# Michaelszeng/GCS-ADMM

Measured on AMD Instinct MI355X. Metric: admm_iterations_per_sec, higher is better.
Workload: dtype f64; 1 GPU; benchmark4; V=42, E=94, n=2, state_dtype=f64, state_columns=incidence, inner_arithmetic=f64, vertex_program=workgroup, vertex_solves=warm start from the previous iteration's record (csrc/warm_start.h), parallelism=1 GPU

## Files before the change

gcs_admm_amd/abi.py:

```python
from __future__ import annotations

import ctypes as C
import os

import numpy as np

LIB_PATH = os.path.join(os.path.dirname(os.path.abspath(__file__)), "libgcsadmm.so")

F64, F32 = 0, 1
RUNNING, CONVERGED, MAX_IT, DIVERGED = -1, 0, 1, 2
STATUS_NAME = {RUNNING: "running", CONVERGED: "converged", MAX_IT: "max_it", DIVERGED: "diverged"}


class GraphDesc(C.Structure):
    _fields_ = [("n", C.c_int32), ("num_vertices", C.c_int32), ("num_edges", C.c_int32), ("num_incidences", C.c_int32),
                ("inc_ptr", C.c_void_p), ("inc_edge", C.c_void_p), ("inc_out", C.c_void_p),
                ("edge_inc_tail", C.c_void_p), ("edge_inc_head", C.c_void_p),
                ("poly_ptr", C.c_void_p), ("poly_A", C.c_void_p), ("poly_b", C.c_void_p), ("center", C.c_void_p),
                ("src", C.c_int32), ("dst", C.c_int32), ("state_dtype", C.c_int32), ("device", C.c_int32),
                ("inc_counted", C.c_void_p), ("edge_counted", C.c_void_p),
                ("nx_global", C.c_double), ("nmu_global", C.c_double),
                ("vertex_program", C.c_int32), ("wave_slots", C.c_int32), ("wave_align", C.c_int32),
                ("wave_store_dl", C.c_int32), ("wave_generic_rows", C.c_int32), ("edge_major_columns", C.c_int32),
                ("vertex_workspace", C.c_int32)]


class Params(C.Structure):
    _fields_ = [("rho", C.c_double), ("tau_incr", C.c_double), ("tau_decr", C.c_double), ("nu", C.c_double),
                ("it_rho_limit", C.c_int32), ("max_it", C.c_int32), ("eps_abs", C.c_double), ("eps_rel", C.c_double),
                ("eps_edge", C.c_double), ("ipm_tol", C.c_double), ("ipm_max_iter", C.c_int32), ("cold_start", C.c_int32)]


class State(C.Structure):
    _fields_ = [("copy", C.c_void_p), ("mu", C.c_void_p), ("zedge", C.c_void_p),
                ("xv", C.c_void_p), ("zv", C.c_void_p), ("yv", C.c_void_p)]


class HaloDesc(C.Structure):
    _fields_ = [("num_peers", C.c_int32), ("peer_rank", C.c_void_p), ("send_ptr", C.c_void_p), ("send_cols", C.c_void_p),
                ("recv_ptr", C.c_void_p), ("recv_cols", C.c_void_p)]


class ControlBlock(C.Structure):
    _fields_ = [("rho", C.c_double), ("mu_scale", C.c_double), ("sums", C.c_double * 5),
                ("pri", C.c_double), ("dual", C.c_double), ("eps_pri", C.c_double), ("eps_dual", C.c_double),
                ("it", C.c_int32), ("status", C.c_int32), ("inner_failures", C.c_int32), ("inner_iters", C.c_int32)]


_p, _i, _d = C.c_void_p, C.c_int32, C.c_double
_run, _run_timed = [_p, _p, _i, _p, _p], [_p, _p, _i, _p, _p] + [_p] * 4
_csr = [_i, _i, _p, _p, _p]
PROTOTYPES = {
    "gcsadmm_create": ([_p, _p], _i),
    "gcsadmm_destroy": ([_p], None),
    "gcsadmm_last_error": ([_p], C.c_char_p),
    "gcsadmm_reset": ([_p] * 3, _i),
    "gcsadmm_vertex_step": ([_p] * 3, _i),
    "gcsadmm_edge_step": ([_p] * 4, _i),
    "gcsadmm_control": ([_p] * 4, _i),
    "gcsadmm_run": (_run, _i),
    "gcsadmm_read_control": ([_p] * 3, _i),
    "gcsadmm_cost": ([_p, _p, _d, _p, _p], _i),
    "gcsadmm_query": ([_p] * 6, _i),
    "gcsadmm_query_workspace": ([_p] * 4, _i),
    "gcsadmm_unit_iterations": ([_p, _p, _i, _p, _p], _i),
    "gcsadmm_run_timed": (_run_timed, _i),
    "gcsadmm_batch_create": ([_p, _i, _p], _i),
    "gcsadmm_batch_destroy": ([_p], None),
    "gcsadmm_batch_last_error": ([_p], C.c_char_p),
    "gcsadmm_batch_bind": ([_p] * 4, _i),
    "gcsadmm_batch_run": ([_p, _i, _p], _i),
    "gcsadmm_batch_poll": ([_p] * 4, _i),
    "gcsadmm_vertex_prox": ([_p] * 6 + [_d, _i, _p, _p], _i),
    "gcsadmm_comm_unique_id": ([_p], _i),
    "gcsadmm_attach_comm": ([_p, _i, _i, _p, _p], _i),
    "gcsadmm_check_halo": ([_p, _i, _i, _p], _i),
    "gcsadmm_run_partitioned": (_run, _i),
    "gcsadmm_run_partitioned_timed": (_run_timed, _i),
    "gcsadmm_set_overlap": ([_p, _i, _p], _i),
    "gcsadmm_comm_count": ([_p, _p], _i),
    "gcsadmm_halo_pack": ([_p] * 3, _i),
    "gcsadmm_halo_unpack": ([_p] * 3, _i),
    "gcsadmm_halo_exchange": ([_p] * 3, _i),
    "gcsadmm_halo_buffers": ([_p] * 4, _i),
    "gcsadmm_polytope_last_error": ([], C.c_char_p),
    "gcsadmm_polytope_centers": (_csr + [_i, _p, _p, _p], _i),
    "gcsadmm_polytope_bounds": (_csr + [_p, _i, _p, _p, _p], _i),
    "gcsadmm_polytope_overlaps": (_csr + [_p, C.c_long, _p, _p, _d, _i, _p, _p], _i),
    "gcsadmm_scene_create": (_csr + [_i, _p], _i),
    "gcsadmm_scene_destroy": ([_p], None),
    "gcsadmm_scene_centers": ([_p] * 4, _i),
    "gcsadmm_scene_bounds": ([_p] * 4, _i),
    "gcsadmm_scene_set_boxes": ([_p] * 3, _i),
    "gcsadmm_scene_candidate_pairs": ([_p, _d, _p], _i),
    "gcsadmm_scene_overlaps": ([_p, _d, _p, _p], _i),
    "gcsadmm_scene_read_pairs": ([_p] * 5, _i),
    "gcsadmm_scene_restrict_paths": ([_p, _i, _p, _p, _p, _d, _i, _p, _p, _p, _p], _i),
    "gcsadmm_scene_locate_points": ([_p, _i, _p, _d, _d, _p], _i),
    "gcsadmm_scene_read_hits": ([_p] * 4, _i),
}
EXPORTS = list(PROTOTYPES)


class GcsAdmmError(RuntimeError):
    pass


def check(status, message):
    if status:
        raise GcsAdmmError(message())


_libs = {}


def load_library(path: str | None = None) -> C.CDLL:
    path = path or LIB_PATH
    if path not in _libs:
        if not os.path.exists(path):
            raise RuntimeError(f"{path} is missing: run `python -m gcs_admm_amd.build` (hipcc, gfx950). "
                               "There is no CPU fallback.")
        import torch
        lib = C.CDLL(path)
        for name, (argtypes, restype) in PROTOTYPES.items():
            f = getattr(lib, name)
            f.argtypes, f.restype = argtypes, restype
        _libs[path] = lib
    return _libs[path]


def graph_desc(g, *, state_dtype, device, num_incidences=None, inc_counted=None, edge_counted=None, nx_global=0.0,
               nmu_global=0.0, columns="incidence", **knobs):
    if columns not in ("incidence", "edge"):
        raise ValueError("columns must be 'incidence' or 'edge'")
    E = g.num_edges
    NI = int(num_incidences) if num_incidences is not None else int(g.inc_ptr[-1])
    tail, head = g.edge_inc_tail.astype(np.int32), g.edge_inc_head.astype(np.int32)
    col_of = np.arange(NI, dtype=np.int64)
    if columns == "edge":
        if NI != 2 * E:
            raise ValueError("edge-major columns need exactly two columns per edge")
        col_of = np.empty(NI, dtype=np.int64)
        col_of[tail] = np.arange(E); col_of[head] = E + np.arange(E)
        tail, head = np.arange(E, dtype=np.int32), (E + np.arange(E)).astype(np.int32)
        if inc_counted is not None:
            ic = np.empty(NI, dtype=np.uint8)
            ic[col_of] = np.asarray(inc_counted, dtype=np.uint8)
            inc_counted = ic
    arrays = dict(inc_ptr=g.inc_ptr.astype(np.int32), inc_edge=g.inc_edge.astype(np.int32), inc_out=g.inc_out.astype(np.int32),
                  edge_inc_tail=tail, edge_inc_head=head, poly_ptr=g.poly_ptr.astype(np.int32), poly_A=g.poly_A.astype(np.float64),
                  poly_b=g.poly_b.astype(np.float64), center=g.interior.astype(np.float64),
                  inc_counted=None if inc_counted is None else np.asarray(inc_counted, dtype=np.uint8),
                  edge_counted=None if edge_counted is None else np.asarray(edge_counted, dtype=np.uint8))
    arrays = {k: None if a is None else np.ascontiguousarray(a) for k, a in arrays.items()}
    desc = GraphDesc(n=g.n, num_vertices=g.num_vertices, num_edges=E, num_incidences=NI, src=g.src, dst=g.dst,
                     state_dtype=state_dtype, device=device, nx_global=float(nx_global), nmu_global=float(nmu_global),
                     edge_major_columns=int(columns == "edge"), **{k: int(v) for k, v in knobs.items()},
                     **{k: None if a is None else a.ctypes.data for k, a in arrays.items()})
    return desc, list(arrays.values()), col_of
```

gcs_admm_amd/build.py:

```python
from __future__ import annotations

import os
import shutil
import subprocess
import sys

HERE = os.path.dirname(os.path.abspath(__file__))
ROOT = os.path.dirname(HERE)
CSRC = os.path.join(HERE, "csrc")
MAIN = os.path.join(CSRC, "gcsadmm.hip")
WG = os.path.join(CSRC, "vertex_wg.hip")
WGD = os.path.join(CSRC, "vertex_wg_dims.hip")
LP = os.path.join(CSRC, "polytope_lp.hip")
TERM = os.path.join(CSRC, "terminal_region.hip")
T512 = ["-DGCS_WG_THREADS=512", "-Dgcs_wg=gcs_wg_t512", "-DGCS_WG_SYM(name)=name##_t512"]
UNITS = [(MAIN, "gcsadmm.o", []), (WG, "vertex_wg.o", []), (WG, "vertex_wg_t512.o", T512), (WGD, "vertex_wg_dims.o", []), (WGD, "vertex_wg_dims_t512.o", T512),
         (LP, "polytope_lp.o", []), (TERM, "terminal_region.o", [])]
HDR = os.path.join(ROOT, "include", "gcsadmm.h")
_c = lambda *names: [os.path.join(CSRC, f) for f in names]
DEPS = [MAIN, HDR] + _c("vertex_program.h", "vertex_program.inc", "vertex_kernel.h", "special_vertex.h", "vertex_wg_launch.h", "canonical_box.h", "create_plan.h", "batch_plan.h", "warm_start.h", "terminal_launch.h", "step_args.h", "gcs_math.h", "hip_owners.h")
UNIT_DEPS = {LP: [LP, HDR] + _c("polytope_lp_core.h", "box_sweep_core.h", "point_locate_core.h", "path_restrict_core.h", "restrict_plan.h", "hip_owners.h", "step_args.h", "gcs_math.h"),
             WG: [WG, HDR] + _c("vertex_wg.h", "vertex_wg_kernel.h", "vertex_wg_launch.h", "special_vertex.h", "gcs_math.h", "warm_start.h", "step_args.h")}
UNIT_DEPS[WGD] = [WGD] + UNIT_DEPS[WG][1:]
UNIT_DEPS[TERM] = [TERM, HDR] + _c("terminal_region.h", "terminal_launch.h", "gcs_math.h", "warm_start.h", "step_args.h")
OUT = os.path.join(HERE, "libgcsadmm.so")


def hipcc() -> str:
    for c in (os.environ.get("HIPCC"), "/opt/rocm/bin/hipcc", shutil.which("hipcc")):
        if c and os.path.exists(c):
            return c
    raise RuntimeError("hipcc not found")


def build(force: bool = False, verbose: bool = False) -> str:
    if not force and os.path.exists(OUT) and all(os.path.getmtime(OUT) >= os.path.getmtime(d) for d in DEPS + UNIT_DEPS[LP] + UNIT_DEPS[WG] + UNIT_DEPS[WGD] + UNIT_DEPS[TERM]):
        return OUT
    flags = ["-Rpass-analysis=kernel-resource-usage", "--offload-arch=gfx950", "-O3", "-std=c++17", "-fPIC",
             "-I" + os.path.join(ROOT, "include"), "-I" + CSRC]
    objs, procs = [], []
    for src, name, extra in UNITS:
        obj = os.path.join(HERE, name)
        objs.append(obj)
        if force or not os.path.exists(obj) or not os.path.exists(obj + ".resources.txt") or \
                any(os.path.getmtime(obj) < os.path.getmtime(d) for d in UNIT_DEPS.get(src, DEPS)):
            log = open(obj + ".resources.txt", "w")
            procs.append((name, subprocess.Popen([hipcc()] + flags + extra + ["-c", src, "-o", obj], stderr=log), log))
    for name, p, log in procs:
        rc = p.wait()
        log.close()
        text = open(os.path.join(HERE, name) + ".resources.txt").read()
        if verbose or rc != 0:
            sys.stderr.write(text)
        if rc != 0:
            os.remove(os.path.join(HERE, name) + ".resources.txt")
            raise RuntimeError(f"hipcc failed on {name}")
    subprocess.check_call([hipcc(), "--offload-arch=gfx950", "-shared", "-fPIC"] + objs + ["-o", OUT])
    return OUT


def kernel_resources() -> dict:
    import re
    build()
    out = {}
    for _, name, _ in UNITS:
        cur = None
        for line in open(os.path.join(HERE, name) + ".resources.txt"):
            m = re.search(r"Function Name: (\S+)", line)
            if m:
                cur = out.setdefault(m.group(1), {})
                continue
            if cur is None:
                continue
            for key, pat in (("vgprs", r" VGPRs: (\d+)"), ("agprs", r"AGPRs: (\d+)"), ("scratch", r"ScratchSize \[bytes/lane\]: (\d+)"),
                             ("lds", r"LDS Size \[bytes/block\]: (\d+)")):
                m = re.search(pat, line)
                if m:
                    cur[key] = int(m.group(1))
    return out


def build_timing() -> str:
    out = os.path.join(HERE, "libgcsadmm_timing.so")
    flags = ["--offload-arch=gfx950", "-O3", "-std=c++17", "-fPIC", "-I" + os.path.join(ROOT, "include"), "-I" + CSRC]
    build()
    obj = os.path.join(HERE, "vertex_wg_t512_timing.o")
    subprocess.check_call([hipcc()] + flags + T512 + ["-DGCS_WG_TIMING", "-c", WG, "-o", obj])
    tobj = os.path.join(HERE, "terminal_region_timing.o")
    subprocess.check_call([hipcc()] + flags + ["-DGCS_TERM_TIMING", "-c", TERM, "-o", tobj])
    objs = [os.path.join(HERE, n) for n in ("gcsadmm.o", "polytope_lp.o", "vertex_wg.o", "vertex_wg_dims.o", "vertex_wg_dims_t512.o")] + [obj, tobj]
    subprocess.check_call([hipcc(), "--offload-arch=gfx950", "-shared", "-fPIC"] + objs + ["-o", out])
    return out


if __name__ == "__main__":
    if "--timing" in sys.argv:
        print(build_timing())
        sys.exit(0)
    print(build(force="--force" in sys.argv, verbose="--verbose" in sys.argv))
```

gcs_admm_amd/csrc/create_plan.h:

```cpp
#pragma once
#include <algorithm>
#include <cmath>
#include <string>
#include <vector>

#include "canonical_box.h"
#include "gcsadmm.h"
#include "step_args.h"
#include "vertex_program.h"
#include "warm_start.h"

int gcsadmm_wg_lds_bytes(int n, int units, int facets, bool box = false);
int gcsadmm_wg_lds_bytes_t512(int n, int units, int facets, bool box = false);
bool gcsadmm_wg_has_box(int n);
long long gcsadmm_terminal_ws_doubles(int n, int facets, int live_edges);
long long gcsadmm_terminal_record_doubles(int n, int facets, int live_edges);

namespace gcsadmm_k {

constexpr int EDGE_BLOCK = 256;
constexpr int REORDER_MIN_UNITS = 512;
constexpr int LDS_CU_BYTES = 160 * 1024;

inline int edge_unroll_rt(int dtype, int c, int E)
{
    const int u = dtype == GCSADMM_F32 ? (c <= 7 ? 4 : 2) : (c <= 7 ? 2 : 1);
    return (E + EDGE_BLOCK * u - 1) / (EDGE_BLOCK * u) >= 256 ? u : 1;
}

struct CreatePlan {
    std::vector<int> deg_in;
    std::vector<double> bc;
    std::vector<int> special_vtx, special_kind;
    int n_term = 0, term_vtx[2] = {-1, -1}, term_is_src[2] = {0, 0};
    long long term_ws_off[2] = {0, 0}, term_rec_off[2] = {0, 0}, term_ws_doubles = 0, term_rec_doubles = 0;
    int term_threads = 256, term_lds_doubles = 0;
    std::vector<int> wg_vtx;
    int wg_lds_bytes = 0, wg_box = 0, wg_t512 = 0;
    std::vector<int> split_vtx;
    std::vector<long long> split_off;
    long long split_doubles = 0;
    int split_lds_bytes = 0;
    std::vector<int> wave_slot_ptr{0}, wave_vtx;
    int slots_cap = 1, align_rows = 0, store_dl = 0, all_m4 = 0;
    int wave_mm = 1;
    int lds_bytes = 0;
    std::vector<long long> warm_ptr;
    bool wave_reorder = false, wg_reorder = false;
    std::vector<int> prox_vtx;
    int prox_lds_bytes = 0;
    std::vector<char> col_owned;
    std::vector<int> col_vertex;
    double nx = 0, nmu = 0;
    int edge_unroll = 1, edge_blocks = 1;
    int n_waves() const { return (int)wave_slot_ptr.size() - 1; }
};

inline gcsadmm_status check_graph_desc(const gcsadmm_graph_desc *g, std::string &err)
{
    auto fail = [&](gcsadmm_status st, const char *msg) { err = msg; return st; };
    if (!g) return fail(GCSADMM_ERR_BAD_ARG, "null descriptor or output pointer");
    if (g->n < 1 || g->n > 8) return fail(GCSADMM_ERR_UNSUPPORTED, "the vertex kernels are instantiated for n = 1 .. 8");
    if (g->num_vertices < 0 || g->num_edges < 0) return fail(GCSADMM_ERR_BAD_ARG, "negative size");
    if (!g->inc_ptr || !g->poly_ptr || (g->num_edges > 0 && (!g->inc_edge || !g->inc_out || !g->edge_inc_tail || !g->edge_inc_head)) ||
        (g->num_vertices > 0 && (!g->poly_A || !g->poly_b || !g->center)))
        return fail(GCSADMM_ERR_BAD_ARG, "null graph array");
    if (g->state_dtype != GCSADMM_F64 && g->state_dtype != GCSADMM_F32) return fail(GCSADMM_ERR_BAD_ARG, "bad state_dtype");
    const int NIo = g->inc_ptr[g->num_vertices];
    if (g->inc_ptr[0] != 0 || NIo < 0 || g->num_incidences < NIo) return fail(GCSADMM_ERR_BAD_ARG, "inconsistent incidence CSR");
    return GCSADMM_OK;
}

inline gcsadmm_status make_create_plan(const gcsadmm_graph_desc &g, CreatePlan &p, std::string &err)
{
    auto fail = [&](gcsadmm_status st, const char *msg) { err = msg; return st; };
    const int V = g.num_vertices, E = g.num_edges, n = g.n;
    p = CreatePlan();

    std::vector<int> deg(V), fac(V);
    p.deg_in.assign(V, 0);
    int mm_all = 1;
    for (int v = 0; v < V; ++v) {
        const int lo = g.inc_ptr[v], hi = g.inc_ptr[v + 1];
        if (hi < lo) return fail(GCSADMM_ERR_BAD_ARG, "inc_ptr not monotone");
        bool seen_out = false;
        for (int k = lo; k < hi; ++k) {
            if (g.inc_edge[k] < 0 || g.inc_edge[k] >= E) return fail(GCSADMM_ERR_BAD_ARG, "inc_edge out of range");
            if (g.inc_out[k]) seen_out = true;
            else { if (seen_out) return fail(GCSADMM_ERR_BAD_ARG, "incoming incidences must precede outgoing ones"); p.deg_in[v]++; }
        }
        deg[v] = hi - lo;
        fac[v] = g.poly_ptr[v + 1] - g.poly_ptr[v];
        if (fac[v] < n + 1) return fail(GCSADMM_ERR_BAD_ARG, "polytope with fewer than n+1 facets cannot be bounded");
        mm_all = std::max(mm_all, fac[v]);
    }
    for (int e = 0; e < E; ++e)
        if (g.edge_inc_tail[e] < 0 || g.edge_inc_tail[e] >= g.num_incidences || g.edge_inc_head[e] < 0 || g.edge_inc_head[e] >= g.num_incidences)
            return fail(GCSADMM_ERR_BAD_ARG, "edge incidence slot out of range");
    if (g.edge_major_columns != 0 && g.edge_major_columns != 1) return fail(GCSADMM_ERR_BAD_ARG, "edge_major_columns must be 0 or 1");
    if (g.edge_major_columns) {
        if (g.num_incidences != 2 * (int64_t)E) return fail(GCSADMM_ERR_BAD_ARG, "edge-major columns: num_incidences must be 2 num_edges");
        for (int e = 0; e < E; ++e)
            if (g.edge_inc_tail[e] != e || g.edge_inc_head[e] != E + e)
                return fail(GCSADMM_ERR_BAD_ARG, "edge-major columns: edge_inc_tail[e] must be e and edge_inc_head[e] num_edges + e");
    }
    auto poly_A = [&](int v) { return g.poly_A + (size_t)g.poly_ptr[v] * n; };

    const int MT = g.poly_ptr[V];
    p.bc.assign(MT > 0 ? MT : 1, 0.0);
    for (int v = 0; v < V; ++v)
        for (int j = g.poly_ptr[v]; j < g.poly_ptr[v + 1]; ++j) {
            double s = g.poly_b[j];
            for (int k = 0; k < n; ++k) s -= g.poly_A[(size_t)j * n + k] * g.center[(size_t)v * n + k];
            p.bc[j] = s;
            if (v != g.src && v != g.dst && !(s > 0.0)) return fail(GCSADMM_ERR_BAD_ARG, "center is not strictly inside its polytope");
        }

    auto live_edges = [&](int v, bool is_src) { return is_src ? deg[v] - p.deg_in[v] : p.deg_in[v]; };
    for (int term : {g.src, g.dst}) {
        if (term < 0 || term >= V) continue;
        double ext = 0;
        for (int j = g.poly_ptr[term]; j < g.poly_ptr[term + 1]; ++j) {
            double nrm = 0;
            for (int k = 0; k < n; ++k) nrm += g.poly_A[(size_t)j * n + k] * g.poly_A[(size_t)j * n + k];
            ext = std::max(ext, std::fabs(p.bc[j]) / std::sqrt(nrm > 0 ? nrm : 1.0));
        }
        if (ext > 1e-5) {
            if (g.src == g.dst) return fail(GCSADMM_ERR_UNSUPPORTED, "source and target are the same region");
            if (live_edges(term, term == g.src) < 1)
                return fail(GCSADMM_ERR_UNSUPPORTED, "a terminal that is a region needs an edge on its live side (outgoing for the source, incoming for the target)");
            p.term_vtx[p.n_term] = term; p.term_is_src[p.n_term] = term == g.src; ++p.n_term;
        }
    }
    auto is_region_terminal = [&](int v) { return (p.n_term > 0 && v == p.term_vtx[0]) || (p.n_term > 1 && v == p.term_vtx[1]); };
    auto is_special = [&](int v) { return v == g.src || v == g.dst || p.deg_in[v] == 0 || deg[v] - p.deg_in[v] == 0; };
    int n_generic = 0;
    for (int v = 0; v < V; ++v) n_generic += !is_region_terminal(v) && !is_special(v);
    constexpr int WG_AUTO_MAX = 1024;
    if (g.vertex_program < 0 || g.vertex_program > 3) return fail(GCSADMM_ERR_BAD_ARG, "vertex_program must be 0, 1, 2 or 3");
    if (g.vertex_workspace < 0 || g.vertex_workspace > 2) return fail(GCSADMM_ERR_BAD_ARG, "vertex_workspace must be 0, 1 or 2");
    const int ws_mode = g.vertex_workspace;
    const bool prefer_wg = g.vertex_program >= 2 || (g.vertex_program == 0 && n_generic <= WG_AUTO_MAX);
    bool wg_box = g.wave_generic_rows == 0 && gcsadmm_wg_has_box(n);
    bool wave_box = n == 2 && g.wave_generic_rows != 1 && g.wave_generic_rows != 2;
    std::vector<int> wave_cand;
    p.warm_ptr.assign(V + 1, 0);
    for (int v = 0; v < V; ++v) {
        p.warm_ptr[v + 1] = p.warm_ptr[v];
        if (is_region_terminal(v)) continue;
        if (is_special(v)) {
            if (deg[v] > MAX_SPECIAL_DEG) return fail(GCSADMM_ERR_UNSUPPORTED, "terminal vertex degree above 256");
            p.special_vtx.push_back(v);
            p.special_kind.push_back(v == g.src ? 1 : (v == g.dst ? 2 : 0));
            continue;
        }
        p.warm_ptr[v + 1] += gcs_ws::warm_record_doubles(n, fac[v], deg[v]);
        const bool wave_too_small = ws_mode == 1 && n == 2 && (size_t)gcs::lds_doubles(n, fac[v], 1, 0) * 8 > (size_t)LDS_CU_BYTES;
        if (n != 2 || deg[v] + 1 > gcs::WAVE || prefer_wg || wave_too_small) {
            p.wg_vtx.push_back(v);
            if (wg_box && !canonical_box(n, fac[v], poly_A(v))) wg_box = false;
        } else {
            wave_cand.push_back(v);
            p.wave_mm = std::max(p.wave_mm, fac[v]);
            if (wave_box && !canonical_box(2, fac[v], poly_A(v))) wave_box = false;
        }
    }

    const int n_wg = (int)p.wg_vtx.size();
    p.wg_t512 = n_wg > 0 && g.vertex_program != 3 && n_wg + 1 <= 256;
    p.wg_box = n_wg > 0 && wg_box;
    auto wg_bytes = [&](int v) { return p.wg_t512 ? gcsadmm_wg_lds_bytes_t512(n, deg[v] + 1, fac[v], wg_box)
                                                  : gcsadmm_wg_lds_bytes(n, deg[v] + 1, fac[v], wg_box); };
    if (ws_mode > 0) {
        std::vector<int> keep;
        for (int v : p.wg_vtx) (ws_mode == 2 || wg_bytes(v) > LDS_CU_BYTES ? p.split_vtx : keep).push_back(v);
        p.wg_vtx.swap(keep);
    }
    for (int v : p.wg_vtx) p.wg_lds_bytes = std::max(p.wg_lds_bytes, wg_bytes(v));
    if (p.wg_lds_bytes > LDS_CU_BYTES) return fail(GCSADMM_ERR_UNSUPPORTED, "a vertex sub-problem (degree x facets) does not fit the 160 KB of LDS of a CU");
    auto heavier = [&](int a, int b) { return (long)(deg[a] + 1) * fac[a] > (long)(deg[b] + 1) * fac[b]; };
    std::stable_sort(p.wg_vtx.begin(), p.wg_vtx.end(), heavier);
    std::stable_sort(p.split_vtx.begin(), p.split_vtx.end(), heavier);
    for (int v : p.split_vtx) {
        const int lds = gcsadmm_wg_lds_bytes(n, 0, fac[v], wg_box);
        if (lds > LDS_CU_BYTES) return fail(GCSADMM_ERR_UNSUPPORTED, "a vertex's border system and polytope do not fit the 160 KB of LDS of a CU");
        p.split_lds_bytes = std::max(p.split_lds_bytes, lds);
        p.split_off.push_back(p.split_doubles);
        p.split_doubles += ((gcsadmm_wg_lds_bytes(n, deg[v] + 1, fac[v], wg_box) - lds) / 8 + 31) / 32 * 32;
    }

    auto lds_need = [&](int slots, int store_dl) {
        return (size_t)(wave_box ? gcs_box::lds_doubles(n, p.wave_mm, slots, store_dl) : gcs::lds_doubles(n, p.wave_mm, slots, store_dl)) * 8;
    };
    int slots_max = gcs::MAX_SLOTS;
    if (!wave_cand.empty()) {
        while (slots_max > 1 && lds_need(slots_max, 0) > LDS_CU_BYTES) --slots_max;
        if (lds_need(slots_max, 0) > LDS_CU_BYTES) return fail(GCSADMM_ERR_UNSUPPORTED, "facet count too large for LDS");
        if (g.wave_slots > 0) slots_max = std::max(1, std::min(slots_max, (int)g.wave_slots));
        else slots_max = std::min(slots_max, std::max(1, ((int)wave_cand.size() + 1023) / 1024));
    }
    auto pack = [&](int align) {
        p.wave_slot_ptr.assign(1, 0); p.wave_vtx.clear();
        int lanes = 0, slots = 0, slots_used = 0;
        for (int v : wave_cand) {
            int base = gcs::group_base(lanes, deg[v], p.deg_in[v], align);
            if (base < 0 || slots + 1 > slots_max) {
                p.wave_slot_ptr.push_back((int)p.wave_vtx.size());
                slots = 0;
                base = gcs::group_base(0, deg[v], p.deg_in[v], align);
            }
            p.wave_vtx.push_back(v);
            lanes = base + deg[v] + 1; slots += 1;
            slots_used = std::max(slots_used, slots);
        }
        if ((int)p.wave_vtx.size() > p.wave_slot_ptr.back()) p.wave_slot_ptr.push_back((int)p.wave_vtx.size());
        p.slots_cap = std::max(1, slots_used);
    };
    pack(1);
    p.align_rows = g.wave_align == 1 ? 1 : (g.wave_align == 2 ? 0 : (p.n_waves() > 2048 ? 0 : 1));
    if (!p.align_rows) pack(0);
    p.all_m4 = wave_box ? 2 : 0;
    if (p.n_waves() > 0) {
        p.store_dl = g.wave_store_dl == 1 ? 1 : (g.wave_store_dl == 2 ? 0 : (lds_need(p.slots_cap, 1) <= 40 * 1024 ? 1 : 0));
        if (p.store_dl && lds_need(p.slots_cap, 1) > LDS_CU_BYTES) p.store_dl = 0;
        p.lds_bytes = (int)lds_need(p.slots_cap, p.store_dl);
    }

    long long largest = 0;
    int rows = 0;
    for (int i = 0; i < p.n_term; ++i) {
        const int v = p.term_vtx[i], live = live_edges(v, p.term_is_src[i]);
        const long long need = gcsadmm_terminal_ws_doubles(n, fac[v], live);
        p.term_ws_off[i] = p.term_ws_doubles; p.term_ws_doubles += need; largest = std::max(largest, need);
        p.term_rec_off[i] = p.term_rec_doubles; p.term_rec_doubles += gcsadmm_terminal_record_doubles(n, fac[v], live);
        rows = std::max(rows, live * 2 * fac[v]);
    }
    if (p.n_term > 0) {
        p.term_lds_doubles = largest * 8 <= 48 * 1024 ? (int)largest : 0;
        p.term_threads = rows <= 256 ? 64 : 256;
    }

    p.wave_reorder = p.n_waves() >= REORDER_MIN_UNITS;
    p.wg_reorder = n_wg >= REORDER_MIN_UNITS;
    for (int v = 0; v < V; ++v)
        if (v != g.src && v != g.dst) p.prox_vtx.push_back(v);
    p.prox_lds_bytes = gcsadmm_wg_lds_bytes(n, 1, mm_all);

    const size_t ncol = (size_t)std::max<int64_t>(g.num_incidences, 1);
    p.col_owned.assign(ncol, 0);
    p.col_vertex.assign(ncol, -1);
    for (int v = 0; v < V; ++v)
        for (int k = g.inc_ptr[v]; k < g.inc_ptr[v + 1]; ++k) {
            const int col = state_column(g.edge_major_columns, E, 0, k, g.inc_edge[k], g.inc_out[k]);
            p.col_owned[col] = 1; p.col_vertex[col] = v;
        }
    p.nx = g.nx_global > 0 ? g.nx_global : (4.0 * n + 1) * (V + 2.0 * E);
    p.nmu = g.nmu_global > 0 ? g.nmu_global : (4.0 * n + 2) * E;
    p.edge_unroll = edge_unroll_rt(g.state_dtype, 2 * n + 1, E);
    const int tile = EDGE_BLOCK * p.edge_unroll;
    p.edge_blocks = std::max(1, std::min((E + tile - 1) / tile, 2048));
    return GCSADMM_OK;
}

}
```

gcs_admm_amd/csrc/gcsadmm.hip:

```cpp
#include <hip/hip_runtime.h>
#include <dlfcn.h>
#include <rccl/rccl.h>

#include <algorithm>
#include <cmath>
#include <cstdio>
#include <cstring>
#include <memory>
#include <new>
#include <string>
#include <type_traits>
#include <vector>

#include "gcsadmm.h"
#include "hip_owners.h"
#include "terminal_launch.h"
#ifdef GCS_PHASE_TIMING
__device__ unsigned long long g_sub_cycles[16];
__device__ __forceinline__ void gcs_stamp(int k)
{
    static __shared__ unsigned long long last;
    __builtin_amdgcn_sched_barrier(0);
    if (threadIdx.x == 0) {
        const unsigned long long t = __builtin_amdgcn_s_memtime();
        if (k > 0) atomicAdd(&g_sub_cycles[k], t - last);
        last = t;
    }
    __builtin_amdgcn_sched_barrier(0);
}
#define GCS_STAMP(k) gcs_stamp(k)
#endif
#include "vertex_kernel.h"
#include "vertex_wg_launch.h"
#include "warm_start.h"
#include "canonical_box.h"
#include "create_plan.h"
#include "batch_plan.h"

namespace {

using namespace gcs;
using namespace gcsadmm_k;

template <class T> struct EdgeArgs {
    int E, NI, c;
    const int *edge_inc_tail, *edge_inc_head;
    const uint8_t *inc_counted, *edge_counted;
    const T *copy;
    T *zedge, *mu;
    double *partials;
};

__device__ __forceinline__ double wave_sum(double v)
{
#pragma unroll
    for (int off = 32; off > 0; off >>= 1) v += __shfl_down(v, off, 64);
    return v;
}

__device__ __forceinline__ double scaled_plus(double scale, double x, double r)
{
#pragma clang fp contract(off)
    return scale * x + r;
}

struct ControlParams {
    double tau_incr, tau_decr, nu, eps_abs, eps_rel, nx, nmu;
    int it_rho_limit, max_it;
};

__device__ void control_body(gcsadmm_control_block *cb, const double *sums, const ControlParams &p, int *counters, double *trace,
                             bool global_fails = false)
{
    if (cb->status != GCSADMM_RUNNING) return;
    double s[5];
    for (int k = 0; k < 5; ++k) { s[k] = sums[k]; cb->sums[k] = s[k]; }
    const int it = cb->it;
    double rho = cb->rho;
    const int fails = global_fails ? (int)(sums[5] + 0.5) : counters[0], iters = counters[1];
    counters[0] = 0; counters[1] = 0;
    cb->inner_failures = fails; cb->inner_iters = iters;
    const double tot = s[0] + s[1] + s[2] + s[3] + s[4];
    if (!(fabs(tot) <= 1.7976931348623157e308)) {
        cb->status = GCSADMM_DIVERGED;
        return;
    }
    const double pri = sqrt(s[0]), dual = rho * sqrt(2.0 * s[1]);
    double mu_scale = 1.0;
    if (pri >= p.nu * dual && it < p.it_rho_limit) { rho *= p.tau_incr; mu_scale = 1.0 / p.tau_incr; }
    else if (dual >= p.nu * pri && it < p.it_rho_limit) { rho *= 1.0 / p.tau_decr; mu_scale = p.tau_incr; }
    const double eps_pri = sqrt(p.nx) * p.eps_abs + p.eps_rel * fmax(sqrt(s[2]), sqrt(2.0 * s[3]));
    const double eps_dual = sqrt(p.nmu) * p.eps_abs + p.eps_rel * mu_scale * sqrt(s[4]);
    cb->rho = rho; cb->mu_scale = mu_scale;
    cb->pri = pri; cb->dual = dual; cb->eps_pri = eps_pri; cb->eps_dual = eps_dual;
    if (trace) {
        double *tr = trace + (size_t)(it - 1) * 6;
        tr[0] = rho; tr[1] = pri; tr[2] = dual; tr[3] = eps_pri; tr[4] = eps_dual; tr[5] = (double)fails;
    }
    if (pri < eps_pri && dual < eps_dual) { cb->status = GCSADMM_CONVERGED; return; }
    cb->it = it + 1;
    if (it + 1 > p.max_it) cb->status = GCSADMM_MAX_IT;
}

__global__ void control_kernel(gcsadmm_control_block *cb, const double *sums, ControlParams p, int *counters, double *trace, bool global_fails)
{
    if (threadIdx.x != 0 || blockIdx.x != 0) return;
    control_body(cb, sums, p, counters, trace, global_fails);
}

template <class T, int C> __host__ __device__ constexpr int edge_unroll() { return sizeof(T) == 4 ? (C <= 7 ? 4 : 2) : (C <= 7 ? 2 : 1); }

template <class T, int MODE, int C, int U>
__device__ __forceinline__ void edge_body(const EdgeArgs<T> &a, gcsadmm_control_block *cb, double *sums, const ControlParams &cp, int *counters,
                                          double *trace, unsigned *ticket, const unsigned bx, const unsigned nblocks, double (*red)[5], int *is_last)
{
    if (cb->status != GCSADMM_RUNNING) return;
    const double mu_scale = cb->mu_scale;
    double s[5] = {0, 0, 0, 0, 0};
    for (int base = bx * (U * EDGE_BLOCK); base < a.E; base += nblocks * (U * EDGE_BLOCK)) {
        int it[U], ih[U];
        T cu_[U][C], cw_[U][C], zo_[U][C], mu_[U][C], mw_[U][C];
#pragma unroll
        for (int q = 0; q < U; ++q) {
            const int e = base + q * EDGE_BLOCK + (int)threadIdx.x, ee = e < a.E ? e : a.E - 1;
            it[q] = a.edge_inc_tail ? a.edge_inc_tail[ee] : ee; ih[q] = a.edge_inc_head ? a.edge_inc_head[ee] : a.E + ee;
#pragma unroll
            for (int w = 0; w < C; ++w) {
                cu_[q][w] = a.copy[(size_t)w * a.NI + it[q]]; cw_[q][w] = a.copy[(size_t)w * a.NI + ih[q]];
                zo_[q][w] = a.zedge[(size_t)w * a.E + ee];
                mu_[q][w] = a.mu[(size_t)w * a.NI + it[q]]; mw_[q][w] = a.mu[(size_t)w * a.NI + ih[q]];
            }
        }
#pragma unroll
        for (int q = 0; q < U; ++q) {
            const int e = base + q * EDGE_BLOCK + (int)threadIdx.x;
            if (e >= a.E) break;
            const double we = a.edge_counted ? (double)a.edge_counted[e] : 1.0;
            const double wt = a.inc_counted ? (double)a.inc_counted[it[q]] : 1.0;
            const double wh = a.inc_counted ? (double)a.inc_counted[ih[q]] : 1.0;
#pragma unroll
            for (int w = 0; w < C; ++w) {
                const double cu = (double)cu_[q][w], cw = (double)cw_[q][w], zo = (double)zo_[q][w];
                const T zn_t = (T)(0.5 * (cu + cw));
                const double zn = (double)zn_t;
                const double ru = cu - zn, rw = cw - zn;
                const T mu_u_t = (T)scaled_plus(mu_scale, (double)mu_[q][w], ru);
                const T mu_w_t = (T)scaled_plus(mu_scale, (double)mw_[q][w], rw);
                a.mu[(size_t)w * a.NI + it[q]] = mu_u_t;
                a.mu[(size_t)w * a.NI + ih[q]] = mu_w_t;
                a.zedge[(size_t)w * a.E + e] = zn_t;
                const double mu_u = (double)mu_u_t, mu_w = (double)mu_w_t;
                s[0] += wt * ru * ru + wh * rw * rw;
                s[1] += we * (zn - zo) * (zn - zo);
                s[2] += wt * cu * cu + wh * cw * cw;
                s[3] += we * zn * zn;
                s[4] += wt * mu_u * mu_u + wh * mu_w * mu_w;
            }
        }
    }
    const int lane = threadIdx.x & 63, wv = threadIdx.x >> 6;
#pragma unroll
    for (int k = 0; k < 5; ++k) {
        const double t = wave_sum(s[k]);
        if (lane == 0) red[wv][k] = t;
    }
    __syncthreads();
    if (threadIdx.x < 5) {
        double t = 0;
        for (int q = 0; q < EDGE_BLOCK / WAVE; ++q) t += red[q][threadIdx.x];
        if (MODE >= 2) __hip_atomic_store(&a.partials[(size_t)bx * 5 + threadIdx.x], t, __ATOMIC_RELAXED, __HIP_MEMORY_SCOPE_AGENT);
        else a.partials[(size_t)bx * 5 + threadIdx.x] = t;
        if (MODE == 1) sums[threadIdx.x] = t;
    }
    if (MODE == 1) {
        __syncthreads();
        if (threadIdx.x == 0) control_body(cb, sums, cp, counters, trace);
    }
    if (MODE >= 2) {
        if (threadIdx.x < WAVE) asm volatile("s_waitcnt vmcnt(0)" ::: "memory");
        if (threadIdx.x == 0) {
            const unsigned t = __hip_atomic_fetch_add(ticket, 1u, __ATOMIC_RELAXED, __HIP_MEMORY_SCOPE_AGENT);
            *is_last = (t == nblocks - 1);
        }
        __syncthreads();
        if (!*is_last) return;
        double acc[5] = {0, 0, 0, 0, 0};
        for (int b = threadIdx.x; b < (int)nblocks; b += EDGE_BLOCK)
            for (int k = 0; k < 5; ++k) acc[k] += __hip_atomic_load(&a.partials[(size_t)b * 5 + k], __ATOMIC_RELAXED, __HIP_MEMORY_SCOPE_AGENT);
        __syncthreads();
        for (int k = 0; k < 5; ++k) red[threadIdx.x][k] = acc[k];
        __syncthreads();
        for (int off = EDGE_BLOCK / 2; off > 0; off >>= 1) {
            if ((int)threadIdx.x < off)
                for (int k = 0; k < 5; ++k) red[threadIdx.x][k] += red[threadIdx.x + off][k];
            __syncthreads();
        }
        if (threadIdx.x < 5) sums[threadIdx.x] = red[0][threadIdx.x];
        __syncthreads();
        if (threadIdx.x == 0) {
            if (MODE == 2) control_body(cb, sums, cp, counters, trace);
            else sums[5] = (double)counters[0];
            __hip_atomic_store(ticket, 0u, __ATOMIC_RELAXED, __HIP_MEMORY_SCOPE_AGENT);
        }
    }
}

template <class T, int MODE, int C, int U>
__global__ __launch_bounds__(EDGE_BLOCK) void edge_kernel(EdgeArgs<T> a, gcsadmm_control_block *cb, double *sums, ControlParams cp,
                                                          int *counters, double *trace, unsigned *ticket)
{
    __shared__ double red[EDGE_BLOCK][5];
    __shared__ int is_last;
    edge_body<T, MODE, C, U>(a, cb, sums, cp, counters, trace, ticket, blockIdx.x, gridDim.x, red, &is_last);
}

template <class T> struct EdgeBatchEntry {
    EdgeArgs<T> a;
    gcsadmm_control_block *cb;
    double *sums;
    ControlParams cp;
    int *counters;
    double *trace;
    unsigned *ticket;
    int nblocks;
};
template <class T, int C>
__global__ __launch_bounds__(EDGE_BLOCK) void edge_batch_kernel(const EdgeBatchEntry<T> *__restrict__ table)
{
    __shared__ double red[EDGE_BLOCK][5];
    __shared__ int is_last;
    __builtin_assume_dereferenceable(table + blockIdx.y, sizeof(EdgeBatchEntry<T>));
    const EdgeBatchEntry<T> e = *(const EdgeBatchEntry<T> *)((const __attribute__((address_space(4))) EdgeBatchEntry<T> *)table + blockIdx.y);
    if ((int)blockIdx.x >= e.nblocks) return;
    if (e.nblocks == 1) edge_body<T, 1, C, 1>(e.a, e.cb, e.sums, e.cp, e.counters, e.trace, e.ticket, 0, 1, red, &is_last);
    else edge_body<T, 2, C, 1>(e.a, e.cb, e.sums, e.cp, e.counters, e.trace, e.ticket, blockIdx.x, (unsigned)e.nblocks, red, &is_last);
}

__global__ __launch_bounds__(256) void batch_poll_kernel(const gcsadmm_control_block *const *cbs, int count, int *out)
{
    const int i = blockIdx.x * blockDim.x + threadIdx.x;
    if (i >= count) return;
    out[i] = cbs[i]->status;
    out[count + i] = cbs[i]->it;
}

constexpr int REORDER_BINS = 64, REORDER_THREADS = 1024, REORDER_EVERY = 8;
__global__ __launch_bounds__(REORDER_THREADS) void reorder_kernel(int n, const int *iters, int *order, const gcsadmm_control_block *cb, const int *ids = nullptr)
{
    if (cb->status != GCSADMM_RUNNING) return;
    __shared__ int cnt[REORDER_BINS], off[REORDER_BINS];
    if (threadIdx.x < REORDER_BINS) cnt[threadIdx.x] = 0;
    __syncthreads();
    auto unit = [&](int i) { return ids ? ids[i] : i; };
    auto key = [&](int i) { const int k = iters[unit(i)]; return k < 0 ? 0 : (k >= REORDER_BINS ? REORDER_BINS - 1 : k); };
    for (int i = threadIdx.x; i < n; i += REORDER_THREADS) atomicAdd(&cnt[key(i)], 1);
    __syncthreads();
    if (threadIdx.x == 0) {
        int run = 0;
        for (int b = REORDER_BINS - 1; b >= 0; --b) { off[b] = run; run += cnt[b]; }
    }
    __syncthreads();
    for (int i = threadIdx.x; i < n; i += REORDER_THREADS) order[atomicAdd(&off[key(i)], 1)] = unit(i);
}

__global__ __launch_bounds__(256) void finalize_kernel(const double *partials, int nblocks, double *sums,
                                                      const gcsadmm_control_block *cb)
{
    if (cb->status != GCSADMM_RUNNING) return;
    __shared__ double red[256][5];
    double s[5] = {0, 0, 0, 0, 0};
    for (int b = threadIdx.x; b < nblocks; b += 256)
        for (int k = 0; k < 5; ++k) s[k] += partials[(size_t)b * 5 + k];
    for (int k = 0; k < 5; ++k) red[threadIdx.x][k] = s[k];
    __syncthreads();
    for (int off = 128; off > 0; off >>= 1) {
        if ((int)threadIdx.x < off)
            for (int k = 0; k < 5; ++k) red[threadIdx.x][k] += red[threadIdx.x + off][k];
        __syncthreads();
    }
    if (threadIdx.x < 5) sums[threadIdx.x] = red[0][threadIdx.x];
}

template <class T>
__global__ __launch_bounds__(256) void halo_pack_kernel(int c, int ncols, int NI, const int *cols, const int *base, const int *stride,
                                                        const T *copy, T *buf, const gcsadmm_control_block *cb)
{
    if (cb->status != GCSADMM_RUNNING) return;
    const int t = blockIdx.x * blockDim.x + threadIdx.x;
    if (t >= c * ncols) return;
    const int w = t / ncols, j = t - w * ncols;
    buf[base[j] + w * stride[j]] = copy[(size_t)w * NI + cols[j]];
}
template <class T>
__global__ __launch_bounds__(256) void halo_unpack_kernel(int c, int ncols, int NI, const int *cols, const int *base, const int *stride,
                                                          const T *buf, T *copy, const gcsadmm_control_block *cb)
{
    if (cb->status != GCSADMM_RUNNING) return;
    const int t = blockIdx.x * blockDim.x + threadIdx.x;
    if (t >= c * ncols) return;
    const int w = t / ncols, j = t - w * ncols;
    copy[(size_t)w * NI + cols[j]] = buf[base[j] + w * stride[j]];
}
template <class T>
__global__ __launch_bounds__(256) void cost_kernel(int V, int E, int n, const double *zv, const T *zedge,
                                                   const uint8_t *edge_counted, double eps_edge, double *cost)
{
    __shared__ double red[256];
    double s = 0;
    for (int v = threadIdx.x; v < V; v += 256) {
        double q = 0;
        for (int k = 0; k < n; ++k) { const double dlt = zv[(size_t)v * 2 * n + k] - zv[(size_t)v * 2 * n + n + k]; q += dlt * dlt; }
        s += sqrt(q);
    }
    for (int e = threadIdx.x; e < E; e += 256)
        s += eps_edge * (edge_counted ? (double)edge_counted[e] : 1.0) * (double)zedge[(size_t)(2 * n) * E + e];
    red[threadIdx.x] = s;
    __syncthreads();
    for (int off = 128; off > 0; off >>= 1) {
        if ((int)threadIdx.x < off) red[threadIdx.x] += red[threadIdx.x + off];
        __syncthreads();
    }
    if (threadIdx.x == 0) cost[0] = red[0];
}


}

struct Halo {
    std::vector<int> peers, peer_cnt, peer_off;
    std::vector<int> send_cols;
    int n_send = 0, n_recv = 0;
    DevBuf<int> d_send_cols, d_send_base, d_send_stride, d_recv_cols, d_recv_base, d_recv_stride;
    DevBuf<char> d_sendbuf, d_recvbuf;
    DevBuf<double> d_sums6;
    bool attached() const { return (bool)d_sums6; }
};
struct Overlap {
    int n_wave_b = 0;
    DevBuf<int> d_split_ids, d_split_order;
    Stream comm_stream;
    Event ev_boundary, ev_halo;
};
struct Terminals {
    DevBuf<double> d_term_ws, d_term_rec;
    Stream term_stream;
    Event ev_term_fork, ev_term_join;
};

struct gcsadmm_handle_s {
    int n = 0, V = 0, E = 0, NI = 0, c = 0, dtype = 0, device = 0, src = -1, dst = -1;
    int edge_major = 0;
    CreatePlan plan;
    gcsadmm_params params{};
    bool params_set = false;
    int vertex_steps = 0;
    unsigned resets = 0;
    gcsadmm_batch_s *batch = nullptr;
    std::vector<gcsadmm_batch_s *> batches;
    int overlap_mode = 0;
    std::string err;
    void *comm = nullptr;
    int rank = 0, world = 1;
    std::vector<int> iota;
    struct Graph {
        DevBuf<int> d_inc_ptr, d_deg_in, d_inc_edge, d_poly_ptr, d_edge_inc_tail, d_edge_inc_head;
        DevBuf<int> d_wave_slot_ptr, d_wave_vtx, d_special_vtx, d_special_kind, d_wg_vtx;
        DevBuf<double> d_poly_A, d_poly_bc, d_center;
        DevBuf<uint8_t> d_inc_counted, d_edge_counted;
        DevBuf<int> d_split_vtx;
        DevBuf<long long> d_split_off;
        DevBuf<double> d_split_ws;
        DevBuf<double> d_warm;
        DevBuf<long long> d_warm_ptr;
        DevBuf<int> d_wave_iters, d_wave_order, d_wg_iters, d_wg_order;
    } g;
    struct Loop {
        DevBuf<gcsadmm_control_block> d_cb;
        DevBuf<int> d_counters;
        DevBuf<double> d_partials, d_sums;
        DevBuf<unsigned> d_ticket;
    } loop;
    struct Prox { DevBuf<int> d_prox_vtx, d_prox_counters; } prox;
    Halo halo;
    Overlap overlap;
    Terminals term;
    std::vector<Event> events;

    int n_special() const { return (int)g.d_special_vtx.size(); }
    int n_wg() const { return (int)g.d_wg_vtx.size(); }
    int n_split() const { return (int)g.d_split_vtx.size(); }
};

struct gcsadmm_batch_s {
    int device = 0;
    std::string err;
    std::vector<gcsadmm_handle> members;
    std::vector<unsigned> resets;
    BatchPlan plan;
    bool bound = false;
    DevBuf<char> d_vertex_table, d_edge_table;
    DevBuf<const gcsadmm_control_block *> d_cbs;
    DevBuf<int> d_poll;
    std::vector<int> poll_host;
};

namespace {
struct RcclApi {
    void *lib = nullptr;
    decltype(&ncclGetUniqueId) GetUniqueId = nullptr;
    decltype(&ncclCommInitRank) CommInitRank = nullptr;
    decltype(&ncclCommDestroy) CommDestroy = nullptr;
    decltype(&ncclGroupStart) GroupStart = nullptr;
    decltype(&ncclGroupEnd) GroupEnd = nullptr;
    decltype(&ncclSend) Send = nullptr;
    decltype(&ncclRecv) Recv = nullptr;
    decltype(&ncclAllReduce) AllReduce = nullptr;
    decltype(&ncclGetErrorString) GetErrorString = nullptr;
    decltype(&ncclCommCount) CommCount = nullptr;
    std::string err;
    bool ok() const { return lib && GetUniqueId && CommInitRank && CommDestroy && GroupStart && GroupEnd && Send && Recv && AllReduce; }
};
RcclApi &rccl()
{
    static RcclApi api = [] {
        RcclApi a;
        for (const char *name : {"librccl.so.1", "librccl.so"}) {
            a.lib = dlopen(name, RTLD_NOW | RTLD_GLOBAL);
            if (a.lib) break;
        }
        if (!a.lib) {
            const char *why = dlerror();
            a.err = std::string("dlopen(librccl): ") + (why ? why : "not found");
            return a;
        }
#define RCCL_SYM(f) a.f = (decltype(a.f))dlsym(a.lib, "nccl" #f)
        RCCL_SYM(GetUniqueId); RCCL_SYM(CommInitRank); RCCL_SYM(CommDestroy); RCCL_SYM(GroupStart); RCCL_SYM(GroupEnd);
        RCCL_SYM(Send); RCCL_SYM(Recv); RCCL_SYM(AllReduce); RCCL_SYM(GetErrorString); RCCL_SYM(CommCount);
#undef RCCL_SYM
        if (!a.ok()) a.err = "librccl lacks an expected symbol";
        return a;
    }();
    return api;
}
}
#define NCCLCHK(h, call)                                                                             \
    do {                                                                                             \
        ncclResult_t r_ = (call);                                                                    \
        if (r_ != ncclSuccess) {                                                                     \
            (h)->err = std::string(#call) + ": " + (rccl().GetErrorString ? rccl().GetErrorString(r_) : "RCCL error"); \
            return GCSADMM_ERR_HIP;                                                                  \
        }                                                                                            \
    } while (0)


static thread_local std::string g_create_error;

#define USE_DEVICE(h)                                                                               \
    DeviceGuard device_guard_((h)->device);                                                          \
    do {                                                                                             \
        if (device_guard_.err != hipSuccess) {                                                       \
            (h)->err = std::string("hipSetDevice: ") + hipGetErrorString(device_guard_.err);        \
            return GCSADMM_ERR_HIP;                                                                  \
        }                                                                                            \
    } while (0)

#define HIPCHK(h, call)                                                                              \
    do {                                                                                             \
        hipError_t e_ = (call);                                                                      \
        if (e_ != hipSuccess) {                                                                      \
            (h)->err = std::string(#call) + ": " + hipGetErrorString(e_);                            \
            return GCSADMM_ERR_HIP;                                                                  \
        }                                                                                            \
    } while (0)

template <class F> static auto with_state(const gcsadmm_handle_s *h, F &&f) { return with_state_type(h->dtype == GCSADMM_F64, f); }
static size_t state_bytes(const gcsadmm_handle_s *h) { return h->dtype == GCSADMM_F64 ? 8 : 4; }

static ControlParams control_params(const gcsadmm_handle_s *h)
{
    const gcsadmm_params &p = h->params;
    return ControlParams{p.tau_incr, p.tau_decr, p.nu, p.eps_abs, p.eps_rel, h->plan.nx, h->plan.nmu, p.it_rho_limit, p.max_it};
}

static StepDesc make_step(gcsadmm_handle h, const gcsadmm_state *st)
{
    StepDesc a;
    a.inc_ptr = h->g.d_inc_ptr.get(); a.deg_in = h->g.d_deg_in.get(); a.inc_edge = h->g.d_inc_edge.get(); a.poly_ptr = h->g.d_poly_ptr.get();
    a.poly_A = h->g.d_poly_A.get(); a.poly_bc = h->g.d_poly_bc.get(); a.center = h->g.d_center.get();
    a.E = h->E; a.NI = h->NI; a.edge_major = h->edge_major;
    a.zedge = st->zedge; a.mu = st->mu; a.copy = st->copy; a.xv = st->xv; a.zv = st->zv; a.yv = st->yv;
    a.counters = h->loop.d_counters.get(); a.cb = h->loop.d_cb.get();
    a.eps_edge = h->params.eps_edge; a.ipm_tol = h->params.ipm_tol; a.ipm_max_iter = h->params.ipm_max_iter;
    a.warm = h->params.cold_start ? nullptr : h->g.d_warm.get(); a.warm_ptr = h->g.d_warm_ptr.get();
    return a;
}

static WgLaunchDesc make_wg_desc(gcsadmm_handle h, const gcsadmm_state *st, bool with_special)
{
    WgLaunchDesc d;
    d.step = make_step(h, st);
    d.n = h->n; d.dtype = h->dtype; d.n_vtx = h->n_wg(); d.n_special = with_special ? h->n_special() : 0; d.lds_bytes = h->plan.wg_lds_bytes;
    d.vtx = h->g.d_wg_vtx.get(); d.special_vtx = h->g.d_special_vtx.get(); d.special_kind = h->g.d_special_kind.get(); d.box = h->plan.wg_box;
    d.order = h->g.d_wg_order.get(); d.unit_iters = h->g.d_wg_iters.get();
    return d;
}

static gcsadmm_k::TermLaunchDesc make_term_desc(gcsadmm_handle h, const gcsadmm_state *st)
{
    gcsadmm_k::TermLaunchDesc d;
    const CreatePlan &p = h->plan;
    d.step = make_step(h, st);
    d.n = h->n; d.dtype = h->dtype; d.count = p.n_term; d.threads = p.term_threads; d.lds_doubles = p.term_lds_doubles;
    for (int i = 0; i < 2; ++i) {
        d.t.vtx[i] = p.term_vtx[i]; d.t.is_src[i] = p.term_is_src[i]; d.t.ws_off[i] = p.term_ws_off[i]; d.t.rec_off[i] = p.term_rec_off[i];
    }
    d.t.ws = h->term.d_term_ws.get();
    d.t.rec = h->params.cold_start ? nullptr : h->term.d_term_rec.get();
    return d;
}

static VertexLaunchDesc make_launch_desc(gcsadmm_handle h, const gcsadmm_state *st)
{
    VertexLaunchDesc d;
    const CreatePlan &p = h->plan;
    d.step = make_step(h, st);
    d.n_waves = p.n_waves(); d.n_special = h->n_special(); d.all_m4 = p.all_m4; d.lds_bytes = p.lds_bytes; d.align_rows = p.align_rows;
    d.store_dl = p.store_dl; d.MM = p.wave_mm;
    d.wave_slot_ptr = h->g.d_wave_slot_ptr.get(); d.wave_vtx = h->g.d_wave_vtx.get(); d.special_vtx = h->g.d_special_vtx.get(); d.special_kind = h->g.d_special_kind.get();
    d.wave_order = h->g.d_wave_order.get(); d.wave_iters = h->g.d_wave_iters.get();
    return d;
}

static gcsadmm_status launch_vertex(gcsadmm_handle h, const gcsadmm_state *st, hipStream_t s, int part = -1, bool reorder = false)
{
    const auto &g = h->g;
    const int n_waves = h->plan.n_waves();
    const gcsadmm_control_block *cb = h->loop.d_cb.get();
    auto launch_waves = [&](const VertexLaunchDesc &d) { with_state(h, [&](auto t) { launch_vertex_dim<2, decltype(t)>(d, s); }); };
    const bool with_term = h->plan.n_term > 0 && part <= 0;
    if (with_term) {
        HIPCHK(h, hipEventRecord(h->term.ev_term_fork.get(), s));
        HIPCHK(h, hipStreamWaitEvent(h->term.term_stream.get(), h->term.ev_term_fork.get(), 0));
        gcsadmm_terminal_launch(make_term_desc(h, st), h->term.term_stream.get());
        HIPCHK(h, hipEventRecord(h->term.ev_term_join.get(), h->term.term_stream.get()));
    }
    struct Join {
        gcsadmm_handle h; hipStream_t s; bool on;
        ~Join() { if (on) (void)hipStreamWaitEvent(s, h->term.ev_term_join.get(), 0); }
    } join_{h, s, with_term};
    if (part >= 0) {
        const Overlap &o = h->overlap;
        VertexLaunchDesc d = make_launch_desc(h, st);
        const int off = part ? o.n_wave_b : 0, cnt = part ? n_waves - o.n_wave_b : o.n_wave_b;
        d.wave_order = o.d_split_order.get() + off;
        d.n_waves = cnt;
        if (part) d.n_special = 0;
        launch_waves(d);
        if (reorder && g.d_wave_iters)
            hipLaunchKernelGGL(reorder_kernel, dim3(1), dim3(REORDER_THREADS), 0, s, cnt, g.d_wave_iters.get(), o.d_split_order.get() + off, cb, o.d_split_ids.get() + off);
        HIPCHK(h, hipGetLastError());
        return GCSADMM_OK;
    }
    const bool special_on_wave = n_waves > 0;
    if (n_waves > 0) launch_waves(make_launch_desc(h, st));
    if (h->n_wg() > 0 || (!special_on_wave && h->n_special() > 0)) {
        if (h->plan.wg_t512) gcsadmm_wg_launch_t512(make_wg_desc(h, st, !special_on_wave), s);
        else gcsadmm_wg_launch(make_wg_desc(h, st, !special_on_wave), s);
    }
    if (h->n_split() > 0) {
        WgLaunchDesc d = make_wg_desc(h, st, false);
        d.n_vtx = h->n_split(); d.vtx = g.d_split_vtx.get(); d.lds_bytes = h->plan.split_lds_bytes; d.order = nullptr; d.unit_iters = nullptr;
        gcsadmm_wg_launch_split(d, WgSplitArgs{g.d_split_ws.get(), g.d_split_off.get()}, s);
    }
    if (++h->vertex_steps % REORDER_EVERY == 0) {
        if (g.d_wave_order) hipLaunchKernelGGL(reorder_kernel, dim3(1), dim3(REORDER_THREADS), 0, s, n_waves, g.d_wave_iters.get(), g.d_wave_order.get(), cb);
        if (g.d_wg_order) hipLaunchKernelGGL(reorder_kernel, dim3(1), dim3(REORDER_THREADS), 0, s, h->n_wg(), g.d_wg_iters.get(), g.d_wg_order.get(), cb);
    }
    HIPCHK(h, hipGetLastError());
    return GCSADMM_OK;
}

template <class T> static EdgeArgs<T> make_edge_args(gcsadmm_handle h, const gcsadmm_state *st)
{
    EdgeArgs<T> a;
    a.E = h->E; a.NI = h->NI; a.c = h->c;
    a.edge_inc_tail = h->edge_major ? nullptr : h->g.d_edge_inc_tail.get(); a.edge_inc_head = h->edge_major ? nullptr : h->g.d_edge_inc_head.get();
    a.inc_counted = h->g.d_inc_counted.get(); a.edge_counted = h->g.d_edge_counted.get();
    a.copy = (const T *)st->copy; a.zedge = (T *)st->zedge; a.mu = (T *)st->mu; a.partials = h->loop.d_partials.get();
    return a;
}

static gcsadmm_status launch_edge(gcsadmm_handle h, const gcsadmm_state *st, double *sums, hipStream_t s, bool with_control = false,
                                  double *trace = nullptr, bool sums6 = false)
{
    const ControlParams cp = control_params(h);
    const int edge_blocks = h->plan.edge_blocks;
    with_state(h, [&](auto t) {
        using T = decltype(t);
        const EdgeArgs<T> a = make_edge_args<T>(h, st);
        auto go = [&](auto mode, int blocks) {
            constexpr int M = decltype(mode)::value;
#define GCS_EDGE_U(CC, UU) hipLaunchKernelGGL((edge_kernel<T, M, CC, UU>), dim3(blocks), dim3(EDGE_BLOCK), 0, s, a, h->loop.d_cb.get(), sums, cp, h->loop.d_counters.get(), trace, h->loop.d_ticket.get())
#define GCS_EDGE(CC) do { if (h->plan.edge_unroll > 1) GCS_EDGE_U(CC, (edge_unroll<T, CC>())); else GCS_EDGE_U(CC, 1); } while (0)
            switch (h->c) {
            case 3: GCS_EDGE(3); break;
            case 5: GCS_EDGE(5); break;
            case 7: GCS_EDGE(7); break;
            case 9: GCS_EDGE(9); break;
            case 11: GCS_EDGE(11); break;
            case 13: GCS_EDGE(13); break;
            case 15: GCS_EDGE(15); break;
            default: GCS_EDGE(17);
            }
#undef GCS_EDGE_U
#undef GCS_EDGE
        };
        if (sums6) go(std::integral_constant<int, 3>(), edge_blocks);
        else if (with_control && edge_blocks == 1) go(std::integral_constant<int, 1>(), 1);
        else if (with_control) go(std::integral_constant<int, 2>(), edge_blocks);
        else {
            go(std::integral_constant<int, 0>(), edge_blocks);
            hipLaunchKernelGGL(finalize_kernel, dim3(1), dim3(256), 0, s, a.partials, edge_blocks, sums, h->loop.d_cb.get());
        }
    });
    HIPCHK(h, hipGetLastError());
    return GCSADMM_OK;
}

static bool state_ok(gcsadmm_handle h, const gcsadmm_state *st)
{
    if (!h || !st || !st->copy || !st->mu || !st->zedge || !st->xv || !st->zv || !st->yv) { if (h) h->err = "null state pointer"; return false; }
    if (!h->params_set) { h->err = "gcsadmm_reset has not been called"; return false; }
    return true;
}

static gcsadmm_status halo_validate(gcsadmm_handle h, int rank, int world, const gcsadmm_halo_desc *hd)
{
    if (!hd || world < 1 || rank < 0 || rank >= world) { h->err = "bad communicator arguments"; return GCSADMM_ERR_BAD_ARG; }
    const int P = hd->num_peers;
    if (P < 0 || (P > 0 && (!hd->peer_rank || !hd->send_ptr || !hd->recv_ptr || !hd->send_cols || !hd->recv_cols))) { h->err = "null halo array"; return GCSADMM_ERR_BAD_ARG; }
    const int n_send = P ? hd->send_ptr[P] : 0, n_recv = P ? hd->recv_ptr[P] : 0;
    if (n_send != n_recv) { h->err = "halo lists: a partition sends and receives one column per cut edge and neighbour"; return GCSADMM_ERR_BAD_ARG; }
    for (int p = 0; p < P; ++p) {
        const int lo = hd->send_ptr[p], cnt = hd->send_ptr[p + 1] - lo;
        if (cnt < 0 || hd->recv_ptr[p + 1] - hd->recv_ptr[p] != cnt || hd->recv_ptr[p] != lo) { h->err = "halo lists: send and receive counts per peer must agree"; return GCSADMM_ERR_BAD_ARG; }
        if (hd->peer_rank[p] < 0 || hd->peer_rank[p] >= world || hd->peer_rank[p] == rank) { h->err = "halo lists: bad peer rank"; return GCSADMM_ERR_BAD_ARG; }
    }
    const std::vector<char> &col_owned = h->plan.col_owned;
    for (int j = 0; j < n_send; ++j) {
        if (hd->send_cols[j] < 0 || hd->send_cols[j] >= h->NI || hd->recv_cols[j] < 0 || hd->recv_cols[j] >= h->NI) { h->err = "halo lists: column out of range"; return GCSADMM_ERR_BAD_ARG; }
        if (!col_owned[hd->send_cols[j]]) { h->err = "halo lists: send column is not an owned incidence"; return GCSADMM_ERR_BAD_ARG; }
        if (col_owned[hd->recv_cols[j]]) { h->err = "halo lists: receive column is not a ghost column"; return GCSADMM_ERR_BAD_ARG; }
    }
    return GCSADMM_OK;
}

static gcsadmm_status overlap_setup(gcsadmm_handle h, const std::vector<int> &send_cols)
{
    const CreatePlan &p = h->plan;
    const int n_waves = p.n_waves(), n_send = (int)send_cols.size();
    Overlap &o = h->overlap;
    o = {};
    if (h->overlap_mode == 2 || n_waves < 2 || h->n_wg() > 0 || h->n_split() > 0) return GCSADMM_OK;
    if (n_send == 0 && h->overlap_mode != 1) return GCSADMM_OK;
    std::vector<char> vb((size_t)std::max(h->V, 1), 0);
    for (int j = 0; j < n_send; ++j) {
        const int v = p.col_vertex[send_cols[j]];
        if (v >= 0) vb[v] = 1;
    }
    std::vector<int> ids_b, ids_i;
    for (int w = 0; w < n_waves; ++w) {
        bool b = (n_send == 0) && w < std::max(1, n_waves / 4);
        for (int q = p.wave_slot_ptr[w]; q < p.wave_slot_ptr[w + 1] && !b; ++q) b = vb[p.wave_vtx[q]] != 0;
        (b ? ids_b : ids_i).push_back(w);
    }
    if (ids_b.empty() || ids_i.empty()) return GCSADMM_OK;
    o.n_wave_b = (int)ids_b.size();
    ids_b.insert(ids_b.end(), ids_i.begin(), ids_i.end());
    HIPCHK(h, o.d_split_ids.upload(ids_b.data(), ids_b.size()));
    HIPCHK(h, o.d_split_order.upload(ids_b.data(), ids_b.size()));
    if (!h->g.d_wave_iters) HIPCHK(h, h->g.d_wave_iters.upload(nullptr, (size_t)n_waves));
    HIPCHK(h, create_owned(o.comm_stream, hipStreamCreateWithFlags, hipStreamNonBlocking));
    HIPCHK(h, create_owned(o.ev_boundary, hipEventCreateWithFlags, hipEventDisableTiming));
    HIPCHK(h, create_owned(o.ev_halo, hipEventCreateWithFlags, hipEventDisableTiming));
    return GCSADMM_OK;
}

static gcsadmm_status halo_upload(gcsadmm_handle h, const gcsadmm_halo_desc *hd)
{
    const int P = hd->num_peers, c = h->c;
    Halo &H = h->halo;
    H.peers.assign(hd->peer_rank, hd->peer_rank + P);
    H.peer_cnt.resize(P); H.peer_off.resize(P);
    H.n_send = P ? hd->send_ptr[P] : 0; H.n_recv = P ? hd->recv_ptr[P] : 0;
    H.send_cols.assign(hd->send_cols, hd->send_cols + H.n_send);
    std::vector<int> sbase(std::max(H.n_send, 1)), sstride(std::max(H.n_send, 1));
    for (int p = 0; p < P; ++p) {
        const int lo = hd->send_ptr[p], cnt = hd->send_ptr[p + 1] - lo;
        H.peer_cnt[p] = cnt; H.peer_off[p] = lo;
        for (int j = 0; j < cnt; ++j) { sbase[lo + j] = lo * c + j; sstride[lo + j] = cnt; }
    }
    const size_t esz = state_bytes(h);
    HIPCHK(h, H.d_send_cols.upload(hd->send_cols, (size_t)H.n_send));
    HIPCHK(h, H.d_recv_cols.upload(hd->recv_cols, (size_t)H.n_recv));
    HIPCHK(h, H.d_send_base.upload(sbase.data(), (size_t)H.n_send));
    HIPCHK(h, H.d_send_stride.upload(sstride.data(), (size_t)H.n_send));
    HIPCHK(h, H.d_recv_base.upload(sbase.data(), (size_t)H.n_recv));
    HIPCHK(h, H.d_recv_stride.upload(sstride.data(), (size_t)H.n_recv));
    HIPCHK(h, H.d_sendbuf.alloc(std::max<size_t>((size_t)H.n_send * c * esz, 16)));
    HIPCHK(h, H.d_recvbuf.alloc(std::max<size_t>((size_t)H.n_recv * c * esz, 16)));
    HIPCHK(h, H.d_sums6.upload(nullptr, 12));
    return GCSADMM_OK;
}

template <class T> static gcsadmm_status halo_pack(gcsadmm_handle h, const gcsadmm_state *st, hipStream_t s)
{
    const Halo &H = h->halo;
    if (H.n_send == 0) return GCSADMM_OK;
    const int tot = h->c * H.n_send;
    hipLaunchKernelGGL((halo_pack_kernel<T>), dim3((tot + 255) / 256), dim3(256), 0, s, h->c, H.n_send, h->NI, H.d_send_cols.get(),
                       H.d_send_base.get(), H.d_send_stride.get(), (const T *)st->copy, (T *)H.d_sendbuf.get(), h->loop.d_cb.get());
    HIPCHK(h, hipGetLastError());
    return GCSADMM_OK;
}
template <class T> static gcsadmm_status halo_unpack(gcsadmm_handle h, const gcsadmm_state *st, hipStream_t s)
{
    const Halo &H = h->halo;
    if (H.n_recv == 0) return GCSADMM_OK;
    const int tot = h->c * H.n_recv;
    hipLaunchKernelGGL((halo_unpack_kernel<T>), dim3((tot + 255) / 256), dim3(256), 0, s, h->c, H.n_recv, h->NI, H.d_recv_cols.get(),
                       H.d_recv_base.get(), H.d_recv_stride.get(), (const T *)H.d_recvbuf.get(), (T *)st->copy, h->loop.d_cb.get());
    HIPCHK(h, hipGetLastError());
    return GCSADMM_OK;
}

static gcsadmm_status halo_transfer(gcsadmm_handle h, hipStream_t s)
{
    const Halo &H = h->halo;
    if (H.peers.empty()) return GCSADMM_OK;
    if (!h->comm) { h->err = "halo exchange needs a communicator (gcsadmm_attach_comm with an id)"; return GCSADMM_ERR_BAD_ARG; }
    const ncclDataType_t dt = h->dtype == GCSADMM_F64 ? ncclFloat64 : ncclFloat32;
    const size_t esz = state_bytes(h);
    NCCLCHK(h, rccl().GroupStart());
    for (size_t p = 0; p < H.peers.size(); ++p) {
        const size_t off = (size_t)H.peer_off[p] * h->c * esz, cnt = (size_t)H.peer_cnt[p] * h->c;
        NCCLCHK(h, rccl().Send(H.d_sendbuf.get() + off, cnt, dt, H.peers[p], (ncclComm_t)h->comm, s));
        NCCLCHK(h, rccl().Recv(H.d_recvbuf.get() + off, cnt, dt, H.peers[p], (ncclComm_t)h->comm, s));
    }
    NCCLCHK(h, rccl().GroupEnd());
    return GCSADMM_OK;
}

static gcsadmm_status ensure_events(gcsadmm_handle h, size_t count)
{
    while (h->events.size() < count) {
        Event e;
        HIPCHK(h, create_owned(e, hipEventCreateWithFlags, hipEventDefault));
        h->events.push_back(std::move(e));
    }
    return GCSADMM_OK;
}

static gcsadmm_status batch_plan_of(const std::vector<gcsadmm_handle> &members, BatchPlan &bp, std::string &err)
{
    std::vector<BatchMember> m;
    for (gcsadmm_handle h : members)
        m.push_back(h ? BatchMember{h, &h->plan, h->n, h->dtype, h->device, h->n_wg(), h->n_special(), h->n_split(), h->halo.attached() || h->comm != nullptr}
                      : BatchMember{});
    return make_batch_plan(m.data(), (int)m.size(), bp, err);
}

static void batch_unbind(gcsadmm_batch_s *b)
{
    for (gcsadmm_handle h : b->members)
        if (h && h->batch == b) h->batch = nullptr;
    b->bound = false;
}

static void batches_forget(gcsadmm_handle h)
{
    for (gcsadmm_batch_s *b : h->batches) {
        batch_unbind(b);
        std::replace(b->members.begin(), b->members.end(), h, (gcsadmm_handle) nullptr);
    }
}

static gcsadmm_status launch_batch_iteration(gcsadmm_batch_s *b, hipStream_t s)
{
    const BatchPlan &bp = b->plan;
    if (bp.vertex_grid_x > 0)
        gcsadmm_wg_launch_batch(WgBatchLaunch{bp.n, bp.dtype, bp.box, b->d_vertex_table.get(), (unsigned)bp.vertex_grid_x, (unsigned)bp.count, bp.vertex_lds_bytes}, s);
    with_state_type(bp.dtype == GCSADMM_F64, [&](auto t) {
        using T = decltype(t);
        const auto *table = (const EdgeBatchEntry<T> *)b->d_edge_table.get();
#define GCS_EDGE_BATCH(CC) hipLaunchKernelGGL((edge_batch_kernel<T, CC>), dim3(bp.edge_grid_x, bp.count), dim3(EDGE_BLOCK), 0, s, table)
        switch (2 * bp.n + 1) {
        case 3: GCS_EDGE_BATCH(3); break;
        case 5: GCS_EDGE_BATCH(5); break;
        case 7: GCS_EDGE_BATCH(7); break;
        case 9: GCS_EDGE_BATCH(9); break;
        case 11: GCS_EDGE_BATCH(11); break;
        case 13: GCS_EDGE_BATCH(13); break;
        case 15: GCS_EDGE_BATCH(15); break;
        default: GCS_EDGE_BATCH(17);
        }
#undef GCS_EDGE_BATCH
    });
    HIPCHK(b, hipGetLastError());
    return GCSADMM_OK;
}

extern "C" {

const char *gcsadmm_last_error(gcsadmm_handle h) { return h ? h->err.c_str() : g_create_error.c_str(); }

void gcsadmm_destroy(gcsadmm_handle h)
{
    if (!h) return;
    DeviceGuard device_guard_(h->device);
    batches_forget(h);
    if (h->comm && rccl().ok()) (void)rccl().CommDestroy((ncclComm_t)h->comm);
    delete h;
}

gcsadmm_status gcsadmm_create(const gcsadmm_graph_desc *g, gcsadmm_handle *out)
{
    if (out) *out = nullptr;
    auto fail = [&](gcsadmm_status st, const std::string &msg) { g_create_error = msg; return st; };
    std::string msg;
    gcsadmm_status st;
    if (!out) return fail(GCSADMM_ERR_BAD_ARG, "null descriptor or output pointer");
    if ((st = check_graph_desc(g, msg)) != GCSADMM_OK) return fail(st, msg);
    int ndev = 0;
    if (hipGetDeviceCount(&ndev) != hipSuccess || ndev <= 0) return fail(GCSADMM_ERR_NO_DEVICE, "no HIP device");
    if (g->device < 0 || g->device >= ndev) return fail(GCSADMM_ERR_BAD_ARG, "device ordinal out of range");
    CreatePlan plan;
    if ((st = make_create_plan(*g, plan, msg)) != GCSADMM_OK) return fail(st, msg);

    const int V = g->num_vertices, E = g->num_edges, n = g->n, NIo = g->inc_ptr[V], MT = g->poly_ptr[V];
    auto *h = new (std::nothrow) gcsadmm_handle_s;
    if (!h) return fail(GCSADMM_ERR_HIP, "out of host memory");
    h->n = n; h->V = V; h->E = E; h->NI = g->num_incidences; h->c = 2 * n + 1;
    h->edge_major = g->edge_major_columns; h->src = g->src; h->dst = g->dst;
    h->dtype = g->state_dtype; h->device = g->device;
    h->plan = std::move(plan);
    CreatePlan &p = h->plan;
    DeviceGuard device_guard_(g->device);
    auto bail = [&](hipError_t e, const char *what) {
        g_create_error = std::string(what) + ": " + hipGetErrorString(e);
        delete h;
        return GCSADMM_ERR_HIP;
    };
    hipError_t e;
    if ((e = device_guard_.err) != hipSuccess) return bail(e, "hipSetDevice");
#define UP(group, dst, src, cnt) if ((e = h->group.dst.upload(src, (size_t)(cnt))) != hipSuccess) return bail(e, "upload " #dst)
    UP(g, d_inc_ptr, g->inc_ptr, V + 1);
    UP(g, d_deg_in, p.deg_in.data(), V);
    UP(g, d_inc_edge, g->inc_edge, NIo);
    UP(g, d_poly_ptr, g->poly_ptr, V + 1);
    UP(g, d_edge_inc_tail, g->edge_inc_tail, E);
    UP(g, d_edge_inc_head, g->edge_inc_head, E);
    UP(g, d_wave_slot_ptr, p.wave_slot_ptr.data(), p.wave_slot_ptr.size());
    UP(g, d_wave_vtx, p.wave_vtx.data(), p.wave_vtx.size());
    UP(g, d_special_vtx, p.special_vtx.data(), p.special_vtx.size());
    UP(g, d_special_kind, p.special_kind.data(), p.special_kind.size());
    UP(g, d_wg_vtx, p.wg_vtx.data(), p.wg_vtx.size());
    if (!p.split_vtx.empty()) {
        UP(g, d_split_vtx, p.split_vtx.data(), p.split_vtx.size());
        UP(g, d_split_off, p.split_off.data(), p.split_off.size());
        UP(g, d_split_ws, nullptr, p.split_doubles);
    }
    UP(g, d_poly_A, g->poly_A, (size_t)MT * n);
    UP(g, d_poly_bc, p.bc.data(), MT);
    UP(g, d_center, g->center, (size_t)V * n);
    if (g->inc_counted) UP(g, d_inc_counted, g->inc_counted, g->num_incidences);
    if (g->edge_counted) UP(g, d_edge_counted, g->edge_counted, E);
    UP(loop, d_cb, nullptr, 1);
    UP(loop, d_counters, nullptr, 2);
    UP(loop, d_partials, nullptr, (size_t)p.edge_blocks * 5);
    UP(loop, d_sums, nullptr, 5);
    UP(loop, d_ticket, nullptr, 1);
    if (p.n_term > 0) {
        UP(term, d_term_ws, nullptr, p.term_ws_doubles);
        UP(term, d_term_rec, nullptr, p.term_rec_doubles);
        if ((e = create_owned(h->term.term_stream, hipStreamCreateWithFlags, hipStreamNonBlocking)) != hipSuccess) return bail(e, "hipStreamCreate");
        if ((e = create_owned(h->term.ev_term_fork, hipEventCreateWithFlags, hipEventDisableTiming)) != hipSuccess) return bail(e, "hipEventCreate");
        if ((e = create_owned(h->term.ev_term_join, hipEventCreateWithFlags, hipEventDisableTiming)) != hipSuccess) return bail(e, "hipEventCreate");
    }
    UP(g, d_warm_ptr, p.warm_ptr.data(), V + 1);
    UP(g, d_warm, nullptr, p.warm_ptr[V]);
    const int n_waves = p.n_waves(), n_wg = h->n_wg();
    h->iota.resize(std::max(std::max(n_waves, n_wg), 1));
    for (size_t i = 0; i < h->iota.size(); ++i) h->iota[i] = (int)i;
    if (p.wave_reorder) { UP(g, d_wave_iters, nullptr, n_waves); UP(g, d_wave_order, h->iota.data(), n_waves); }
    if (p.wg_reorder) { UP(g, d_wg_iters, nullptr, n_wg); UP(g, d_wg_order, h->iota.data(), n_wg); }
    UP(prox, d_prox_vtx, p.prox_vtx.data(), p.prox_vtx.size());
    UP(prox, d_prox_counters, nullptr, 2);
#undef UP
    auto release = [](auto &v) { v.clear(); v.shrink_to_fit(); };
    release(p.bc); release(p.deg_in); release(p.warm_ptr); release(p.prox_vtx); release(p.special_vtx); release(p.special_kind);
    release(p.wg_vtx); release(p.split_vtx); release(p.split_off);
    if (p.lds_bytes > 48 * 1024) {
        e = with_state(h, [&](auto t) { return set_lds_attr<2, decltype(t)>(p.all_m4, p.lds_bytes); });
        if (e != hipSuccess) return bail(e, "hipFuncSetAttribute(MaxDynamicSharedMemorySize)");
    }
    if (p.wg_lds_bytes > 48 * 1024 && (e = p.wg_t512 ? gcsadmm_wg_set_lds_t512(h->n, h->dtype, p.wg_lds_bytes)
                                                      : gcsadmm_wg_set_lds(h->n, h->dtype, p.wg_lds_bytes)) != hipSuccess)
        return bail(e, "hipFuncSetAttribute(MaxDynamicSharedMemorySize, workgroup program)");
    if (p.split_lds_bytes > 48 * 1024 && (e = gcsadmm_wg_set_split_lds(h->n, h->dtype, p.split_lds_bytes)) != hipSuccess)
        return bail(e, "hipFuncSetAttribute(MaxDynamicSharedMemorySize, split workgroup program)");
    *out = h;
    return GCSADMM_OK;
}

gcsadmm_status gcsadmm_reset(gcsadmm_handle h, const gcsadmm_params *p, void *stream)
{
    if (!h || !p) return GCSADMM_ERR_BAD_ARG;
    if (!(p->rho > 0) || p->max_it < 1 || !(p->ipm_tol > 0) || p->ipm_max_iter < 1) { h->err = "bad parameter"; return GCSADMM_ERR_BAD_ARG; }
    h->params = *p; h->params_set = true; ++h->resets;
    gcsadmm_control_block cb{};
    cb.rho = p->rho; cb.mu_scale = 1.0; cb.it = 1; cb.status = GCSADMM_RUNNING;
    USE_DEVICE(h);
    hipStream_t s = (hipStream_t)stream;
    HIPCHK(h, hipMemcpyAsync(h->loop.d_cb.get(), &cb, sizeof(cb), hipMemcpyHostToDevice, s));
    HIPCHK(h, h->loop.d_counters.zero(s));
    HIPCHK(h, h->g.d_warm.zero(s));
    HIPCHK(h, h->term.d_term_rec.zero(s));
    h->vertex_steps = 0;
    const Overlap &o = h->overlap;
    if (o.d_split_order) HIPCHK(h, hipMemcpyAsync(o.d_split_order.get(), o.d_split_ids.get(), sizeof(int) * o.d_split_order.size(), hipMemcpyDeviceToDevice, s));
    for (const DevBuf<int> *order : {&h->g.d_wave_order, &h->g.d_wg_order})
        if (*order) HIPCHK(h, hipMemcpyAsync(order->get(), h->iota.data(), sizeof(int) * order->size(), hipMemcpyHostToDevice, s));
    HIPCHK(h, hipStreamSynchronize(s));
    return GCSADMM_OK;
}

gcsadmm_status gcsadmm_vertex_step(gcsadmm_handle h, const gcsadmm_state *st, void *stream)
{
    if (!state_ok(h, st)) return GCSADMM_ERR_BAD_ARG;
    USE_DEVICE(h);
    return launch_vertex(h, st, (hipStream_t)stream);
}

gcsadmm_status gcsadmm_edge_step(gcsadmm_handle h, const gcsadmm_state *st, double *sums_dev, void *stream)
{
    if (!state_ok(h, st) || !sums_dev) return GCSADMM_ERR_BAD_ARG;
    USE_DEVICE(h);
    return launch_edge(h, st, sums_dev, (hipStream_t)stream);
}

gcsadmm_status gcsadmm_control(gcsadmm_handle h, const double *sums_dev, double *trace_dev, void *stream)
{
    if (!h || !sums_dev || !h->params_set) return GCSADMM_ERR_BAD_ARG;
    USE_DEVICE(h);
    hipLaunchKernelGGL(control_kernel, dim3(1), dim3(1), 0, (hipStream_t)stream, h->loop.d_cb.get(), sums_dev, control_params(h), h->loop.d_counters.get(), trace_dev, false);
    HIPCHK(h, hipGetLastError());
    return GCSADMM_OK;
}

gcsadmm_status gcsadmm_run(gcsadmm_handle h, const gcsadmm_state *st, int32_t k, double *trace_dev, void *stream)
{
    if (!state_ok(h, st) || k < 0) return GCSADMM_ERR_BAD_ARG;
    USE_DEVICE(h);
    for (int i = 0; i < k; ++i) {
        gcsadmm_status s;
        if ((s = gcsadmm_vertex_step(h, st, stream)) != GCSADMM_OK) return s;
        if ((s = launch_edge(h, st, h->loop.d_sums.get(), (hipStream_t)stream, true, trace_dev)) != GCSADMM_OK) return s;
    }
    return GCSADMM_OK;
}

gcsadmm_status gcsadmm_comm_unique_id(void *id128)
{
    if (!id128) return GCSADMM_ERR_BAD_ARG;
    if (!rccl().ok()) { g_create_error = rccl().err; return GCSADMM_ERR_HIP; }
    static_assert(sizeof(ncclUniqueId) == 128, "ncclUniqueId is 128 bytes");
    ncclUniqueId id;
    if (rccl().GetUniqueId(&id) != ncclSuccess) { g_create_error = "ncclGetUniqueId failed"; return GCSADMM_ERR_HIP; }
    std::memcpy(id128, &id, sizeof(id));
    return GCSADMM_OK;
}

gcsadmm_status gcsadmm_check_halo(gcsadmm_handle h, int32_t rank, int32_t world, const gcsadmm_halo_desc *halo)
{
    if (!h) return GCSADMM_ERR_BAD_ARG;
    if (h->halo.attached()) { h->err = "a communicator is already attached"; return GCSADMM_ERR_BAD_ARG; }
    return halo_validate(h, rank, world, halo);
}

gcsadmm_status gcsadmm_attach_comm(gcsadmm_handle h, int32_t rank, int32_t world, const void *id128, const gcsadmm_halo_desc *halo)
{
    gcsadmm_status st = gcsadmm_check_halo(h, rank, world, halo);
    if (st != GCSADMM_OK) return st;
    if (id128 && !rccl().ok()) { h->err = rccl().err; return GCSADMM_ERR_HIP; }
    USE_DEVICE(h);
    h->rank = rank; h->world = world;
    if ((st = halo_upload(h, halo)) != GCSADMM_OK) { h->halo = {}; return st; }
    if (id128) {
        ncclUniqueId id;
        std::memcpy(&id, id128, sizeof(id));
        ncclComm_t comm = nullptr;
        const ncclResult_t r = rccl().CommInitRank(&comm, world, id, rank);
        if (r != ncclSuccess) {
            h->err = std::string("ncclCommInitRank: ") + (rccl().GetErrorString ? rccl().GetErrorString(r) : "RCCL error");
            h->halo = {};
            return GCSADMM_ERR_HIP;
        }
        h->comm = comm;
    }
    return overlap_setup(h, h->halo.send_cols);
}

gcsadmm_status gcsadmm_halo_pack(gcsadmm_handle h, const gcsadmm_state *st, void *stream)
{
    if (!state_ok(h, st) || !h->halo.attached()) { if (h) h->err = "no halo attached"; return GCSADMM_ERR_BAD_ARG; }
    USE_DEVICE(h);
    return with_state(h, [&](auto t) { return halo_pack<decltype(t)>(h, st, (hipStream_t)stream); });
}
gcsadmm_status gcsadmm_halo_unpack(gcsadmm_handle h, const gcsadmm_state *st, void *stream)
{
    if (!state_ok(h, st) || !h->halo.attached()) { if (h) h->err = "no halo attached"; return GCSADMM_ERR_BAD_ARG; }
    USE_DEVICE(h);
    return with_state(h, [&](auto t) { return halo_unpack<decltype(t)>(h, st, (hipStream_t)stream); });
}
gcsadmm_status gcsadmm_halo_buffers(gcsadmm_handle h, void **send_buf, void **recv_buf, int64_t *num_elements)
{
    if (!h || !h->halo.attached()) { if (h) h->err = "no halo attached"; return GCSADMM_ERR_BAD_ARG; }
    if (send_buf) *send_buf = h->halo.d_sendbuf.get();
    if (recv_buf) *recv_buf = h->halo.d_recvbuf.get();
    if (num_elements) *num_elements = (int64_t)h->c * h->halo.n_send;
    return GCSADMM_OK;
}

gcsadmm_status gcsadmm_halo_exchange(gcsadmm_handle h, const gcsadmm_state *st, void *stream)
{
    if (!state_ok(h, st) || !h->halo.attached()) { if (h) h->err = "no halo attached"; return GCSADMM_ERR_BAD_ARG; }
    USE_DEVICE(h);
    hipStream_t s = (hipStream_t)stream;
    return with_state(h, [&](auto t) {
        using T = decltype(t);
        gcsadmm_status r;
        if ((r = halo_pack<T>(h, st, s)) != GCSADMM_OK) return r;
        if ((r = halo_transfer(h, s)) != GCSADMM_OK) return r;
        return halo_unpack<T>(h, st, s);
    });
}

static gcsadmm_status partitioned_tail(gcsadmm_handle h, const gcsadmm_state *st, double *trace_dev, hipStream_t s, const Event *ev)
{
    double *sums6 = h->halo.d_sums6.get();
    gcsadmm_status r = launch_edge(h, st, sums6, s, false, nullptr, true);
    if (r != GCSADMM_OK) return r;
    if (ev) HIPCHK(h, hipEventRecord(ev[0].get(), s));
    const double *reduced = sums6;
    if (h->comm) {
        NCCLCHK(h, rccl().AllReduce(sums6, sums6 + 6, 6, ncclFloat64, ncclSum, (ncclComm_t)h->comm, s));
        reduced = sums6 + 6;
    }
    if (ev) HIPCHK(h, hipEventRecord(ev[1].get(), s));
    hipLaunchKernelGGL(control_kernel, dim3(1), dim3(1), 0, s, h->loop.d_cb.get(), reduced, control_params(h), h->loop.d_counters.get(), trace_dev, true);
    HIPCHK(h, hipGetLastError());
    if (ev) HIPCHK(h, hipEventRecord(ev[2].get(), s));
    return GCSADMM_OK;
}

static gcsadmm_status run_partitioned_loop(gcsadmm_handle h, const gcsadmm_state *st, int k, double *trace_dev, hipStream_t s, const Event *ev)
{
    if (!h->comm && h->world > 1) { h->err = "gcsadmm_run_partitioned needs a communicator (gcsadmm_attach_comm with an id)"; return GCSADMM_ERR_BAD_ARG; }
    gcsadmm_status r;
    const Overlap &o = h->overlap;
    if (!ev && o.n_wave_b > 0 && h->overlap_mode != 2) {
        hipStream_t sc = o.comm_stream.get();
        for (int i = 0; i < k; ++i) {
            const bool reorder = ++h->vertex_steps % REORDER_EVERY == 0;
            HIPCHK(h, hipEventRecord(o.ev_boundary.get(), s));
            HIPCHK(h, hipStreamWaitEvent(sc, o.ev_boundary.get(), 0));
            if ((r = launch_vertex(h, st, sc, 0, reorder)) != GCSADMM_OK) return r;
            if ((r = gcsadmm_halo_exchange(h, st, (void *)sc)) != GCSADMM_OK) return r;
            HIPCHK(h, hipEventRecord(o.ev_halo.get(), sc));
            if ((r = launch_vertex(h, st, s, 1, reorder)) != GCSADMM_OK) return r;
            HIPCHK(h, hipStreamWaitEvent(s, o.ev_halo.get(), 0));
            if ((r = partitioned_tail(h, st, trace_dev, s, nullptr)) != GCSADMM_OK) return r;
        }
        HIPCHK(h, hipEventRecord(o.ev_halo.get(), sc));
        HIPCHK(h, hipStreamWaitEvent(s, o.ev_halo.get(), 0));
        return GCSADMM_OK;
    }
    for (int i = 0; i < k; ++i) {
        if (ev) HIPCHK(h, hipEventRecord(ev[6 * i + 0].get(), s));
        if ((r = gcsadmm_vertex_step(h, st, (void *)s)) != GCSADMM_OK) return r;
        if (ev) HIPCHK(h, hipEventRecord(ev[6 * i + 1].get(), s));
        if ((r = gcsadmm_halo_exchange(h, st, (void *)s)) != GCSADMM_OK) return r;
        if (ev) HIPCHK(h, hipEventRecord(ev[6 * i + 2].get(), s));
        if ((r = partitioned_tail(h, st, trace_dev, s, ev ? ev + 6 * i + 3 : nullptr)) != GCSADMM_OK) return r;
    }
    return GCSADMM_OK;
}

gcsadmm_status gcsadmm_run_partitioned(gcsadmm_handle h, const gcsadmm_state *st, int32_t k, double *trace_dev, void *stream)
{
    if (!state_ok(h, st) || k < 0) return GCSADMM_ERR_BAD_ARG;
    if (!h->halo.attached()) { h->err = "gcsadmm_attach_comm has not been called"; return GCSADMM_ERR_BAD_ARG; }
    USE_DEVICE(h);
    return run_partitioned_loop(h, st, k, trace_dev, (hipStream_t)stream, nullptr);
}

gcsadmm_status gcsadmm_run_partitioned_timed(gcsadmm_handle h, const gcsadmm_state *st, int32_t k, double *trace_dev, void *stream,
                                             float *vertex_ms, float *halo_ms, float *edge_ms, float *reduce_ms)
{
    if (!state_ok(h, st) || k < 0 || !vertex_ms || !halo_ms || !edge_ms || !reduce_ms) return GCSADMM_ERR_BAD_ARG;
    if (!h->halo.attached()) { h->err = "gcsadmm_attach_comm has not been called"; return GCSADMM_ERR_BAD_ARG; }
    USE_DEVICE(h);
    hipStream_t s = (hipStream_t)stream;
    gcsadmm_status r = ensure_events(h, (size_t)6 * k);
    if (r != GCSADMM_OK) return r;
    const std::vector<Event> &ev = h->events;
    if ((r = run_partitioned_loop(h, st, k, trace_dev, s, ev.data())) != GCSADMM_OK) return r;
    HIPCHK(h, hipStreamSynchronize(s));
    double acc[4] = {0, 0, 0, 0};
    for (int i = 0; i < k; ++i) {
        float t = 0;
        HIPCHK(h, hipEventElapsedTime(&t, ev[6 * i + 0].get(), ev[6 * i + 1].get())); acc[0] += t;
        HIPCHK(h, hipEventElapsedTime(&t, ev[6 * i + 1].get(), ev[6 * i + 2].get())); acc[1] += t;
        HIPCHK(h, hipEventElapsedTime(&t, ev[6 * i + 2].get(), ev[6 * i + 3].get())); acc[2] += t;
        HIPCHK(h, hipEventElapsedTime(&t, ev[6 * i + 3].get(), ev[6 * i + 5].get())); acc[3] += t;
    }
    *vertex_ms = (float)acc[0]; *halo_ms = (float)acc[1]; *edge_ms = (float)acc[2]; *reduce_ms = (float)acc[3];
    return GCSADMM_OK;
}

gcsadmm_status gcsadmm_set_overlap(gcsadmm_handle h, int32_t mode, int32_t *boundary_units)
{
    if (!h || mode < 0 || mode > 2) return GCSADMM_ERR_BAD_ARG;
    if (boundary_units) *boundary_units = 0;
    if (!h->halo.attached()) { h->err = "gcsadmm_attach_comm has not been called"; return GCSADMM_ERR_BAD_ARG; }
    USE_DEVICE(h);
    h->overlap_mode = mode;
    const gcsadmm_status r = overlap_setup(h, h->halo.send_cols);
    if (boundary_units) *boundary_units = h->overlap.n_wave_b;
    return r;
}

gcsadmm_status gcsadmm_comm_count(gcsadmm_handle h, int32_t *count)
{
    if (!h || !count) return GCSADMM_ERR_BAD_ARG;
    *count = 0;
    if (!h->comm) return GCSADMM_OK;
    if (!rccl().CommCount) { h->err = "librccl lacks ncclCommCount"; return GCSADMM_ERR_HIP; }
    USE_DEVICE(h);
    int n = 0;
    NCCLCHK(h, rccl().CommCount((ncclComm_t)h->comm, &n));
    *count = n;
    return GCSADMM_OK;
}

gcsadmm_status gcsadmm_vertex_prox(gcsadmm_handle h, const double *q_dev, const double *c_dev, double *xv_dev, double *zv_dev,
                                   double *yv_dev, double ipm_tol, int32_t ipm_max_iter, int32_t *failures_host, void *stream)
{
    if (!h || !q_dev || !c_dev || !xv_dev || !zv_dev || !yv_dev || !(ipm_tol > 0) || ipm_max_iter < 1) { if (h) h->err = "bad prox argument"; return GCSADMM_ERR_BAD_ARG; }
    if (h->plan.prox_lds_bytes > 160 * 1024) { h->err = "facet count too large for LDS"; return GCSADMM_ERR_UNSUPPORTED; }
    if (h->plan.n_term > 0) { h->err = "the prox kernel (v1 x-update) takes its terminals as points; this graph has a terminal that is a region"; return GCSADMM_ERR_UNSUPPORTED; }
    USE_DEVICE(h);
    hipStream_t s = (hipStream_t)stream;
    const auto &g = h->g;
    HIPCHK(h, h->prox.d_prox_counters.zero(s));
    WgLaunchDesc d{};
    d.n = h->n; d.dtype = GCSADMM_F64; d.n_vtx = (int)h->prox.d_prox_vtx.size(); d.lds_bytes = h->plan.prox_lds_bytes; d.vtx = h->prox.d_prox_vtx.get();
    StepDesc &p = d.step;
    p.inc_ptr = g.d_inc_ptr.get(); p.deg_in = g.d_deg_in.get(); p.inc_edge = g.d_inc_edge.get(); p.poly_ptr = g.d_poly_ptr.get();
    p.poly_A = g.d_poly_A.get(); p.poly_bc = g.d_poly_bc.get(); p.center = g.d_center.get();
    p.xv = xv_dev; p.zv = zv_dev; p.yv = yv_dev; p.counters = h->prox.d_prox_counters.get(); p.ipm_tol = ipm_tol; p.ipm_max_iter = ipm_max_iter;
    gcsadmm_wg_launch_prox(d, q_dev, c_dev, h->src, h->dst, s);
    HIPCHK(h, hipGetLastError());
    if (failures_host) {
        int cnt[2] = {0, 0};
        HIPCHK(h, hipMemcpyAsync(cnt, h->prox.d_prox_counters.get(), sizeof(cnt), hipMemcpyDeviceToHost, s));
        HIPCHK(h, hipStreamSynchronize(s));
        *failures_host = cnt[0];
    }
    return GCSADMM_OK;
}

gcsadmm_status gcsadmm_run_timed(gcsadmm_handle h, const gcsadmm_state *st, int32_t k, double *trace_dev, void *stream,
                                 float *vertex_ms, int32_t *vertex_launches, float *edge_ms, int32_t *edge_launches)
{
    if (!state_ok(h, st) || k < 0 || !vertex_ms || !edge_ms || !vertex_launches || !edge_launches) return GCSADMM_ERR_BAD_ARG;
    USE_DEVICE(h);
    hipStream_t s = (hipStream_t)stream;
    gcsadmm_status r = ensure_events(h, (size_t)4 * k);
    if (r != GCSADMM_OK) return r;
    const std::vector<Event> &ev = h->events;
    for (int i = 0; i < k; ++i) {
        HIPCHK(h, hipEventRecord(ev[4 * i + 0].get(), s));
        if ((r = gcsadmm_vertex_step(h, st, stream)) != GCSADMM_OK) return r;
        HIPCHK(h, hipEventRecord(ev[4 * i + 1].get(), s));
        HIPCHK(h, hipEventRecord(ev[4 * i + 2].get(), s));
        if ((r = launch_edge(h, st, h->loop.d_sums.get(), s, true, trace_dev)) != GCSADMM_OK) return r;
        HIPCHK(h, hipEventRecord(ev[4 * i + 3].get(), s));
    }
    HIPCHK(h, hipStreamSynchronize(s));
    double vm = 0, em = 0;
    for (int i = 0; i < k; ++i) {
        float t = 0;
        HIPCHK(h, hipEventElapsedTime(&t, ev[4 * i + 0].get(), ev[4 * i + 1].get())); vm += t;
        HIPCHK(h, hipEventElapsedTime(&t, ev[4 * i + 2].get(), ev[4 * i + 3].get())); em += t;
    }
    *vertex_ms = (float)vm; *edge_ms = (float)em; *vertex_launches = k; *edge_launches = k;
    return GCSADMM_OK;
}

gcsadmm_status gcsadmm_read_control(gcsadmm_handle h, gcsadmm_control_block *out, void *stream)
{
    if (!h || !out) return GCSADMM_ERR_BAD_ARG;
    USE_DEVICE(h);
    HIPCHK(h, hipMemcpyAsync(out, h->loop.d_cb.get(), sizeof(*out), hipMemcpyDeviceToHost, (hipStream_t)stream));
    HIPCHK(h, hipStreamSynchronize((hipStream_t)stream));
    return GCSADMM_OK;
}

gcsadmm_status gcsadmm_cost(gcsadmm_handle h, const gcsadmm_state *st, double eps_edge, double *cost_dev, void *stream)
{
    if (!h || !st || !st->zv || !st->zedge || !cost_dev) return GCSADMM_ERR_BAD_ARG;
    USE_DEVICE(h);
    with_state(h, [&](auto t) {
        using T = decltype(t);
        hipLaunchKernelGGL((cost_kernel<T>), dim3(1), dim3(256), 0, (hipStream_t)stream, h->V, h->E, h->n, st->zv,
                           (const T *)st->zedge, h->g.d_edge_counted.get(), eps_edge, cost_dev);
    });
    HIPCHK(h, hipGetLastError());
    return GCSADMM_OK;
}

#ifdef GCS_PHASE_TIMING
int gcsadmm_debug_sub_cycles(unsigned long long *out16)
{
    return (int)hipMemcpyFromSymbol(out16, HIP_SYMBOL(g_sub_cycles), 16 * sizeof(unsigned long long));
}

int gcsadmm_debug_phase_cycles(unsigned long long *out64)
{
    return (int)hipMemcpyFromSymbol(out64, HIP_SYMBOL(g_phase_cycles), 64 * sizeof(unsigned long long));
}
#endif

gcsadmm_status gcsadmm_query(gcsadmm_handle h, int32_t *num_waves, int32_t *lds_bytes, int32_t *num_special,
                             int32_t *num_workgroup_vertices, int32_t *workgroup_lds_bytes)
{
    if (!h) return GCSADMM_ERR_BAD_ARG;
    if (num_waves) *num_waves = h->plan.n_waves();
    if (lds_bytes) *lds_bytes = h->plan.lds_bytes;
    if (num_special) *num_special = h->n_special();
    if (num_workgroup_vertices) *num_workgroup_vertices = h->n_wg();
    if (workgroup_lds_bytes) *workgroup_lds_bytes = h->plan.wg_lds_bytes;
    return GCSADMM_OK;
}

gcsadmm_status gcsadmm_query_workspace(gcsadmm_handle h, int32_t *num_split_vertices, int32_t *split_lds_bytes, int64_t *workspace_bytes)
{
    if (!h) return GCSADMM_ERR_BAD_ARG;
    if (num_split_vertices) *num_split_vertices = h->n_split();
    if (split_lds_bytes) *split_lds_bytes = h->plan.split_lds_bytes;
    if (workspace_bytes) *workspace_bytes = (int64_t)((size_t)h->plan.split_doubles * sizeof(double));
    return GCSADMM_OK;
}

gcsadmm_status gcsadmm_unit_iterations(gcsadmm_handle h, int32_t *out, int32_t capacity, int32_t *count, void *stream)
{
    if (!h || !count) return GCSADMM_ERR_BAD_ARG;
    USE_DEVICE(h);
    const auto &g = h->g;
    const int *src = g.d_wave_iters ? g.d_wave_iters.get() : g.d_wg_iters.get();
    const int n = g.d_wave_iters ? h->plan.n_waves() : (g.d_wg_iters ? h->n_wg() : 0);
    *count = n;
    if (n == 0 || !out) return GCSADMM_OK;
    HIPCHK(h, hipStreamSynchronize((hipStream_t)stream));
    HIPCHK(h, hipMemcpy(out, src, sizeof(int) * (size_t)(n < capacity ? n : capacity), hipMemcpyDeviceToHost));
    return GCSADMM_OK;
}

const char *gcsadmm_batch_last_error(struct gcsadmm_batch_s *b) { return b ? b->err.c_str() : g_create_error.c_str(); }

void gcsadmm_batch_destroy(struct gcsadmm_batch_s *b)
{
    if (!b) return;
    DeviceGuard device_guard_(b->device);
    batch_unbind(b);
    for (gcsadmm_handle h : b->members)
        if (h) h->batches.erase(std::remove(h->batches.begin(), h->batches.end(), b), h->batches.end());
    delete b;
}

gcsadmm_status gcsadmm_batch_create(const gcsadmm_handle *members, int32_t count, struct gcsadmm_batch_s **out)
{
    if (out) *out = nullptr;
    auto fail = [&](gcsadmm_status st, const std::string &msg) { g_create_error = msg; return st; };
    if (!out) return fail(GCSADMM_ERR_BAD_ARG, "null output pointer");
    if (!members || count < 1) return fail(GCSADMM_ERR_BAD_ARG, "a batch needs at least one member");
    auto b = std::unique_ptr<gcsadmm_batch_s>(new (std::nothrow) gcsadmm_batch_s);
    if (!b) return fail(GCSADMM_ERR_HIP, "out of host memory");
    b->members.assign(members, members + count);
    std::string msg;
    const gcsadmm_status st = batch_plan_of(b->members, b->plan, msg);
    if (st != GCSADMM_OK) return fail(st, msg);
    b->device = b->plan.device;
    DeviceGuard device_guard_(b->device);
    hipError_t e = device_guard_.err;
    if (e == hipSuccess) e = b->d_vertex_table.alloc(gcsadmm_wg_batch_entry_bytes(b->plan.dtype) * (size_t)count);
    if (e == hipSuccess) e = b->d_edge_table.alloc((b->plan.dtype == GCSADMM_F64 ? sizeof(EdgeBatchEntry<double>) : sizeof(EdgeBatchEntry<float>)) * (size_t)count);
    if (e == hipSuccess) e = b->d_cbs.alloc((size_t)count);
    if (e == hipSuccess) e = b->d_poll.upload(nullptr, 2 * (size_t)count);
    if (e == hipSuccess && b->plan.vertex_lds_bytes > 48 * 1024) e = gcsadmm_wg_set_batch_lds(b->plan.n, b->plan.dtype, b->plan.vertex_lds_bytes);
    if (e != hipSuccess) return fail(GCSADMM_ERR_HIP, std::string("gcsadmm_batch_create: ") + hipGetErrorString(e));
    b->poll_host.resize(2 * (size_t)count);
    for (gcsadmm_handle h : b->members) h->batches.push_back(b.get());
    *out = b.release();
    return GCSADMM_OK;
}

gcsadmm_status gcsadmm_batch_bind(struct gcsadmm_batch_s *b, const gcsadmm_state *states, double *const *traces_dev, void *stream)
{
    if (!b) return GCSADMM_ERR_BAD_ARG;
    if (!states) { b->err = "null state array"; return GCSADMM_ERR_BAD_ARG; }
    const int count = (int)b->members.size();
    BatchPlan bp;
    gcsadmm_status st = batch_plan_of(b->members, bp, b->err);
    if (st != GCSADMM_OK) return st;
    for (int i = 0; i < count; ++i) {
        gcsadmm_handle h = b->members[i];
        const std::string who = "member " + std::to_string(i) + ": ";
        if (!state_ok(h, &states[i])) { b->err = who + h->err; return GCSADMM_ERR_BAD_ARG; }
        if (h->batch && h->batch != b) { b->err = who + "the handle is bound to another batch (destroy that batch, or bind it to other states, first)"; return GCSADMM_ERR_BAD_ARG; }
    }
    DeviceGuard device_guard_(b->device);
    HIPCHK(b, device_guard_.err);
    hipStream_t s = (hipStream_t)stream;
    HIPCHK(b, hipStreamSynchronize(s));
    batch_unbind(b);
    b->plan = bp;
    const size_t vbytes = gcsadmm_wg_batch_entry_bytes(bp.dtype);
    std::vector<char> vtab(vbytes * (size_t)count);
    std::vector<const gcsadmm_control_block *> cbs((size_t)count);
    b->resets.assign((size_t)count, 0u);
    for (int i = 0; i < count; ++i) {
        gcsadmm_handle h = b->members[i];
        gcsadmm_wg_batch_fill(make_wg_desc(h, &states[i], true), vtab.data() + vbytes * (size_t)i);
        cbs[i] = h->loop.d_cb.get();
        b->resets[i] = h->resets;
    }
    HIPCHK(b, hipMemcpy(b->d_vertex_table.get(), vtab.data(), vtab.size(), hipMemcpyHostToDevice));
    HIPCHK(b, hipMemcpy(b->d_cbs.get(), cbs.data(), sizeof(cbs[0]) * cbs.size(), hipMemcpyHostToDevice));
    const gcsadmm_status est = with_state_type(bp.dtype == GCSADMM_F64, [&](auto t) -> gcsadmm_status {
        using T = decltype(t);
        std::vector<EdgeBatchEntry<T>> etab((size_t)count);
        for (int i = 0; i < count; ++i) {
            gcsadmm_handle h = b->members[i];
            etab[i] = EdgeBatchEntry<T>{make_edge_args<T>(h, &states[i]), h->loop.d_cb.get(), h->loop.d_sums.get(), control_params(h), h->loop.d_counters.get(),
                                        traces_dev ? traces_dev[i] : nullptr, h->loop.d_ticket.get(), h->plan.edge_blocks};
        }
        HIPCHK(b, hipMemcpy(b->d_edge_table.get(), etab.data(), sizeof(etab[0]) * etab.size(), hipMemcpyHostToDevice));
        return GCSADMM_OK;
    });
    if (est != GCSADMM_OK) return est;
    for (gcsadmm_handle h : b->members) h->batch = b;
    b->bound = true;
    return GCSADMM_OK;
}

gcsadmm_status gcsadmm_batch_run(struct gcsadmm_batch_s *b, int32_t k, void *stream)
{
    if (!b || k < 0) return GCSADMM_ERR_BAD_ARG;
    if (!b->bound) { b->err = "gcsadmm_batch_bind has not been called"; return GCSADMM_ERR_BAD_ARG; }
    for (size_t i = 0; i < b->members.size(); ++i)
        if (b->members[i]->resets != b->resets[i]) {
            b->err = "member " + std::to_string(i) + ": gcsadmm_reset was called after gcsadmm_batch_bind (bind again: the tables hold the parameters)";
            return GCSADMM_ERR_BAD_ARG;
        }
    DeviceGuard device_guard_(b->device);
    HIPCHK(b, device_guard_.err);
    for (int i = 0; i < k; ++i) {
        const gcsadmm_status st = launch_batch_iteration(b, (hipStream_t)stream);
        if (st != GCSADMM_OK) return st;
    }
    return GCSADMM_OK;
}

gcsadmm_status gcsadmm_batch_poll(struct gcsadmm_batch_s *b, int32_t *status, int32_t *it, void *stream)
{
    if (!b) return GCSADMM_ERR_BAD_ARG;
    if (!b->bound) { b->err = "gcsadmm_batch_bind has not been called"; return GCSADMM_ERR_BAD_ARG; }
    DeviceGuard device_guard_(b->device);
    HIPCHK(b, device_guard_.err);
    hipStream_t s = (hipStream_t)stream;
    const int count = (int)b->members.size();
    hipLaunchKernelGGL(batch_poll_kernel, dim3((count + 255) / 256), dim3(256), 0, s, b->d_cbs.get(), count, b->d_poll.get());
    HIPCHK(b, hipGetLastError());
    HIPCHK(b, hipMemcpyAsync(b->poll_host.data(), b->d_poll.get(), sizeof(int) * 2 * (size_t)count, hipMemcpyDeviceToHost, s));
    HIPCHK(b, hipStreamSynchronize(s));
    for (int i = 0; i < count; ++i) {
        if (status) status[i] = b->poll_host[i];
        if (it) it[i] = b->poll_host[count + i];
    }
    return GCSADMM_OK;
}

}
```

gcs_admm_amd/csrc/step_args.h:

```cpp
#pragma once
#include <type_traits>

#include "gcs_math.h"

struct gcsadmm_control_block;

namespace gcsadmm_k {

constexpr int MAX_SPECIAL_DEG = 256;

struct StepArgsBase {
    const int *inc_ptr;
    const int *deg_in;
    const int *inc_edge;
    const int *poly_ptr;
    const double *poly_A;
    const double *poly_bc;
    const double *center;
    int E, NI;
    int edge_major = 0;
    double *xv, *zv, *yv;
    int *counters;
    double eps_edge, ipm_tol;
    int ipm_max_iter;
    double *warm = nullptr;
    const long long *warm_ptr = nullptr;
};

template <class T> struct StepArgs : StepArgsBase {
    const T *zedge, *mu;
    T *copy;
};

struct StepDesc : StepArgsBase {
    const void *zedge, *mu;
    void *copy;
    const gcsadmm_control_block *cb;
    template <class T> StepArgs<T> typed() const
    {
        StepArgs<T> a;
        static_cast<StepArgsBase &>(a) = *this;
        a.zedge = (const T *)zedge; a.mu = (const T *)mu; a.copy = (T *)copy;
        return a;
    }
};

GCS_HD int state_column(int edge_major, int E, int lo, int k, int edge, bool out) { return edge_major ? edge + (out ? 0 : E) : lo + k; }
template <class A> GCS_HD int state_column(const A &a, int lo, int k, int edge, bool out) { return state_column(a.edge_major, a.E, lo, k, edge, out); }
template <class A> GCS_HD int state_column(const A &a, int lo, int k, const int *edges, bool out)
{
    return state_column(a.edge_major, a.E, lo, k, a.edge_major ? edges[k] : 0, out);
}

template <class A> GCS_HD double consensus_target(const A &a, int w, int edge, int col, double mu_scale)
{
    return (double)a.zedge[(size_t)w * a.E + edge] - mu_scale * (double)a.mu[(size_t)w * a.NI + col];
}

template <int... Ns, class F> bool dispatch_dim(int n, F &&f)
{
    return ((n == Ns ? (f(std::integral_constant<int, Ns>()), true) : false) || ...);
}

template <class F> auto with_state_type(bool f64, F &&f) { return f64 ? f(double()) : f(float()); }

}
```

gcs_admm_amd/csrc/vertex_wg.h:

```cpp
#pragma once
#include <type_traits>

#include "gcs_math.h"
#include "step_args.h"
#include "warm_start.h"

#if defined(__HIP_DEVICE_COMPILE__)
#define WG_DEVICE 1
#else
#define WG_DEVICE 0
#endif

namespace gcs_wg {

using gcs_math::REG_DELTA;
using gcs_math::rcp;
using gcs_math::rcp1;
using gcs_math::rsqrt_nr;
using gcs_math::sqrt_nr;

#ifndef GCS_WG_THREADS
#define GCS_WG_THREADS 256
#endif
constexpr int WG_THREADS = GCS_WG_THREADS;
// ... 1154 lines not shown
            double acc2 = 0;
            if constexpr (BOX) {
                if (c == r) {
#pragma unroll 4
                    for (int u = 0; u <= d; ++u) acc2 += UN(u)[W::XD + r];
                }
            } else {
#pragma unroll 4
                for (int u = 0; u <= d; ++u) acc2 += UN(u)[W::X + r * NX + c];
            }
            sm[W::XS + tt] = acc2;
        }
        WG_FOR_AT(tt, 2 * NW, plq.at(2 * NW)) {
            const int s = tt / NW, k = tt - s * NW;
            double acc2 = UN(0)[W::P + k];
#pragma unroll 4
            for (int u = side_lo(s); u <= side_hi(s); ++u) acc2 -= UN(u)[W::P + k];
            sm[W::RP + tt] = acc2;
        }
        if (!first_warm) bg_tasks(plq);
        WG_ARRIVE(6);
        WG_SYNC();
        WG_STAMP(6);
        Place ply;
        if (sides) {
            WG_FIRST_WAVES(sd, 2) wave_ldl<NW>(sm + W::BS + sd * NW * NW, sm + W::PIVS + sd * NW);
            WG_ARRIVE(7);
            WG_SYNC();
            WG_STAMP(7);
            WG_FOR(t, 2 * NW) {
                const int s = t / NW, c = t - s * NW;
                ldl_inverse_col<NW, (!BOX && NW > 9)>(sm + W::BS + s * NW * NW, sm + W::PIVS + s * NW, c, sm + W::BSI + s * NW * NW, NW);
            }
            WG_SYNC();
            WG_FOR_AT(t, 2 * NW * NX, ply.at(2 * NW * NX)) {
                const int s = t / (NW * NX), ic = t - s * NW * NX, i = ic / NX, c = ic - i * NX;
                const double *Bsi = sm + W::BSI + s * NW * NW, *BXs = sm + W::BXS + s * NW * NX;
                double acc2 = 0;
#pragma unroll
                for (int k = 0; k < NW; ++k) acc2 += Bsi[i * NW + k] * BXs[k * NX + c];
                sm[W::BS + s * NW * NW + ic] = acc2;
            }
        } else {
            WG_FOR(t, 2 * NW * NW) { sm[W::BSI + t] = 0.0; sm[W::BS + t] = 0.0; }
            WG_SYNC();
        }
        if (!first_warm) v_tasks(ply);
        WG_ARRIVE(9);
        WG_SYNC();
        WG_STAMP(9);
        {
            const double *YS0 = sm + W::BS, *YS1 = sm + W::BS + NW * NW, *u0 = UN(0);
            auto x0 = [&](int i, int c) {
                if constexpr (BOX) return i == c ? u0[W::XD + c] : (i == 2 * N ? u0[W::XY + c] : 0.0);
                else return u0[W::X + i * NX + c];
            };
            auto k0 = [&](int hi, int lo) {
                if constexpr (BOX) return hi == lo ? (hi < 2 * N ? u0[W::KD + hi] : u0[W::KYY]) : (hi == 2 * N ? u0[W::KY + lo] : 0.0);
                else return u0[W::K + hi * NW + lo];
            };
            auto zx = [&](int i, int c) { return x0(i, c) + YS0[i * NX + c] + YS1[i * NX + c]; };
            auto zz = [&](int i, int k) {
                const int hi = i > k ? i : k, lo = i > k ? k : i;
                return k0(hi, lo) + sm[W::BSI + hi * NW + lo] + sm[W::BSI + NW * NW + hi * NW + lo];
            };
            Place plm;
            WG_FOR_AT(t, NX * (NX + 1) / 2, plm.at(NX * (NX + 1) / 2)) {
                int r, c;
                tri_decode(t, r, c);
                double val = (r == c ? REG_DELTA + (prox ? sm[W::PQ + r] : 0.0) : 0.0) - sm[W::XBX + r * NX + c] - sm[W::XBX + NX * NX + r * NX + c];
                if (r / N == c / N) val -= sm[W::XS + r * N + (c - (c / N) * N)];
#pragma unroll
                for (int k = 0; k < NW; ++k)
                    val += sm[W::BXS + k * NX + r] * YS0[k * NX + c] + sm[W::BXS + NW * NX + k * NX + r] * YS1[k * NX + c];
                sm[W::M + r * NB1 + c] = val;
            }
            WG_FOR_AT(t, NW * NX, plm.at(NW * NX)) {
                const int i = t / NX, c = t - i * NX;
                double val = zx(i, c);
                if (i >= N && i < 2 * N) val += zx(i - N, c);
                sm[W::M + (NX + i) * NB1 + c] = val;
            }
            WG_FOR_AT(t, NW * (NW + 1) / 2, plm.at(NW * (NW + 1) / 2)) {
                int i, k;
                tri_decode(t, i, k);
                const bool rz2 = i >= N && i < 2 * N, cz2 = k >= N && k < 2 * N;
                double val = zz(i, k);
                if (cz2) val += zz(i, k - N);
                if (rz2) val += zz(i - N, k);
                if (rz2 && cz2) val += zz(i - N, k - N);
                if (i < N && k < N) val += SOC[SO::SU + i * N + k];
                sm[W::M + (NX + i) * NB1 + NX + k] = val;
            }
            if (!first_warm) rhs_tasks(plm, false);
        }
        WG_ARRIVE(10);
        WG_SYNC();
        WG_STAMP(10);
        WG_WAVE0() wave_ldl<NB1>(sm + W::M, sm + W::PIVM);
        WG_ARRIVE(11);
        WG_SYNC();
        WG_STAMP(11);
        WG_STAMP(12);
        double rmax = 0.0, c1 = 0.0, c2 = 0.0, amax_cone = 1e300;
        double sigmu;
        if (first_warm) {
            Place plb;
            WG_ROWS_BEGIN(plb)
                un[oR1 + ro] = 0.0;
                un[oR2 + ro] = rcp1(s);
            WG_ROWS_END()
            WG_FOR_AT(u, U, plb.at(U)) { double *un = UN(u); un[W::KB] = 0.0; un[W::KB + 1] = 0.0; }
            sigmu = mu_ref;
            WG_ARRIVE(14);
            WG_SYNC();
            WG_STAMP(14);
        } else {
        solve_tail(SC_DTA, false);
        WG_STAMP(13);
        Place plb;
        WG_ROWS_BEGIN_DS(plb)
            const double l = un[oLAM + ro], is = rcp1(s);
            const double q = ds * is, dl = -l - l * q;
            rmax = fmax(rmax, fmax(-q, 1.0 + q));
            c1 += s * dl + l * ds; c2 += ds * dl;
            un[oR1 + ro] = ds * dl;
            un[oR2 + ro] = is;
        WG_ROWS_END()
        WG_FOR_AT(u, U, plb.at(U)) {
            double *un = UN(u);
            const double yy = un[W::P + 2 * N], dy = un[W::DW + 2 * N];
            const double s5 = yy, s6 = 1.0 - yy, l5 = un[W::LB], l6 = un[W::LB + 1];
            const double q5 = dy * rcp1(s5), q6 = -dy * rcp1(s6);
            const double dl5 = -l5 - l5 * q5, dl6 = -l6 - l6 * q6;
            rmax = fmax(rmax, fmax(fmax(-q5, 1.0 + q5), fmax(-q6, 1.0 + q6)));
            c1 += s5 * dl5 + l5 * dy + s6 * dl6 - l6 * dy; c2 += dy * dl5 - dy * dl6;
            un[W::KB] = dy * dl5; un[W::KB + 1] = -dy * dl6;
        }
        WG_CONE() { amax_cone = fmin(SC[SC_AMAXC], SC[SC_AMAXC2]); c1 += SC[SC_C1C]; c2 += SC[SC_C2C]; }
        WG_ARRIVE(14);
        const Red3 rb = wg_reduce<WG_VM>(Red3{fmin(rmax > 0.0 ? rcp1(rmax) : 1e300, amax_cone), c1, c2}, sm + W::RED, red_phase);
        WG_STAMP(14);
        {
            const double al = fmin(1.0, rb.mn);
            const double mu_aff = (gap + al * rb.s1 + al * al * rb.s2) * inv_deg;
            sigmu = wg_uniform(gcs_math::centring(mu_aff * rcp(mu)) * mu);
        }
        }
        WG_CONE() {
            double wb[Q], a1[Q], a2[Q], pr[Q], qv[Q], xs[Q], lt[Q], ss[Q];
            const double eta = SC[SC_ETA];
#pragma unroll
            for (int k = 0; k < Q; ++k) { wb[k] = SOC[SO::WB + k]; xs[k] = SOC[SO::DSSA + k]; lt[k] = SOC[SO::LT + k]; ss[k] = SOC[SO::SS + k]; }
            soc_apply_Wi<Q>(wb, eta, xs, a1);
#pragma unroll
            for (int k = 0; k < Q; ++k) xs[k] = SOC[SO::DLSA + k];
            soc_apply_W<Q>(wb, eta, xs, a2);
            double dsum = 0;
#pragma unroll
            for (int k = 0; k < Q; ++k) dsum += a1[k] * a2[k];
            pr[0] = dsum;
#pragma unroll
            for (int k = 1; k < Q; ++k) pr[k] = a1[0] * a2[k] + a2[0] * a1[k];
            const double det = gcs_math::soc_det<Q>(lt);
            double ld1 = 0;
#pragma unroll
            for (int k = 1; k < Q; ++k) ld1 += lt[k] * pr[k];
            qv[0] = (lt[0] * pr[0] - ld1) * rcp(det);
            const double ilt0 = rcp(lt[0]);
#pragma unroll
            for (int k = 1; k < Q; ++k) qv[k] = (pr[k] - qv[0] * lt[k]) * ilt0;
            const double smd = sigmu * rcp(gcs_math::soc_det<Q>(ss));
            soc_apply_Wi<Q>(wb, eta, qv, a1);
#pragma unroll
            for (int i = 0; i < Q; ++i) SOC[SO::KS + i] = smd * (i == 0 ? ss[0] : -ss[i]) - (first_warm ? 0.0 : a1[i]);
            SC[SC_GT] = 1.0 - SOC[SO::KS];
        }
        Place plg;
        WG_FOR_AT(t, U * 2 * N, plg.at(U * 2 * N)) {
            const int u = t / (2 * N), q = t - u * (2 * N), i = q / N, k = q - i * N;
            double *un = UN(u);
            const double *ea = un + oR1, *eb = ea + m2, *ia = un + oR2, *ib = ia + m2;
            double su = 0, sx = 0;
            if constexpr (BOX) {
                const int jp = i * m + k, jn = jp + N;
                const double kbp = (sigmu - eb[jp]) * ib[jp], kbn = (sigmu - eb[jn]) * ib[jn];
                su = ((sigmu - ea[jp]) * ia[jp] - kbp) - ((sigmu - ea[jn]) * ia[jn] - kbn);
                sx = kbp - kbn;
            } else {
#pragma unroll 4
                for (int j = 0; j < m; ++j) {
                    const double kb = (sigmu - eb[i * m + j]) * ib[i * m + j], aj = A[j * N + k];
                    su += aj * ((sigmu - ea[i * m + j]) * ia[i * m + j] - kb);
                    sx += aj * kb;
                }
            }
            un[W::GU + q] = su;
            un[W::GX + q] = sx;
        }
        WG_FOR_AT(u, U, plg.at(U)) {
            double *un = UN(u);
            const double *ea = un + oR1, *eb = ea + m2, *ia = un + oR2, *ib = ia + m2;
            double s = 0;
#pragma unroll 4
            for (int j = 0; j < m2; ++j) s += BC[j >= m ? j - m : j] * ((sigmu - eb[j]) * ib[j] - (sigmu - ea[j]) * ia[j]);
            const double yy = un[W::P + 2 * N];
            un[W::GU + 2 * N] = s - (sigmu - un[W::KB]) * rcp1(yy) + (sigmu - un[W::KB + 1]) * rcp1(1.0 - yy);
        }
        WG_ARRIVE(16);
        WG_SYNC();
        WG_STAMP(16);
        solve_head(true);
        solve_tail(SC_DT, true);
        WG_STAMP(18);
        rmax = 0.0;
        Place pld;
        WG_ROWS_BEGIN_DS(pld)
            const double l = un[oLAM + ro];
            const double ip = rcp1(s * l), is = l * ip, il = s * ip;
            const double dl = (sigmu - un[oR1 + ro]) * un[oR2 + ro] - l - (l * is) * ds;
            un[oR2 + ro] = dl;
            rmax = fmax(rmax, fmax(-ds * is, -dl * il));
        WG_ROWS_END()
        WG_FOR_AT(u, U, pld.at(U)) {
            double *un = UN(u);
            const double yy = un[W::P + 2 * N], dy = un[W::DW + 2 * N];
            const double s5 = yy, s6 = 1.0 - yy, l5 = un[W::LB], l6 = un[W::LB + 1];
            const double i5 = rcp1(s5), i6 = rcp1(s6);
            const double dl5 = (sigmu - un[W::KB]) * i5 - l5 - l5 * i5 * dy, dl6 = (sigmu - un[W::KB + 1]) * i6 - l6 + l6 * i6 * dy;
            un[W::DLB] = dl5; un[W::DLB + 1] = dl6;
            rmax = fmax(rmax, fmax(fmax(-dy * i5, -dl5 * rcp1(l5)), fmax(dy * i6, -dl6 * rcp1(l6))));
        }
        amax_cone = 1e300;
        WG_CONE() amax_cone = fmin(SC[SC_AMAXC], SC[SC_AMAXC2]);
        WG_ARRIVE(19);
        const Red3 rd = wg_reduce<WG_VM>(Red3{fmin(rmax > 0.0 ? rcp1(rmax) : 1e300, amax_cone), 0.0, 0.0}, sm + W::RED, red_phase);
        WG_STAMP(19);
        WG_CONE() {
            double al = gcs_math::step_length(rd.mn);
            for (int tries = 0; tries < 40; ++tries) {
                double s2[Q], l2[Q];
#pragma unroll
                for (int k = 0; k < Q; ++k) { s2[k] = SOC[SO::SS + k] + al * SOC[SO::DSS + k]; l2[k] = SOC[SO::LS + k] + al * SOC[SO::DLS + k]; }
                if (gcs_math::soc_interior<Q>(s2) && gcs_math::soc_interior<Q>(l2)) break;
                al *= 0.7;
            }
            SC[SC_ALPHA] = al;
        }
        WG_ARRIVE(20);
        WG_SYNC();
        WG_STAMP(20);
        const double alpha = wg_uniform(SC[SC_ALPHA]);
        stalled = gcs_math::step_stalled(alpha);
        Place plu;
        WG_ROWS_BEGIN(plu)
            (void)s;
            un[oLAM + ro] += alpha * un[oR2 + ro];
        WG_ROWS_END()
        WG_FOR_AT(t, U * NW, plu.at(U * NW)) {
            const int u = t / NW, k = t - u * NW;
            double *un = UN(u);
            un[W::P + k] += alpha * un[W::DW + k];
        }
        WG_FOR_AT(t, 2 * U, plu.at(2 * U)) {
            double *un = UN(t >> 1);
            un[W::LB + (t & 1)] += alpha * un[W::DLB + (t & 1)];
        }
        WG_FOR_AT(t, NX + 2 * NW, plu.at(NX + 2 * NW)) {
            if (t < NX) sm[W::XV + t] += alpha * sm[W::DX + t];
            else sm[W::NU + (t - NX)] += alpha * sm[W::DNU + (t - NX)];
        }
        WG_CONE() {
            SC[SC_T] += alpha * SC[SC_DT];
            for (int k = 0; k < Q; ++k) SOC[SO::LS + k] += alpha * SOC[SO::DLS + k];
        }
        WG_ARRIVE(21);
        WG_SYNC();
        WG_STAMP(21);
    }
#undef WG_FAIL_OR_RESTART
    it_total += it;
    if (wrec != nullptr) {
        WG_ONE() {
            if (status != 0) wrec[0] = 0.0;
            else gcs_ws::ws_learn(wrec, use_warm, ws_started_warm && !use_warm, ws_dT, it);
        }
    }
    status_out = status;
    iters_out = it_total;
    WG_STAMP(22);
    WG_SYNC();
    if (status != 0) return;
    Place plo;
    WG_FOR_AT(t, d * NW, plo.at(d * NW)) {
        const int e = t / NW, w = t - e * NW;
        const bool out = e >= d_in;
        const int inc = gcsadmm_k::state_column(a, lo, e, a.inc_edge + lo, out);
        const double *un = UN(e + 1), *p = un + W::P;
        const double yy = p[2 * N];
        double val;
        if (w == 2 * N) val = yy;
        else if (w < N) val = out ? p[w] + yy * CEN[w] : un[W::TF + w];
        else val = out ? p[w] + yy * CEN[w - N] : p[w - N] + yy * CEN[w - N];
        a.copy[(size_t)w * a.NI + inc] = (T)val;
    }
    WG_FOR_AT(k, NX, plo.at(NX)) {
        const int c = k < N ? k : k - N;
        const double *u0 = UN(0);
        a.xv[(size_t)v * NX + k] = sm[W::XV + k] + CEN[c];
        a.zv[(size_t)v * NX + k] = u0[W::P + k] + u0[W::P + 2 * N] * CEN[c];
    }
    WG_ONE() a.yv[v] = UN(0)[W::P + 2 * N];
}

}
```

gcs_admm_amd/csrc/vertex_wg_kernel.h:

```cpp
#pragma once
#include <hip/hip_runtime.h>

#include <algorithm>

#include "special_vertex.h"
#include "vertex_wg.h"
#include "vertex_wg_launch.h"

namespace {

using namespace gcsadmm_k;
using gcs_wg::WG_THREADS;

#ifdef GCS_WG_TIMING
#define GCS_WG_MIN_BLOCKS 1
#else
#define GCS_WG_MIN_BLOCKS (gcs_wg::WG_THREADS <= 256 ? 2 : 1)
#endif
#if defined(GCS_WG_TIMING) && !defined(GCS_WG_BLOCKTIME)
#define GCS_WG_BLOCKTIME 1
#endif
#ifdef GCS_WG_BLOCKTIME
__device__ unsigned long long g_wg_block_ticks[64], g_wg_block_iters[64];
#endif
template <int N, bool BOX> constexpr int wg_min_blocks() { return GCS_WG_MIN_BLOCKS == 1 ? 1 : (N <= 3 ? 4 : 2); }
template <int N, class T, bool BOX>
__device__ __forceinline__ void vertex_wg_body(const gcs_wg::WgArgs<T> &a, const SpecialArgs &sp, double rho, double mu_scale, int bx, double *smem)
{
    if (bx >= a.n_vtx) {
        const int i = (bx - a.n_vtx) * WG_THREADS + (int)threadIdx.x;
        if (i < sp.count) {
            double *vals = smem + (sp.kind[i] == 2 ? 2 * MAX_SPECIAL_DEG : 0);
            special_body<N, T>(a, sp, i, rho, mu_scale, vals, vals + MAX_SPECIAL_DEG);
        }
        return;
    }
    int status = 0, iters = 0;
#ifdef GCS_WG_BLOCKTIME
    const unsigned long long t_begin = __builtin_amdgcn_s_memtime();
#endif
    const int slot = a.order ? a.order[bx] : bx;
    gcs_wg::wg_solve_vertex<N, T, BOX>(a, a.vtx[slot], rho, mu_scale, smem, status, iters);
    if (threadIdx.x == 0) {
        if (status != 0) atomicAdd(&a.counters[0], 1);
        atomicAdd(&a.counters[1], iters);
        if (a.unit_iters) a.unit_iters[slot] = iters;
#ifdef GCS_WG_BLOCKTIME
        if (bx < 64) {
            g_wg_block_ticks[bx] += __builtin_amdgcn_s_memtime() - t_begin;
            g_wg_block_iters[bx] += (unsigned long long)iters;
        }
#endif
    }
}

template <int N, class T, bool BOX>
__global__ __launch_bounds__(WG_THREADS, (wg_min_blocks<N, BOX>())) void vertex_wg_kernel(gcs_wg::WgArgs<T> a, SpecialArgs sp, const gcsadmm_control_block *cb)
{
    extern __shared__ __attribute__((aligned(16))) double smem[];
    if (cb->status != GCSADMM_RUNNING) return;
    vertex_wg_body<N, T, BOX>(a, sp, cb->rho, cb->mu_scale, (int)blockIdx.x, smem);
}

#if GCS_WG_THREADS == 256
template <class T> struct WgBatchEntry {
    gcs_wg::WgArgs<T> a;
    SpecialArgs sp;
    const gcsadmm_control_block *cb;
    int grid_x;
};
template <int N, class T, bool BOX>
__global__ __launch_bounds__(WG_THREADS, (wg_min_blocks<N, BOX>())) void vertex_wg_batch_kernel(const WgBatchEntry<T> *__restrict__ table)
{
    extern __shared__ __attribute__((aligned(16))) double smem[];
    __builtin_assume_dereferenceable(table + blockIdx.y, sizeof(WgBatchEntry<T>));
    const WgBatchEntry<T> e = *(const WgBatchEntry<T> *)((const __attribute__((address_space(4))) WgBatchEntry<T> *)table + blockIdx.y);
    if ((int)blockIdx.x >= e.grid_x || e.cb->status != GCSADMM_RUNNING) return;
    vertex_wg_body<N, T, BOX>(e.a, e.sp, e.cb->rho, e.cb->mu_scale, (int)blockIdx.x, smem);
}
#endif

template <int N, bool BOX> constexpr int wg_split_min_blocks() { return N >= 7 ? 1 : wg_min_blocks<N, BOX>(); }
template <int N, class T, bool BOX>
__global__ __launch_bounds__(WG_THREADS, (wg_split_min_blocks<N, BOX>())) void vertex_wg_split_kernel(gcs_wg::WgArgs<T> a, WgSplitArgs w,
                                                                                              const gcsadmm_control_block *cb)
{
    extern __shared__ __attribute__((aligned(16))) double smem[];
    if (cb->status != GCSADMM_RUNNING) return;
    int status = 0, iters = 0;
    gcs_wg::wg_solve_vertex<N, T, BOX, true>(a, a.vtx[blockIdx.x], cb->rho, cb->mu_scale, smem, status, iters, w.units + w.unit_off[blockIdx.x]);
    if (threadIdx.x == 0) {
        if (status != 0) atomicAdd(&a.counters[0], 1);
        atomicAdd(&a.counters[1], iters);
    }
}

struct InLdsKernels { template <int N, class T, bool BOX> static constexpr auto kernel() { return vertex_wg_kernel<N, T, BOX>; } };
struct SplitKernels { template <int N, class T, bool BOX> static constexpr auto kernel() { return vertex_wg_split_kernel<N, T, BOX>; } };
#if GCS_WG_THREADS == 256
struct BatchKernels { template <int N, class T, bool BOX> static constexpr auto kernel() { return vertex_wg_batch_kernel<N, T, BOX>; } };
#endif
template <int N> constexpr bool WG_HAS_BOX = N == 3 || N == 6;
template <class F> auto with_state(int dtype, F &&f) { return with_state_type(dtype == GCSADMM_F64, f); }

template <class K, int N, class T, class X>
void launch_kernels(const WgLaunchDesc &d, const gcs_wg::WgArgs<T> &a, unsigned grid, int lds, const X &extra, hipStream_t s)
{
    if constexpr (WG_HAS_BOX<N>) {
        if (d.box) { hipLaunchKernelGGL((K::template kernel<N, T, true>()), dim3(grid), dim3(WG_THREADS), lds, s, a, extra, d.step.cb); return; }
    }
    hipLaunchKernelGGL((K::template kernel<N, T, false>()), dim3(grid), dim3(WG_THREADS), lds, s, a, extra, d.step.cb);
}

template <class K, int N> hipError_t set_lds(int dtype, int lds_bytes)
{
    return with_state(dtype, [&](auto t) {
        using T = decltype(t);
        hipError_t e = hipFuncSetAttribute((const void *)K::template kernel<N, T, false>(), hipFuncAttributeMaxDynamicSharedMemorySize, lds_bytes);
        if constexpr (WG_HAS_BOX<N>)
            if (e == hipSuccess) e = hipFuncSetAttribute((const void *)K::template kernel<N, T, true>(), hipFuncAttributeMaxDynamicSharedMemorySize, lds_bytes);
        return e;
    });
}

template <class T> gcs_wg::WgArgs<T> in_lds_args(const WgLaunchDesc &d)
{
    gcs_wg::WgArgs<T> a;
    static_cast<StepArgs<T> &>(a) = d.step.typed<T>();
    a.n_vtx = d.n_vtx; a.vtx = d.vtx; a.order = d.order; a.unit_iters = d.unit_iters;
    return a;
}

template <int N> void launch(const WgLaunchDesc &d, hipStream_t s)
{
    with_state(d.dtype, [&](auto t) {
        using T = decltype(t);
        const gcs_wg::WgArgs<T> a = in_lds_args<T>(d);
        const SpecialArgs sp{d.n_special, d.special_vtx, d.special_kind};
        const unsigned grid = (unsigned)(d.n_vtx + (d.n_special + WG_THREADS - 1) / WG_THREADS);
        if (grid == 0) return;
        const int lds = std::max(d.lds_bytes, (int)(4 * MAX_SPECIAL_DEG * sizeof(double)));
        launch_kernels<InLdsKernels, N, T>(d, a, grid, lds, sp, s);
    });
}

#if GCS_WG_THREADS == 256
template <int N> void launch_batch(const WgBatchLaunch &b, hipStream_t s)
{
    with_state(b.dtype, [&](auto t) {
        using T = decltype(t);
        const auto *table = (const WgBatchEntry<T> *)b.table;
        if constexpr (WG_HAS_BOX<N>) {
            if (b.box) { hipLaunchKernelGGL((vertex_wg_batch_kernel<N, T, true>), dim3(b.grid_x, b.count), dim3(WG_THREADS), b.lds_bytes, s, table); return; }
        }
        hipLaunchKernelGGL((vertex_wg_batch_kernel<N, T, false>), dim3(b.grid_x, b.count), dim3(WG_THREADS), b.lds_bytes, s, table);
    });
}
#endif

template <int N> void launch_split(const WgLaunchDesc &d, const WgSplitArgs &w, hipStream_t s)
{
    if (d.n_vtx <= 0) return;
    with_state(d.dtype, [&](auto t) {
        using T = decltype(t);
        gcs_wg::WgArgs<T> a;
        static_cast<StepArgs<T> &>(a) = d.step.typed<T>();
        a.n_vtx = d.n_vtx; a.vtx = d.vtx;
        launch_kernels<SplitKernels, N, T>(d, a, (unsigned)d.n_vtx, d.lds_bytes, w, s);
    });
}

template <int N>
__global__ __launch_bounds__(WG_THREADS, 2) void vertex_prox_kernel(gcs_wg::WgArgs<double> a, int src, int dst)
{
    extern __shared__ __attribute__((aligned(16))) double smem[];
    constexpr int NX = 2 * N, NU = 4 * N + 1;
    if ((int)blockIdx.x >= a.n_vtx) {
        const int t = (int)threadIdx.x;
        const int v = t == 0 ? src : (t == 1 ? dst : -1);
        if (v < 0) return;
        const double *q = a.prox_q + (size_t)v * NU, *c = a.prox_c + (size_t)v * NU;
        double num = q[2 * NX] * c[2 * NX], den = q[2 * NX];
        for (int k = 0; k < NX; ++k) {
            const double pt = a.center[(size_t)v * N + (k < N ? k : k - N)];
            num += q[NX + k] * pt * c[NX + k];
            den += q[NX + k] * pt * pt;
        }
        double y = den > 0.0 ? num / den : 0.5;
        y = y < 0.0 ? 0.0 : (y > 1.0 ? 1.0 : y);
        for (int k = 0; k < NX; ++k) {
            const double pt = a.center[(size_t)v * N + (k < N ? k : k - N)];
            a.xv[(size_t)v * NX + k] = pt;
            a.zv[(size_t)v * NX + k] = y * pt;
        }
        a.yv[v] = y;
        return;
    }
    int status = 0, iters = 0;
    gcs_wg::wg_solve_vertex<N, double>(a, a.vtx[blockIdx.x], 1.0, 1.0, smem, status, iters);
    if (threadIdx.x == 0 && a.counters) {
        if (status != 0) atomicAdd(&a.counters[0], 1);
        atomicAdd(&a.counters[1], iters);
    }
}

template <int N> void launch_prox(const WgLaunchDesc &d, const double *q, const double *c, int src, int dst, hipStream_t s)
{
    gcs_wg::WgArgs<double> a{};
    static_cast<StepArgs<double> &>(a) = d.step.typed<double>();
    a.n_vtx = d.n_vtx; a.vtx = d.vtx; a.prox_q = q; a.prox_c = c;
    if (d.lds_bytes > 48 * 1024)
        (void)hipFuncSetAttribute((const void *)vertex_prox_kernel<N>, hipFuncAttributeMaxDynamicSharedMemorySize, d.lds_bytes);
    hipLaunchKernelGGL((vertex_prox_kernel<N>), dim3(d.n_vtx + 1), dim3(WG_THREADS), d.lds_bytes, s, a, src, dst);
}

}
```

gcs_admm_amd/csrc/vertex_wg_launch.h:

```cpp
#pragma once
#include <hip/hip_runtime.h>

#include "gcsadmm.h"
#include "step_args.h"

namespace gcsadmm_k {

struct WgLaunchDesc {
    StepDesc step;
    int n, dtype;
    int n_vtx, n_special, lds_bytes;
    const int *vtx;
    const int *special_vtx, *special_kind;
    int box;
    const int *order;
    int *unit_iters;
};

struct WgSplitArgs {
    double *units;
    const long long *unit_off;
};

struct WgBatchLaunch {
    int n, dtype, box;
    const void *table;
    unsigned grid_x, count;
    int lds_bytes;
};

}

hipError_t gcsadmm_wg_set_lds(int n, int dtype, int lds_bytes);
void gcsadmm_wg_launch(const gcsadmm_k::WgLaunchDesc &d, hipStream_t s);

hipError_t gcsadmm_wg_set_lds_t512(int n, int dtype, int lds_bytes);
void gcsadmm_wg_launch_t512(const gcsadmm_k::WgLaunchDesc &d, hipStream_t s);

hipError_t gcsadmm_wg_set_split_lds(int n, int dtype, int lds_bytes);
void gcsadmm_wg_launch_split(const gcsadmm_k::WgLaunchDesc &d, const gcsadmm_k::WgSplitArgs &w, hipStream_t s);

size_t gcsadmm_wg_batch_entry_bytes(int dtype);
int gcsadmm_wg_batch_fill(const gcsadmm_k::WgLaunchDesc &d, void *entry_host);
hipError_t gcsadmm_wg_set_batch_lds(int n, int dtype, int lds_bytes);
void gcsadmm_wg_launch_batch(const gcsadmm_k::WgBatchLaunch &b, hipStream_t s);

void gcsadmm_wg_launch_prox(const gcsadmm_k::WgLaunchDesc &d, const double *q, const double *c, int src, int dst, hipStream_t s);
```

gcs_admm_amd/solver.py:

```python
from __future__ import annotations

import contextlib
import ctypes as C
import time
from typing import Optional

import numpy as np

from . import abi
from .abi import (CONVERGED, DIVERGED, EXPORTS, F32, F64, LIB_PATH, MAX_IT, RUNNING, STATUS_NAME,
                  ControlBlock, GcsAdmmError, GraphDesc, HaloDesc, Params, State)
from .graph import GcsGraph


def load_library() -> C.CDLL:
    return abi.load_library(LIB_PATH)


def halo_arrays(send_idx, recv_idx):
    peers = sorted(send_idx)
    if sorted(recv_idx) != peers:
        raise ValueError("a partition sends to and receives from the same neighbours")
    cnt = [len(send_idx[r]) for r in peers]
    if cnt != [len(recv_idx[r]) for r in peers]:
        raise ValueError("send and receive lists of a neighbour must be equally long")
    ptr = np.zeros(len(peers) + 1, np.int32); ptr[1:] = np.cumsum(cnt)
    cat = lambda d: (np.concatenate([np.asarray(d[r], np.int32) for r in peers]) if peers else np.zeros(0, np.int32))
    return np.asarray(peers, np.int32), ptr, np.ascontiguousarray(cat(send_idx)), np.ascontiguousarray(cat(recv_idx))


class DeviceSolver:

    def __init__(self, graph: GcsGraph, state_dtype: str = "f64", device: Optional[int] = None,
                 num_incidences: Optional[int] = None, inc_counted=None, edge_counted=None,
                 nx_global: float = 0.0, nmu_global: float = 0.0, program: str = "auto", wave_slots: int = 0,
                 wave_align: int = 0, wave_store_dl: int = 0, wave_generic_rows: int = 0, columns: str = "incidence",
                 vertex_workspace: int = 0):
        import torch
        if not torch.cuda.is_available():
            raise RuntimeError("no HIP device visible: the ADMM loop only runs on the GPU (no CPU fallback)")
        self.torch = torch
        self.lib = load_library()
        self.g = g = graph
        self.device_index = torch.cuda.current_device() if device is None else int(device)
        self.device = torch.device("cuda", self.device_index)
        self.dtype_code = {"f64": F64, "f32": F32}[state_dtype]
        self.tdtype = torch.float64 if state_dtype == "f64" else torch.float32
        desc, self._keep, self.col_of = abi.graph_desc(
            g, state_dtype=self.dtype_code, device=self.device_index, num_incidences=num_incidences, inc_counted=inc_counted,
            edge_counted=edge_counted, nx_global=nx_global, nmu_global=nmu_global, columns=columns,
            vertex_program={"auto": 0, "wavefront": 1, "workgroup": 2, "workgroup256": 3}[program], wave_slots=wave_slots,
            wave_align=wave_align, wave_store_dl=wave_store_dl, wave_generic_rows=wave_generic_rows, vertex_workspace=vertex_workspace)
        self.NI, self.edge_major = desc.num_incidences, columns == "edge"
        h = C.c_void_p()
        self._call("gcsadmm_create", C.byref(desc), C.byref(h), handle=False, select=False)
        self.h = h
        c, E, V, n = g.c, g.num_edges, g.num_vertices, g.n
        z = lambda *s, dt=self.tdtype: torch.zeros(*s, dtype=dt, device=self.device)
        self.copy, self.mu, self.zedge = z(c, max(self.NI, 1)), z(c, max(self.NI, 1)), z(c, max(E, 1))
        self.xv, self.zv, self.yv = z(V, 2 * n, dt=torch.float64), z(V, 2 * n, dt=torch.float64), z(V, dt=torch.float64)
        self.sums = z(5, dt=torch.float64)
        self._cost = z(1, dt=torch.float64)
        self.state = State(self.copy.data_ptr(), self.mu.data_ptr(), self.zedge.data_ptr(),
                           self.xv.data_ptr(), self.zv.data_ptr(), self.yv.data_ptr())
        self.params = None
        self.trace = None

    def _call(self, name, *args, handle=True, select=True):
        h = self.h if handle else None
        with self.torch.cuda.device(self.device) if select else contextlib.nullcontext():
            st = getattr(self.lib, name)(*((h,) if handle else ()), *args)
        abi.check(st, lambda: f"{name} failed ({st}): {self.lib.gcsadmm_last_error(h).decode()}")

    def _stream(self):
        return self.torch.cuda.current_stream(self.device).cuda_stream

    def close(self):
        if getattr(self, "h", None):
            self._call("gcsadmm_destroy", select=False)
            self.h = None

    def __del__(self):
        try:
            self.close()
        except Exception:
            pass

    def reset(self, rho=1.0, tau_incr=2.0, tau_decr=2.0, nu=10.0, it_rho_limit=100, max_it=1000, eps_abs=1e-4,
              eps_rel=1e-3, eps_edge=1e-4, ipm_tol=None, ipm_max_iter=60, zero_state=True, cold_start=False):
        if ipm_tol is None:
            from . import IPM_TOL as ipm_tol
        self.params = Params(rho, tau_incr, tau_decr, nu, it_rho_limit, max_it, eps_abs, eps_rel, eps_edge,
                             ipm_tol, ipm_max_iter, 1 if cold_start else 0)
        if zero_state:
            for t in (self.copy, self.mu, self.zedge, self.xv, self.zv, self.yv):
                t.zero_()
        self.trace = self.torch.zeros(max_it, 6, dtype=self.torch.float64, device=self.device)
        self._call("gcsadmm_reset", C.byref(self.params), self._stream())

    def vertex_step(self):
        self._call("gcsadmm_vertex_step", C.byref(self.state), self._stream())

    def edge_step(self):
        self._call("gcsadmm_edge_step", C.byref(self.state), self.sums.data_ptr(), self._stream())
        return self.sums

    def control(self, sums=None):
        s = self.sums if sums is None else sums
        self._call("gcsadmm_control", s.data_ptr(), self.trace.data_ptr(), self._stream())

    def enqueue(self, k: int):
        self._call("gcsadmm_run", C.byref(self.state), int(k), self.trace.data_ptr(), self._stream())

    def enqueue_timed(self, k: int):
        vm, em = C.c_float(0), C.c_float(0)
        vl, el = C.c_int32(0), C.c_int32(0)
        self._call("gcsadmm_run_timed", C.byref(self.state), int(k), self.trace.data_ptr(), self._stream(),
                   C.byref(vm), C.byref(vl), C.byref(em), C.byref(el))
        return dict(vertex_ms=vm.value, vertex_launches=vl.value, edge_ms=em.value, edge_launches=el.value)

    def vertex_prox(self, q, c, ipm_tol: float = 1e-10, ipm_max_iter: int = 60):
        torch = self.torch
        V, n = self.g.num_vertices, self.g.n
        qd = torch.as_tensor(np.ascontiguousarray(q, dtype=np.float64), device=self.device)
        cd = torch.as_tensor(np.ascontiguousarray(c, dtype=np.float64), device=self.device)
        assert qd.shape == (V, 4 * n + 1) and cd.shape == qd.shape
        xv = torch.zeros(V, 2 * n, dtype=torch.float64, device=self.device); zv = torch.zeros_like(xv)
        yv = torch.zeros(V, dtype=torch.float64, device=self.device)
        fails = C.c_int32(0)
        self._call("gcsadmm_vertex_prox", qd.data_ptr(), cd.data_ptr(), xv.data_ptr(), zv.data_ptr(), yv.data_ptr(),
                   float(ipm_tol), int(ipm_max_iter), C.byref(fails), self._stream(), select=False)
        return xv, zv, yv, fails.value

    def unique_id(self) -> bytes:
        buf = (C.c_ubyte * 128)()
        self._call("gcsadmm_comm_unique_id", buf, handle=False, select=False)
        return bytes(buf)

    def _halo_desc(self, send_idx, recv_idx):
        peers, ptr, sc, rc = halo_arrays(send_idx, recv_idx)
        if self.edge_major:
            sc = np.ascontiguousarray(self.col_of[sc].astype(np.int32)); rc = np.ascontiguousarray(self.col_of[rc].astype(np.int32))
        self._halo_keep = (peers, ptr, sc, rc)
        return HaloDesc(len(peers), peers.ctypes.data, ptr.ctypes.data, sc.ctypes.data, ptr.ctypes.data, rc.ctypes.data)

    def check_halo(self, rank: int, world: int, send_idx, recv_idx):
        self._call("gcsadmm_check_halo", int(rank), int(world), C.byref(self._halo_desc(send_idx, recv_idx)), select=False)

    def attach_comm(self, rank: int, world: int, unique_id, send_idx, recv_idx):
        idb = (C.c_ubyte * 128).from_buffer_copy(unique_id) if unique_id is not None else None
        self._call("gcsadmm_attach_comm", int(rank), int(world), idb, C.byref(self._halo_desc(send_idx, recv_idx)))
        self.has_comm = unique_id is not None

    def enqueue_partitioned(self, k: int):
        self._call("gcsadmm_run_partitioned", C.byref(self.state), int(k), self.trace.data_ptr(), self._stream())

    def enqueue_partitioned_timed(self, k: int):
        v, hl, e, r = (C.c_float(0) for _ in range(4))
        self._call("gcsadmm_run_partitioned_timed", C.byref(self.state), int(k), self.trace.data_ptr(), self._stream(),
                   C.byref(v), C.byref(hl), C.byref(e), C.byref(r))
        return dict(vertex_ms=v.value, halo_ms=hl.value, edge_ms=e.value, reduce_ms=r.value)

    def set_overlap(self, mode: int = 0) -> int:
        n = C.c_int32(0)
        self._call("gcsadmm_set_overlap", int(mode), C.byref(n))
        return n.value

    def comm_count(self) -> int:
        n = C.c_int32(0)
        self._call("gcsadmm_comm_count", C.byref(n), select=False)
        return n.value

    def halo_pack(self):
        self._call("gcsadmm_halo_pack", C.byref(self.state), self._stream(), select=False)

    def halo_unpack(self):
        self._call("gcsadmm_halo_unpack", C.byref(self.state), self._stream(), select=False)

    def halo_exchange(self):
        self._call("gcsadmm_halo_exchange", C.byref(self.state), self._stream(), select=False)

    def halo_buffers(self):
        a, b, n = C.c_void_p(), C.c_void_p(), C.c_int64(0)
        self._call("gcsadmm_halo_buffers", C.byref(a), C.byref(b), C.byref(n), select=False)
        return a.value, b.value, n.value

    def read_control(self) -> ControlBlock:
        cb = ControlBlock()
        self._call("gcsadmm_read_control", C.byref(cb), self._stream(), select=False)
        return cb

    def query(self):
        a, b, c, d, e = (C.c_int32(0) for _ in range(5))
        self._call("gcsadmm_query", C.byref(a), C.byref(b), C.byref(c), C.byref(d), C.byref(e), select=False)
        return dict(num_waves=a.value, lds_bytes=b.value, num_special=c.value, num_workgroup_vertices=d.value,
                    workgroup_lds_bytes=e.value)

    def query_workspace(self):
        a, b, c = C.c_int32(0), C.c_int32(0), C.c_int64(0)
        self._call("gcsadmm_query_workspace", C.byref(a), C.byref(b), C.byref(c), select=False)
        return dict(num_split_vertices=a.value, split_lds_bytes=b.value, workspace_bytes=c.value)

    def unit_iterations(self):
        n = C.c_int32(0)
        self._call("gcsadmm_unit_iterations", None, 0, C.byref(n), self._stream())
        out = np.zeros(n.value, np.int32)
        if n.value:
            self._call("gcsadmm_unit_iterations", out.ctypes.data, n.value, C.byref(n), self._stream())
        return out

    def cost(self) -> float:
        eps = self.params.eps_edge if self.params is not None else 1e-4
        self._call("gcsadmm_cost", C.byref(self.state), eps, self._cost.data_ptr(), self._stream(), select=False)
        return float(self._cost.item())

    def _loop(self, enqueue, chunk, params, clock=False):
        self.reset(**params)
        max_it, done, dev_ms = self.params.max_it, 0, 0.0
        if clock:
            self.torch.cuda.synchronize(self.device)
        t0 = time.perf_counter()
        while True:
            k = min(chunk, max_it - done)
            if k > 0:
                dev_ms += enqueue(k) or 0.0
                done += k
            cb = self.read_control()
            if cb.status != RUNNING or done >= max_it:
                return cb, time.perf_counter() - t0, dev_ms

    def solve_partitioned(self, chunk: int = 25, **params):
        return self._loop(self.enqueue_partitioned, chunk, params)[0]

    def solve(self, chunk: int = 25, timed: bool = False, **params):
        def enqueue_timed(k):
            tm = self.enqueue_timed(k)
            return tm["vertex_ms"] + tm["edge_ms"]
        cb, wall, dev_ms = self._loop(enqueue_timed if timed else self.enqueue, chunk, params, clock=True)
        return self.record(cb, wall, dev_ms * 1e-3 if timed else None)

    def record(self, cb, wall_time_s, device_time_s=None):
        tr = self.trace[:min(cb.it, self.params.max_it)].cpu().numpy()
        return dict(iterations=int(cb.it), status=STATUS_NAME[cb.status],
                    rho_seq=np.concatenate([[self.params.rho], tr[:, 0]]),
                    pri_res_seq=np.concatenate([[0.0], tr[:, 1]]),
                    dual_res_seq=np.concatenate([[0.0], tr[:, 2]]),
                    eps_pri_seq=tr[:, 3], eps_dual_seq=tr[:, 4],
                    inner_failures=int(tr[:, 5].sum()), cost=self.cost(),
                    wall_time_s=wall_time_s, device_time_s=device_time_s)
```

include/gcsadmm.h:

```cpp
#ifndef GCSADMM_H
#define GCSADMM_H

#include <stdint.h>

#ifdef __cplusplus
extern "C" {
#endif

typedef enum gcsadmm_status {
    GCSADMM_OK = 0,
    GCSADMM_ERR_BAD_ARG = 1,
    GCSADMM_ERR_UNSUPPORTED = 2,
    GCSADMM_ERR_HIP = 3,
    GCSADMM_ERR_NO_DEVICE = 4,
    GCSADMM_ERR_NO_MEMORY = 5
} gcsadmm_status;

enum { GCSADMM_F64 = 0, GCSADMM_F32 = 1 };

enum { GCSADMM_RUNNING = -1, GCSADMM_CONVERGED = 0, GCSADMM_MAX_IT = 1, GCSADMM_DIVERGED = 2 };

typedef struct gcsadmm_graph_desc {
    int32_t n;
    int32_t num_vertices;
    int32_t num_edges;
    int32_t num_incidences;
    const int32_t *inc_ptr;
    const int32_t *inc_edge;
    const int32_t *inc_out;
    const int32_t *edge_inc_tail;
    const int32_t *edge_inc_head;
    const int32_t *poly_ptr;
    const double *poly_A;
    const double *poly_b;
    const double *center;
    int32_t src, dst;
    int32_t state_dtype;
    int32_t device;
    const uint8_t *inc_counted;
    const uint8_t *edge_counted;
    double nx_global, nmu_global;
    int32_t vertex_program;
    int32_t wave_slots;
    int32_t wave_align;
    int32_t wave_store_dl;
    int32_t wave_generic_rows;
    int32_t edge_major_columns;
    int32_t vertex_workspace;
} gcsadmm_graph_desc;

typedef struct gcsadmm_params {
    double rho;
    double tau_incr;
    double tau_decr;
    double nu;
    int32_t it_rho_limit;
    int32_t max_it;
    double eps_abs;
    double eps_rel;
    double eps_edge;
    double ipm_tol;
    int32_t ipm_max_iter;
    int32_t cold_start;
} gcsadmm_params;

typedef struct gcsadmm_state {
    void *copy;
    void *mu;
    void *zedge;
    double *xv;
    double *zv;
    double *yv;
} gcsadmm_state;

typedef struct gcsadmm_control_block {
    double rho;
    double mu_scale;
    double sums[5];
    double pri, dual, eps_pri, eps_dual;
    int32_t it;
    int32_t status;
    int32_t inner_failures;
    int32_t inner_iters;
} gcsadmm_control_block;

typedef struct gcsadmm_handle_s *gcsadmm_handle;

gcsadmm_status gcsadmm_create(const gcsadmm_graph_desc *desc, gcsadmm_handle *out);
void gcsadmm_destroy(gcsadmm_handle h);
const char *gcsadmm_last_error(gcsadmm_handle h);

gcsadmm_status gcsadmm_reset(gcsadmm_handle h, const gcsadmm_params *p, void *stream);

gcsadmm_status gcsadmm_vertex_step(gcsadmm_handle h, const gcsadmm_state *st, void *stream);

gcsadmm_status gcsadmm_edge_step(gcsadmm_handle h, const gcsadmm_state *st, double *sums_dev, void *stream);

gcsadmm_status gcsadmm_control(gcsadmm_handle h, const double *sums_dev, double *trace_dev, void *stream);

gcsadmm_status gcsadmm_run(gcsadmm_handle h, const gcsadmm_state *st, int32_t k, double *trace_dev, void *stream);

gcsadmm_status gcsadmm_read_control(gcsadmm_handle h, gcsadmm_control_block *out, void *stream);

gcsadmm_status gcsadmm_cost(gcsadmm_handle h, const gcsadmm_state *st, double eps_edge, double *cost_dev, void *stream);

gcsadmm_status gcsadmm_query(gcsadmm_handle h, int32_t *num_waves, int32_t *lds_bytes, int32_t *num_special,
                             int32_t *num_workgroup_vertices, int32_t *workgroup_lds_bytes);

gcsadmm_status gcsadmm_query_workspace(gcsadmm_handle h, int32_t *num_split_vertices, int32_t *split_lds_bytes, int64_t *workspace_bytes);

gcsadmm_status gcsadmm_unit_iterations(gcsadmm_handle h, int32_t *out, int32_t capacity, int32_t *count, void *stream);

gcsadmm_status gcsadmm_run_timed(gcsadmm_handle h, const gcsadmm_state *st, int32_t k, double *trace_dev,
                                 void *stream, float *vertex_ms, int32_t *vertex_launches,
                                 float *edge_ms, int32_t *edge_launches);

typedef struct gcsadmm_batch_s gcsadmm_batch_s;

gcsadmm_status gcsadmm_batch_create(const gcsadmm_handle *members, int32_t count, struct gcsadmm_batch_s **out);
void gcsadmm_batch_destroy(struct gcsadmm_batch_s *b);
const char *gcsadmm_batch_last_error(struct gcsadmm_batch_s *b);

gcsadmm_status gcsadmm_batch_bind(struct gcsadmm_batch_s *b, const gcsadmm_state *states, double *const *traces_dev, void *stream);

gcsadmm_status gcsadmm_batch_run(struct gcsadmm_batch_s *b, int32_t k, void *stream);

gcsadmm_status gcsadmm_batch_poll(struct gcsadmm_batch_s *b, int32_t *status, int32_t *it, void *stream);

gcsadmm_status gcsadmm_vertex_prox(gcsadmm_handle h, const double *q_dev, const double *c_dev, double *xv_dev, double *zv_dev,
                                   double *yv_dev, double ipm_tol, int32_t ipm_max_iter, int32_t *failures_host, void *stream);

typedef struct gcsadmm_halo_desc {
    int32_t num_peers;
    const int32_t *peer_rank;
    const int32_t *send_ptr;
    const int32_t *send_cols;
    const int32_t *recv_ptr;
    const int32_t *recv_cols;
} gcsadmm_halo_desc;

gcsadmm_status gcsadmm_comm_unique_id(void *id128);

gcsadmm_status gcsadmm_attach_comm(gcsadmm_handle h, int32_t rank, int32_t world, const void *id128, const gcsadmm_halo_desc *halo);
gcsadmm_status gcsadmm_check_halo(gcsadmm_handle h, int32_t rank, int32_t world, const gcsadmm_halo_desc *halo);

gcsadmm_status gcsadmm_run_partitioned(gcsadmm_handle h, const gcsadmm_state *st, int32_t k, double *trace_dev, void *stream);

gcsadmm_status gcsadmm_run_partitioned_timed(gcsadmm_handle h, const gcsadmm_state *st, int32_t k, double *trace_dev, void *stream,
                                             float *vertex_ms, float *halo_ms, float *edge_ms, float *reduce_ms);

gcsadmm_status gcsadmm_set_overlap(gcsadmm_handle h, int32_t mode, int32_t *boundary_units);

gcsadmm_status gcsadmm_comm_count(gcsadmm_handle h, int32_t *count);

gcsadmm_status gcsadmm_halo_pack(gcsadmm_handle h, const gcsadmm_state *st, void *stream);
gcsadmm_status gcsadmm_halo_unpack(gcsadmm_handle h, const gcsadmm_state *st, void *stream);
gcsadmm_status gcsadmm_halo_exchange(gcsadmm_handle h, const gcsadmm_state *st, void *stream);
gcsadmm_status gcsadmm_halo_buffers(gcsadmm_handle h, void **send_buf, void **recv_buf, int64_t *num_elements);

const char *gcsadmm_polytope_last_error(void);

int gcsadmm_polytope_centers(int n, int num_polytopes, const int *poly_ptr, const double *poly_A, const double *poly_b,
                             int device, double *centers, double *radii, int *status);

int gcsadmm_polytope_bounds(int n, int num_polytopes, const int *poly_ptr, const double *poly_A, const double *poly_b,
                            const double *centers, int device, double *lo, double *hi, int *status);

int gcsadmm_polytope_overlaps(int n, int num_polytopes, const int *poly_ptr, const double *poly_A, const double *poly_b,
                              const double *centers, long num_pairs, const int *pair_a, const int *pair_b, double tol,
                              int device, unsigned char *overlap, int *status);

typedef struct gcsadmm_scene_s *gcsadmm_scene;

int gcsadmm_scene_create(int n, int num_polytopes, const int *poly_ptr, const double *poly_A, const double *poly_b, int device,
                         gcsadmm_scene *out);
void gcsadmm_scene_destroy(gcsadmm_scene s);

int gcsadmm_scene_centers(gcsadmm_scene s, double *centers, double *radii, int *status);

int gcsadmm_scene_bounds(gcsadmm_scene s, double *lo, double *hi, int *status);

int gcsadmm_scene_set_boxes(gcsadmm_scene s, const double *lo, const double *hi);

int gcsadmm_scene_candidate_pairs(gcsadmm_scene s, double pad, int64_t *num_pairs);

int gcsadmm_scene_overlaps(gcsadmm_scene s, double tol, int64_t *num_overlapping, int64_t *num_undecided);

int gcsadmm_scene_read_pairs(gcsadmm_scene s, int *pair_a, int *pair_b, unsigned char *overlap, int *status);

int gcsadmm_scene_restrict_paths(gcsadmm_scene s, int num_paths, const int *path_ptr, const int *path_poly, const double *start, double tol,
                                 int max_iter, double *points, double *cost, int *iterations, int *status);

int gcsadmm_scene_locate_points(gcsadmm_scene s, int num_points, const double *points, double eps, double tol, int64_t *num_hits);

int gcsadmm_scene_read_hits(gcsadmm_scene s, int64_t *hit_ptr, int *hit_region, unsigned char *hit_class);

#ifdef __cplusplus
}
#endif
#endif
```

Before: 9796 iterations/s.

## Fuse single-block edge step and control into the vertex workgroup kernel tail

For small graphs where the edge step fits in one block (E <= EDGE_BLOCK, no waves, no split or terminal vertices, not partitioned), the last vertex workgroup to finish, chosen by an atomic ticket, runs the edge update, the residual reduction and the control logic. This removes the separate edge and control kernel launches each iteration. Copy stores become agent-scope atomic stores so the tail block can see them, and the tail arguments are read from the kernarg segment at a fixed offset. The added release fences and atomics may cost a little, and the offset trick relies on the assumed kernarg layout.

```diff
diff --git a/gcs_admm_amd/abi.py b/gcs_admm_amd/abi.py
--- a/gcs_admm_amd/abi.py
+++ b/gcs_admm_amd/abi.py
@@ -59,6 +59,7 @@
     "gcsadmm_edge_step": ([_p] * 4, _i),
     "gcsadmm_control": ([_p] * 4, _i),
     "gcsadmm_run": (_run, _i),
+    "gcsadmm_set_fused_tail": ([_p, _i], _i),
     "gcsadmm_read_control": ([_p] * 3, _i),
     "gcsadmm_cost": ([_p, _p, _d, _p, _p], _i),
     "gcsadmm_query": ([_p] * 6, _i),
diff --git a/gcs_admm_amd/build.py b/gcs_admm_amd/build.py
--- a/gcs_admm_amd/build.py
+++ b/gcs_admm_amd/build.py
@@ -18,9 +18,9 @@
          (LP, "polytope_lp.o", []), (TERM, "terminal_region.o", [])]
 HDR = os.path.join(ROOT, "include", "gcsadmm.h")
 _c = lambda *names: [os.path.join(CSRC, f) for f in names]
-DEPS = [MAIN, HDR] + _c("vertex_program.h", "vertex_program.inc", "vertex_kernel.h", "special_vertex.h", "vertex_wg_launch.h", "canonical_box.h", "create_plan.h", "batch_plan.h", "warm_start.h", "terminal_launch.h", "step_args.h", "gcs_math.h", "hip_owners.h")
+DEPS = [MAIN, HDR] + _c("vertex_program.h", "vertex_program.inc", "vertex_kernel.h", "special_vertex.h", "vertex_wg_launch.h", "canonical_box.h", "create_plan.h", "batch_plan.h", "warm_start.h", "terminal_launch.h", "step_args.h", "gcs_math.h", "hip_owners.h", "edge_step.h")
 UNIT_DEPS = {LP: [LP, HDR] + _c("polytope_lp_core.h", "box_sweep_core.h", "point_locate_core.h", "path_restrict_core.h", "restrict_plan.h", "hip_owners.h", "step_args.h", "gcs_math.h"),
-             WG: [WG, HDR] + _c("vertex_wg.h", "vertex_wg_kernel.h", "vertex_wg_launch.h", "special_vertex.h", "gcs_math.h", "warm_start.h", "step_args.h")}
+             WG: [WG, HDR] + _c("vertex_wg.h", "vertex_wg_kernel.h", "vertex_wg_launch.h", "special_vertex.h", "gcs_math.h", "warm_start.h", "step_args.h", "edge_step.h")}
 UNIT_DEPS[WGD] = [WGD] + UNIT_DEPS[WG][1:]
 UNIT_DEPS[TERM] = [TERM, HDR] + _c("terminal_region.h", "terminal_launch.h", "gcs_math.h", "warm_start.h", "step_args.h")
 OUT = os.path.join(HERE, "libgcsadmm.so")
diff --git a/gcs_admm_amd/csrc/create_plan.h b/gcs_admm_amd/csrc/create_plan.h
--- a/gcs_admm_amd/csrc/create_plan.h
+++ b/gcs_admm_amd/csrc/create_plan.h
@@ -18,7 +18,6 @@
 
 namespace gcsadmm_k {
 
-constexpr int EDGE_BLOCK = 256;
 constexpr int REORDER_MIN_UNITS = 512;
 constexpr int LDS_CU_BYTES = 160 * 1024;
 
@@ -53,6 +52,7 @@
     std::vector<int> col_vertex;
     double nx = 0, nmu = 0;
     int edge_unroll = 1, edge_blocks = 1;
+    int fused_tail = 0;
     int n_waves() const { return (int)wave_slot_ptr.size() - 1; }
 };
 
@@ -259,6 +259,8 @@
     p.edge_unroll = edge_unroll_rt(g.state_dtype, 2 * n + 1, E);
     const int tile = EDGE_BLOCK * p.edge_unroll;
     p.edge_blocks = std::max(1, std::min((E + tile - 1) / tile, 2048));
+    const bool partitioned = g.num_incidences > g.inc_ptr[V] || g.inc_counted != nullptr || g.edge_counted != nullptr;
+    p.fused_tail = p.edge_blocks == 1 && E <= EDGE_BLOCK && p.n_waves() == 0 && p.split_vtx.empty() && p.n_term == 0 && !p.wg_vtx.empty() && !partitioned;
     return GCSADMM_OK;
 }
 
diff --git a/gcs_admm_amd/csrc/edge_step.h b/gcs_admm_amd/csrc/edge_step.h
--- /dev/null
+++ b/gcs_admm_amd/csrc/edge_step.h
@@ -0,0 +1,249 @@
+#pragma once
+#include <hip/hip_runtime.h>
+
+#include <cstdint>
+
+#include "gcsadmm.h"
+#include "step_args.h"
+
+namespace gcsadmm_k {
+
+constexpr int EDGE_WAVE = 64;
+
+template <class T> struct EdgeArgs {
+    int E, NI, c;
+    const int *edge_inc_tail, *edge_inc_head;
+    const uint8_t *inc_counted, *edge_counted;
+    const T *copy;
+    T *zedge, *mu;
+    double *partials;
+};
+
+__device__ __forceinline__ double wave_sum(double v)
+{
+#pragma unroll
+    for (int off = 32; off > 0; off >>= 1) v += __shfl_down(v, off, 64);
+    return v;
+}
+
+__device__ __forceinline__ double scaled_plus(double scale, double x, double r)
+{
+#pragma clang fp contract(off)
+    return scale * x + r;
+}
+
+struct ControlParams {
+    double tau_incr, tau_decr, nu, eps_abs, eps_rel, nx, nmu;
+    int it_rho_limit, max_it;
+};
+
+struct EdgeInKernel {
+    static constexpr bool TAIL = false;
+    template <class T> static __device__ __forceinline__ T load_copy(const T *p) { return *p; }
+    static __device__ __forceinline__ int load_counter(const int *p) { return *p; }
+    static __device__ __forceinline__ void store_counter(int *p, int v) { *p = v; }
+    static __device__ __forceinline__ bool edge_thread() { return true; }
+    static __device__ __forceinline__ void sync() { __syncthreads(); }
+};
+struct EdgeInTail {
+    static constexpr bool TAIL = true;
+    template <class T> static __device__ __forceinline__ T load_copy(const T *p) { return __hip_atomic_load(p, __ATOMIC_RELAXED, __HIP_MEMORY_SCOPE_AGENT); }
+    static __device__ __forceinline__ int load_counter(const int *p) { return __hip_atomic_load(p, __ATOMIC_RELAXED, __HIP_MEMORY_SCOPE_AGENT); }
+    static __device__ __forceinline__ void store_counter(int *p, int v) { __hip_atomic_store(p, v, __ATOMIC_RELAXED, __HIP_MEMORY_SCOPE_AGENT); }
+    static __device__ __forceinline__ bool edge_thread() { return threadIdx.x < (unsigned)EDGE_BLOCK; }
+    static __device__ __forceinline__ void sync() { __syncthreads(); }
+};
+
+struct EdgePre {
+    int it = 0, ih = 0;
+    double mu_scale = 1.0;
+};
+template <class T> __device__ __forceinline__ EdgePre edge_prefetch(const EdgeArgs<T> &a, double mu_scale)
+{
+    EdgePre p;
+    p.mu_scale = mu_scale;
+    if (threadIdx.x < (unsigned)EDGE_BLOCK && a.E > 0) {
+        const int e = (int)threadIdx.x, ee = e < a.E ? e : a.E - 1;
+        p.it = a.edge_inc_tail ? a.edge_inc_tail[ee] : ee; p.ih = a.edge_inc_head ? a.edge_inc_head[ee] : a.E + ee;
+    }
+    return p;
+}
+
+template <class P = EdgeInKernel>
+__device__ void control_body(gcsadmm_control_block *cb, const double *sums, const ControlParams &p, int *counters, double *trace,
+                             bool global_fails = false)
+{
+    if (cb->status != GCSADMM_RUNNING) return;
+    double s[5];
+    for (int k = 0; k < 5; ++k) { s[k] = sums[k]; cb->sums[k] = s[k]; }
+    const int it = cb->it;
+    double rho = cb->rho;
+    const int fails = global_fails ? (int)(sums[5] + 0.5) : P::load_counter(&counters[0]), iters = P::load_counter(&counters[1]);
+    P::store_counter(&counters[0], 0); P::store_counter(&counters[1], 0);
+    cb->inner_failures = fails; cb->inner_iters = iters;
+    const double tot = s[0] + s[1] + s[2] + s[3] + s[4];
+    if (!(fabs(tot) <= 1.7976931348623157e308)) {
+        cb->status = GCSADMM_DIVERGED;
+        return;
+    }
+    const double pri = sqrt(s[0]), dual = rho * sqrt(2.0 * s[1]);
+    double mu_scale = 1.0;
+    if (pri >= p.nu * dual && it < p.it_rho_limit) { rho *= p.tau_incr; mu_scale = 1.0 / p.tau_incr; }
+    else if (dual >= p.nu * pri && it < p.it_rho_limit) { rho *= 1.0 / p.tau_decr; mu_scale = p.tau_incr; }
+    const double eps_pri = sqrt(p.nx) * p.eps_abs + p.eps_rel * fmax(sqrt(s[2]), sqrt(2.0 * s[3]));
+    const double eps_dual = sqrt(p.nmu) * p.eps_abs + p.eps_rel * mu_scale * sqrt(s[4]);
+    cb->rho = rho; cb->mu_scale = mu_scale;
+    cb->pri = pri; cb->dual = dual; cb->eps_pri = eps_pri; cb->eps_dual = eps_dual;
+    if (trace) {
+        double *tr = trace + (size_t)(it - 1) * 6;
+        tr[0] = rho; tr[1] = pri; tr[2] = dual; tr[3] = eps_pri; tr[4] = eps_dual; tr[5] = (double)fails;
+    }
+    if (pri < eps_pri && dual < eps_dual) { cb->status = GCSADMM_CONVERGED; return; }
+    cb->it = it + 1;
+    if (it + 1 > p.max_it) cb->status = GCSADMM_MAX_IT;
+}
+
+template <class T, int C> __host__ __device__ constexpr int edge_unroll() { return sizeof(T) == 4 ? (C <= 7 ? 4 : 2) : (C <= 7 ? 2 : 1); }
+
+template <class T>
+__device__ __forceinline__ void edge_word(const EdgeArgs<T> &a, int w, int e, int it, int ih, T cu_t, T cw_t, T zo_t, T mu_t, T mw_t, double mu_scale,
+                                          double we, double wt, double wh, double (&s)[5])
+{
+    const double cu = (double)cu_t, cw = (double)cw_t, zo = (double)zo_t;
+    const T zn_t = (T)(0.5 * (cu + cw));
+    const double zn = (double)zn_t;
+    const double ru = cu - zn, rw = cw - zn;
+    const T mu_u_t = (T)scaled_plus(mu_scale, (double)mu_t, ru);
+    const T mu_w_t = (T)scaled_plus(mu_scale, (double)mw_t, rw);
+    a.mu[(size_t)w * a.NI + it] = mu_u_t;
+    a.mu[(size_t)w * a.NI + ih] = mu_w_t;
+    a.zedge[(size_t)w * a.E + e] = zn_t;
+    const double mu_u = (double)mu_u_t, mu_w = (double)mu_w_t;
+    s[0] += wt * ru * ru + wh * rw * rw;
+    s[1] += we * (zn - zo) * (zn - zo);
+    s[2] += wt * cu * cu + wh * cw * cw;
+    s[3] += we * zn * zn;
+    s[4] += wt * mu_u * mu_u + wh * mu_w * mu_w;
+}
+
+#ifndef GCS_TAIL_WORDS
+#define GCS_TAIL_WORDS 5
+#endif
+template <class T, int C> __host__ __device__ constexpr int tail_words() { return C < GCS_TAIL_WORDS ? C : GCS_TAIL_WORDS; }
+
+template <class T, int MODE, int C, int U, class P = EdgeInKernel>
+__device__ __forceinline__ void edge_body(const EdgeArgs<T> &a, gcsadmm_control_block *cb, double *sums, const ControlParams &cp, int *counters,
+                                          double *trace, unsigned *ticket, const unsigned bx, const unsigned nblocks, double (*red)[5], int *is_last,
+                                          const EdgePre &pre = EdgePre())
+{
+    static_assert(!P::TAIL || (MODE == 1 && U == 1), "the tail of the vertex launch is the single-workgroup edge step");
+    double mu_scale;
+    if constexpr (P::TAIL) mu_scale = pre.mu_scale;
+    else {
+        if (cb->status != GCSADMM_RUNNING) return;
+        mu_scale = cb->mu_scale;
+    }
+    double s[5] = {0, 0, 0, 0, 0};
+    if constexpr (P::TAIL) {
+        constexpr int CH = tail_words<T, C>();
+        const int e = (int)threadIdx.x;
+        if (P::edge_thread() && e < a.E) {
+            const int it = pre.it, ih = pre.ih;
+            const double we = a.edge_counted ? (double)a.edge_counted[e] : 1.0;
+            const double wt = a.inc_counted ? (double)a.inc_counted[it] : 1.0;
+            const double wh = a.inc_counted ? (double)a.inc_counted[ih] : 1.0;
+#pragma unroll
+            for (int w0 = 0; w0 < C; w0 += CH) {
+                T cu_[CH], cw_[CH], zo_[CH], mu_[CH], mw_[CH];
+#pragma unroll
+                for (int j = 0; j < CH; ++j) {
+                    const int w = w0 + j;
+                    if (w >= C) break;
+                    cu_[j] = P::load_copy(&a.copy[(size_t)w * a.NI + it]); cw_[j] = P::load_copy(&a.copy[(size_t)w * a.NI + ih]);
+                    zo_[j] = a.zedge[(size_t)w * a.E + e];
+                    mu_[j] = a.mu[(size_t)w * a.NI + it]; mw_[j] = a.mu[(size_t)w * a.NI + ih];
+                }
+#pragma unroll
+                for (int j = 0; j < CH; ++j) {
+                    const int w = w0 + j;
+                    if (w >= C) break;
+                    edge_word(a, w, e, it, ih, cu_[j], cw_[j], zo_[j], mu_[j], mw_[j], mu_scale, we, wt, wh, s);
+                }
+            }
+        }
+    } else
+    for (int base = bx * (U * EDGE_BLOCK); base < a.E; base += nblocks * (U * EDGE_BLOCK)) {
+        int it[U], ih[U];
+        T cu_[U][C], cw_[U][C], zo_[U][C], mu_[U][C], mw_[U][C];
+#pragma unroll
+        for (int q = 0; q < U; ++q) {
+            const int e = base + q * EDGE_BLOCK + (int)threadIdx.x, ee = e < a.E ? e : a.E - 1;
+            it[q] = a.edge_inc_tail ? a.edge_inc_tail[ee] : ee; ih[q] = a.edge_inc_head ? a.edge_inc_head[ee] : a.E + ee;
+#pragma unroll
+            for (int w = 0; w < C; ++w) {
+                cu_[q][w] = a.copy[(size_t)w * a.NI + it[q]]; cw_[q][w] = a.copy[(size_t)w * a.NI + ih[q]];
+                zo_[q][w] = a.zedge[(size_t)w * a.E + ee];
+                mu_[q][w] = a.mu[(size_t)w * a.NI + it[q]]; mw_[q][w] = a.mu[(size_t)w * a.NI + ih[q]];
+            }
+        }
+#pragma unroll
+        for (int q = 0; q < U; ++q) {
+            const int e = base + q * EDGE_BLOCK + (int)threadIdx.x;
+            if (e >= a.E) break;
+            const double we = a.edge_counted ? (double)a.edge_counted[e] : 1.0;
+            const double wt = a.inc_counted ? (double)a.inc_counted[it[q]] : 1.0;
+            const double wh = a.inc_counted ? (double)a.inc_counted[ih[q]] : 1.0;
+#pragma unroll
+            for (int w = 0; w < C; ++w)
+                edge_word(a, w, e, it[q], ih[q], cu_[q][w], cw_[q][w], zo_[q][w], mu_[q][w], mw_[q][w], mu_scale, we, wt, wh, s);
+        }
+    }
+    const int lane = threadIdx.x & 63, wv = threadIdx.x >> 6;
+#pragma unroll
+    for (int k = 0; k < 5; ++k) {
+        const double t = wave_sum(s[k]);
+        if (lane == 0 && P::edge_thread()) red[wv][k] = t;
+    }
+    P::sync();
+    if (threadIdx.x < 5) {
+        double t = 0;
+        for (int q = 0; q < EDGE_BLOCK / EDGE_WAVE; ++q) t += red[q][threadIdx.x];
+        if (MODE >= 2) __hip_atomic_store(&a.partials[(size_t)bx * 5 + threadIdx.x], t, __ATOMIC_RELAXED, __HIP_MEMORY_SCOPE_AGENT);
+        else a.partials[(size_t)bx * 5 + threadIdx.x] = t;
+        if (MODE == 1) sums[threadIdx.x] = t;
+        if constexpr (P::TAIL) red[0][threadIdx.x] = t;
+    }
+    if (MODE == 1) {
+        P::sync();
+        if (threadIdx.x == 0) control_body<P>(cb, P::TAIL ? &red[0][0] : sums, cp, counters, trace);
+    }
+    if (MODE >= 2) {
+        if (threadIdx.x < EDGE_WAVE) asm volatile("s_waitcnt vmcnt(0)" ::: "memory");
+        if (threadIdx.x == 0) {
+            const unsigned t = __hip_atomic_fetch_add(ticket, 1u, __ATOMIC_RELAXED, __HIP_MEMORY_SCOPE_AGENT);
+            *is_last = (t == nblocks - 1);
+        }
+        __syncthreads();
+        if (!*is_last) return;
+        double acc[5] = {0, 0, 0, 0, 0};
+        for (int b = threadIdx.x; b < (int)nblocks; b += EDGE_BLOCK)
+            for (int k = 0; k < 5; ++k) acc[k] += __hip_atomic_load(&a.partials[(size_t)b * 5 + k], __ATOMIC_RELAXED, __HIP_MEMORY_SCOPE_AGENT);
+        __syncthreads();
+        for (int k = 0; k < 5; ++k) red[threadIdx.x][k] = acc[k];
+        __syncthreads();
+        for (int off = EDGE_BLOCK / 2; off > 0; off >>= 1) {
+            if ((int)threadIdx.x < off)
+                for (int k = 0; k < 5; ++k) red[threadIdx.x][k] += red[threadIdx.x + off][k];
+            __syncthreads();
+        }
+        if (threadIdx.x < 5) sums[threadIdx.x] = red[0][threadIdx.x];
+        __syncthreads();
+        if (threadIdx.x == 0) {
+            if (MODE == 2) control_body(cb, sums, cp, counters, trace);
+            else sums[5] = (double)counters[0];
+            __hip_atomic_store(ticket, 0u, __ATOMIC_RELAXED, __HIP_MEMORY_SCOPE_AGENT);
+        }
+    }
+}
+
+}
diff --git a/gcs_admm_amd/csrc/gcsadmm.hip b/gcs_admm_amd/csrc/gcsadmm.hip
--- a/gcs_admm_amd/csrc/gcsadmm.hip
+++ b/gcs_admm_amd/csrc/gcsadmm.hip
@@ -36,173 +36,17 @@
 #include "canonical_box.h"
 #include "create_plan.h"
 #include "batch_plan.h"
+#include "edge_step.h"
 
 namespace {
 
 using namespace gcs;
 using namespace gcsadmm_k;
 
-template <class T> struct EdgeArgs {
-    int E, NI, c;
-    const int *edge_inc_tail, *edge_inc_head;
-    const uint8_t *inc_counted, *edge_counted;
-    const T *copy;
-    T *zedge, *mu;
-    double *partials;
-};
-
-__device__ __forceinline__ double wave_sum(double v)
-{
-#pragma unroll
-    for (int off = 32; off > 0; off >>= 1) v += __shfl_down(v, off, 64);
-    return v;
-}
-
-__device__ __forceinline__ double scaled_plus(double scale, double x, double r)
-{
-#pragma clang fp contract(off)
-    return scale * x + r;
-}
-
-struct ControlParams {
-    double tau_incr, tau_decr, nu, eps_abs, eps_rel, nx, nmu;
-    int it_rho_limit, max_it;
-};
-
-__device__ void control_body(gcsadmm_control_block *cb, const double *sums, const ControlParams &p, int *counters, double *trace,
-                             bool global_fails = false)
-{
-    if (cb->status != GCSADMM_RUNNING) return;
-    double s[5];
-    for (int k = 0; k < 5; ++k) { s[k] = sums[k]; cb->sums[k] = s[k]; }
-    const int it = cb->it;
-    double rho = cb->rho;
-    const int fails = global_fails ? (int)(sums[5] + 0.5) : counters[0], iters = counters[1];
-    counters[0] = 0; counters[1] = 0;
-    cb->inner_failures = fails; cb->inner_iters = iters;
-    const double tot = s[0] + s[1] + s[2] + s[3] + s[4];
-    if (!(fabs(tot) <= 1.7976931348623157e308)) {
-        cb->status = GCSADMM_DIVERGED;
-        return;
-    }
-    const double pri = sqrt(s[0]), dual = rho * sqrt(2.0 * s[1]);
-    double mu_scale = 1.0;
-    if (pri >= p.nu * dual && it < p.it_rho_limit) { rho *= p.tau_incr; mu_scale = 1.0 / p.tau_incr; }
-    else if (dual >= p.nu * pri && it < p.it_rho_limit) { rho *= 1.0 / p.tau_decr; mu_scale = p.tau_incr; }
-    const double eps_pri = sqrt(p.nx) * p.eps_abs + p.eps_rel * fmax(sqrt(s[2]), sqrt(2.0 * s[3]));
-    const double eps_dual = sqrt(p.nmu) * p.eps_abs + p.eps_rel * mu_scale * sqrt(s[4]);
-    cb->rho = rho; cb->mu_scale = mu_scale;
-    cb->pri = pri; cb->dual = dual; cb->eps_pri = eps_pri; cb->eps_dual = eps_dual;
-    if (trace) {
-        double *tr = trace + (size_t)(it - 1) * 6;
-        tr[0] = rho; tr[1] = pri; tr[2] = dual; tr[3] = eps_pri; tr[4] = eps_dual; tr[5] = (double)fails;
-    }
-    if (pri < eps_pri && dual < eps_dual) { cb->status = GCSADMM_CONVERGED; return; }
-    cb->it = it + 1;
-    if (it + 1 > p.max_it) cb->status = GCSADMM_MAX_IT;
-}
-
 __global__ void control_kernel(gcsadmm_control_block *cb, const double *sums, ControlParams p, int *counters, double *trace, bool global_fails)
 {
     if (threadIdx.x != 0 || blockIdx.x != 0) return;
     control_body(cb, sums, p, counters, trace, global_fails);
-}
-
-template <class T, int C> __host__ __device__ constexpr int edge_unroll() { return sizeof(T) == 4 ? (C <= 7 ? 4 : 2) : (C <= 7 ? 2 : 1); }
-
-template <class T, int MODE, int C, int U>
-__device__ __forceinline__ void edge_body(const EdgeArgs<T> &a, gcsadmm_control_block *cb, double *sums, const ControlParams &cp, int *counters,
-                                          double *trace, unsigned *ticket, const unsigned bx, const unsigned nblocks, double (*red)[5], int *is_last)
-{
-    if (cb->status != GCSADMM_RUNNING) return;
-    const double mu_scale = cb->mu_scale;
-    double s[5] = {0, 0, 0, 0, 0};
-    for (int base = bx * (U * EDGE_BLOCK); base < a.E; base += nblocks * (U * EDGE_BLOCK)) {
-        int it[U], ih[U];
-        T cu_[U][C], cw_[U][C], zo_[U][C], mu_[U][C], mw_[U][C];
-#pragma unroll
-        for (int q = 0; q < U; ++q) {
-            const int e = base + q * EDGE_BLOCK + (int)threadIdx.x, ee = e < a.E ? e : a.E - 1;
-            it[q] = a.edge_inc_tail ? a.edge_inc_tail[ee] : ee; ih[q] = a.edge_inc_head ? a.edge_inc_head[ee] : a.E + ee;
-#pragma unroll
-            for (int w = 0; w < C; ++w) {
-                cu_[q][w] = a.copy[(size_t)w * a.NI + it[q]]; cw_[q][w] = a.copy[(size_t)w * a.NI + ih[q]];
-                zo_[q][w] = a.zedge[(size_t)w * a.E + ee];
-                mu_[q][w] = a.mu[(size_t)w * a.NI + it[q]]; mw_[q][w] = a.mu[(size_t)w * a.NI + ih[q]];
-            }
-        }
-#pragma unroll
-        for (int q = 0; q < U; ++q) {
-            const int e = base + q * EDGE_BLOCK + (int)threadIdx.x;
-            if (e >= a.E) break;
-            const double we = a.edge_counted ? (double)a.edge_counted[e] : 1.0;
-            const double wt = a.inc_counted ? (double)a.inc_counted[it[q]] : 1.0;
-            const double wh = a.inc_counted ? (double)a.inc_counted[ih[q]] : 1.0;
-#pragma unroll
-            for (int w = 0; w < C; ++w) {
-                const double cu = (double)cu_[q][w], cw = (double)cw_[q][w], zo = (double)zo_[q][w];
-                const T zn_t = (T)(0.5 * (cu + cw));
-                const double zn = (double)zn_t;
-                const double ru = cu - zn, rw = cw - zn;
-                const T mu_u_t = (T)scaled_plus(mu_scale, (double)mu_[q][w], ru);
-                const T mu_w_t = (T)scaled_plus(mu_scale, (double)mw_[q][w], rw);
-                a.mu[(size_t)w * a.NI + it[q]] = mu_u_t;
-                a.mu[(size_t)w * a.NI + ih[q]] = mu_w_t;
-                a.zedge[(size_t)w * a.E + e] = zn_t;
-                const double mu_u = (double)mu_u_t, mu_w = (double)mu_w_t;
-                s[0] += wt * ru * ru + wh * rw * rw;
-                s[1] += we * (zn - zo) * (zn - zo);
-                s[2] += wt * cu * cu + wh * cw * cw;
-                s[3] += we * zn * zn;
-                s[4] += wt * mu_u * mu_u + wh * mu_w * mu_w;
-            }
-        }
-    }
-    const int lane = threadIdx.x & 63, wv = threadIdx.x >> 6;
-#pragma unroll
-    for (int k = 0; k < 5; ++k) {
-        const double t = wave_sum(s[k]);
-        if (lane == 0) red[wv][k] = t;
-    }
-    __syncthreads();
-    if (threadIdx.x < 5) {
-        double t = 0;
-        for (int q = 0; q < EDGE_BLOCK / WAVE; ++q) t += red[q][threadIdx.x];
-        if (MODE >= 2) __hip_atomic_store(&a.partials[(size_t)bx * 5 + threadIdx.x], t, __ATOMIC_RELAXED, __HIP_MEMORY_SCOPE_AGENT);
-        else a.partials[(size_t)bx * 5 + threadIdx.x] = t;
-        if (MODE == 1) sums[threadIdx.x] = t;
-    }
-    if (MODE == 1) {
-        __syncthreads();
-        if (threadIdx.x == 0) control_body(cb, sums, cp, counters, trace);
-    }
-    if (MODE >= 2) {
-        if (threadIdx.x < WAVE) asm volatile("s_waitcnt vmcnt(0)" ::: "memory");
-        if (threadIdx.x == 0) {
-            const unsigned t = __hip_atomic_fetch_add(ticket, 1u, __ATOMIC_RELAXED, __HIP_MEMORY_SCOPE_AGENT);
-            *is_last = (t == nblocks - 1);
-        }
-        __syncthreads();
-        if (!*is_last) return;
-        double acc[5] = {0, 0, 0, 0, 0};
-        for (int b = threadIdx.x; b < (int)nblocks; b += EDGE_BLOCK)
-            for (int k = 0; k < 5; ++k) acc[k] += __hip_atomic_load(&a.partials[(size_t)b * 5 + k], __ATOMIC_RELAXED, __HIP_MEMORY_SCOPE_AGENT);
-        __syncthreads();
-        for (int k = 0; k < 5; ++k) red[threadIdx.x][k] = acc[k];
-        __syncthreads();
-        for (int off = EDGE_BLOCK / 2; off > 0; off >>= 1) {
-            if ((int)threadIdx.x < off)
-                for (int k = 0; k < 5; ++k) red[threadIdx.x][k] += red[threadIdx.x + off][k];
-            __syncthreads();
-        }
-        if (threadIdx.x < 5) sums[threadIdx.x] = red[0][threadIdx.x];
-        __syncthreads();
-        if (threadIdx.x == 0) {
-            if (MODE == 2) control_body(cb, sums, cp, counters, trace);
-            else sums[5] = (double)counters[0];
-            __hip_atomic_store(ticket, 0u, __ATOMIC_RELAXED, __HIP_MEMORY_SCOPE_AGENT);
-        }
-    }
 }
 
 template <class T, int MODE, int C, int U>
@@ -358,6 +202,7 @@
     gcsadmm_batch_s *batch = nullptr;
     std::vector<gcsadmm_batch_s *> batches;
     int overlap_mode = 0;
+    int fused_tail_mode = 1;
     std::string err;
     void *comm = nullptr;
     int rank = 0, world = 1;
@@ -389,6 +234,7 @@
     int n_special() const { return (int)g.d_special_vtx.size(); }
     int n_wg() const { return (int)g.d_wg_vtx.size(); }
     int n_split() const { return (int)g.d_split_vtx.size(); }
+    bool fuses() const { return plan.fused_tail && fused_tail_mode != 0 && !halo.attached(); }
 };
 
 struct gcsadmm_batch_s {
@@ -531,7 +377,12 @@
     return d;
 }
 
-static gcsadmm_status launch_vertex(gcsadmm_handle h, const gcsadmm_state *st, hipStream_t s, int part = -1, bool reorder = false)
+static gcsadmm_status launch_vertex(gcsadmm_handle h, const gcsadmm_state *st, hipStream_t s, int part = -1, bool reorder = false,
+                                    bool fused = false, double *fused_trace = nullptr);
+template <class T> static EdgeArgs<T> make_edge_args(gcsadmm_handle h, const gcsadmm_state *st);
+static WgTailDesc make_wg_tail(gcsadmm_handle h, const gcsadmm_state *st, double *trace);
+
+static gcsadmm_status launch_vertex(gcsadmm_handle h, const gcsadmm_state *st, hipStream_t s, int part, bool reorder, bool fused, double *fused_trace)
 {
     const auto &g = h->g;
     const int n_waves = h->plan.n_waves();
@@ -564,8 +415,10 @@
     const bool special_on_wave = n_waves > 0;
     if (n_waves > 0) launch_waves(make_launch_desc(h, st));
     if (h->n_wg() > 0 || (!special_on_wave && h->n_special() > 0)) {
-        if (h->plan.wg_t512) gcsadmm_wg_launch_t512(make_wg_desc(h, st, !special_on_wave), s);
-        else gcsadmm_wg_launch(make_wg_desc(h, st, !special_on_wave), s);
+        WgLaunchDesc d = make_wg_desc(h, st, !special_on_wave);
+        if (fused) d.tail = make_wg_tail(h, st, fused_trace);
+        if (h->plan.wg_t512) gcsadmm_wg_launch_t512(d, s);
+        else gcsadmm_wg_launch(d, s);
     }
     if (h->n_split() > 0) {
         WgLaunchDesc d = make_wg_desc(h, st, false);
@@ -588,6 +441,17 @@
     a.inc_counted = h->g.d_inc_counted.get(); a.edge_counted = h->g.d_edge_counted.get();
     a.copy = (const T *)st->copy; a.zedge = (T *)st->zedge; a.mu = (T *)st->mu; a.partials = h->loop.d_partials.get();
     return a;
+}
+
+static WgTailDesc make_wg_tail(gcsadmm_handle h, const gcsadmm_state *st, double *trace)
+{
+    WgTailDesc t;
+    t.enabled = 1;
+    const EdgeArgs<char> a = make_edge_args<char>(h, st);
+    t.edge = EdgeArgs<void>{a.E, a.NI, a.c, a.edge_inc_tail, a.edge_inc_head, a.inc_counted, a.edge_counted, a.copy, a.zedge, a.mu, a.partials};
+    t.cb = h->loop.d_cb.get(); t.sums = h->loop.d_sums.get(); t.cp = control_params(h);
+    t.counters = h->loop.d_counters.get(); t.trace = trace; t.ticket = h->loop.d_ticket.get();
+    return t;
 }
 
 static gcsadmm_status launch_edge(gcsadmm_handle h, const gcsadmm_state *st, double *sums, hipStream_t s, bool with_control = false,
@@ -962,8 +826,13 @@
 {
     if (!state_ok(h, st) || k < 0) return GCSADMM_ERR_BAD_ARG;
     USE_DEVICE(h);
+    const bool fused = h->fuses();
     for (int i = 0; i < k; ++i) {
         gcsadmm_status s;
+        if (fused) {
+            if ((s = launch_vertex(h, st, (hipStream_t)stream, -1, false, true, trace_dev)) != GCSADMM_OK) return s;
+            continue;
+        }
         if ((s = gcsadmm_vertex_step(h, st, stream)) != GCSADMM_OK) return s;
         if ((s = launch_edge(h, st, h->loop.d_sums.get(), (hipStream_t)stream, true, trace_dev)) != GCSADMM_OK) return s;
     }
@@ -1127,6 +996,13 @@
     }
     *vertex_ms = (float)acc[0]; *halo_ms = (float)acc[1]; *edge_ms = (float)acc[2]; *reduce_ms = (float)acc[3];
     return GCSADMM_OK;
+}
+
+int32_t gcsadmm_set_fused_tail(gcsadmm_handle h, int32_t mode)
+{
+    if (!h) return 0;
+    h->fused_tail_mode = mode != 0;
+    return h->fuses() ? 1 : 0;
 }
 
 gcsadmm_status gcsadmm_set_overlap(gcsadmm_handle h, int32_t mode, int32_t *boundary_units)
diff --git a/gcs_admm_amd/csrc/step_args.h b/gcs_admm_amd/csrc/step_args.h
--- a/gcs_admm_amd/csrc/step_args.h
+++ b/gcs_admm_amd/csrc/step_args.h
@@ -8,6 +8,15 @@
 namespace gcsadmm_k {
 
 constexpr int MAX_SPECIAL_DEG = 256;
+constexpr int EDGE_BLOCK = 256;
+constexpr int FUSED_TAIL_LDS_BYTES = (EDGE_BLOCK / 64 * 5 + 1) * 8;
+constexpr int wg_launch_lds_bytes(int plan_lds_bytes, bool fused_tail)
+{
+    int b = 4 * MAX_SPECIAL_DEG * 8;
+    if (plan_lds_bytes > b) b = plan_lds_bytes;
+    if (fused_tail && FUSED_TAIL_LDS_BYTES > b) b = FUSED_TAIL_LDS_BYTES;
+    return b;
+}
 
 struct StepArgsBase {
     const int *inc_ptr;
@@ -25,7 +34,17 @@
     int ipm_max_iter;
     double *warm = nullptr;
     const long long *warm_ptr = nullptr;
+    int publish = 0;
 };
+
+template <class T> GCS_HD void store_copy(T *p, T v, int publish)
+{
+#if defined(__HIP_DEVICE_COMPILE__)
+    if (publish) { __hip_atomic_store(p, v, __ATOMIC_RELAXED, __HIP_MEMORY_SCOPE_AGENT); return; }
+#endif
+    (void)publish;
+    *p = v;
+}
 
 template <class T> struct StepArgs : StepArgsBase {
     const T *zedge, *mu;
diff --git a/gcs_admm_amd/csrc/vertex_wg.h b/gcs_admm_amd/csrc/vertex_wg.h
--- a/gcs_admm_amd/csrc/vertex_wg.h
+++ b/gcs_admm_amd/csrc/vertex_wg.h
@@ -1480,7 +1480,7 @@
         if (w == 2 * N) val = yy;
         else if (w < N) val = out ? p[w] + yy * CEN[w] : un[W::TF + w];
         else val = out ? p[w] + yy * CEN[w - N] : p[w - N] + yy * CEN[w - N];
-        a.copy[(size_t)w * a.NI + inc] = (T)val;
+        gcsadmm_k::store_copy(&a.copy[(size_t)w * a.NI + inc], (T)val, a.publish);
     }
     WG_FOR_AT(k, NX, plo.at(NX)) {
         const int c = k < N ? k : k - N;
diff --git a/gcs_admm_amd/csrc/vertex_wg_kernel.h b/gcs_admm_amd/csrc/vertex_wg_kernel.h
--- a/gcs_admm_amd/csrc/vertex_wg_kernel.h
+++ b/gcs_admm_amd/csrc/vertex_wg_kernel.h
@@ -54,12 +54,61 @@
     }
 }
 
-template <int N, class T, bool BOX>
-__global__ __launch_bounds__(WG_THREADS, (wg_min_blocks<N, BOX>())) void vertex_wg_kernel(gcs_wg::WgArgs<T> a, SpecialArgs sp, const gcsadmm_control_block *cb)
+template <class T> struct WgTail {
+    int enabled;
+    EdgeArgs<T> edge;
+    gcsadmm_control_block *cb;
+    double *sums;
+    ControlParams cp;
+    int *counters;
+    double *trace;
+    unsigned *ticket;
+};
+
+template <class T, int C>
+__device__ __forceinline__ void wg_fused_tail(const WgTail<T> &t, double mu_scale, bool closed_form, double *smem)
+{
+    const EdgePre pre = edge_prefetch(t.edge, mu_scale);
+    asm volatile("s_waitcnt vmcnt(0)" ::: "memory");
+    __syncthreads();
+    double(*red)[5] = (double(*)[5])smem;
+    int *is_last = (int *)(smem + EDGE_BLOCK / EDGE_WAVE * 5);
+    if (threadIdx.x == 0) {
+        if (closed_form) {
+            __builtin_amdgcn_fence(__ATOMIC_RELEASE, "agent");
+            asm volatile("s_waitcnt vmcnt(0)" ::: "memory");
+        }
+        const unsigned k = __hip_atomic_fetch_add(t.ticket, 1u, __ATOMIC_RELAXED, __HIP_MEMORY_SCOPE_AGENT);
+        *is_last = (k == gridDim.x - 1);
+    }
+    __syncthreads();
+    if (!*is_last) return;
+    edge_body<T, 1, C, 1, EdgeInTail>(t.edge, t.cb, t.sums, t.cp, t.counters, t.trace, t.ticket, 0, 1, red, is_last, pre);
+    if (threadIdx.x == 0) __hip_atomic_store(t.ticket, 0u, __ATOMIC_RELAXED, __HIP_MEMORY_SCOPE_AGENT);
+}
+
+template <class T> constexpr size_t wg_tail_kernarg_offset()
+{
+    static_assert(alignof(gcs_wg::WgArgs<T>) == 8 && alignof(SpecialArgs) == 8 && alignof(WgTail<T>) == 8, "kernarg layout: every argument starts on 8 bytes");
+    return sizeof(gcs_wg::WgArgs<T>) + sizeof(SpecialArgs) + sizeof(const gcsadmm_control_block *);
+}
+
+template <int N, class T, bool BOX>
+__global__ __launch_bounds__(WG_THREADS, (wg_min_blocks<N, BOX>())) void vertex_wg_kernel(gcs_wg::WgArgs<T> a, SpecialArgs sp, const gcsadmm_control_block *cb,
+                                                                                 WgTail<T> )
 {
     extern __shared__ __attribute__((aligned(16))) double smem[];
     if (cb->status != GCSADMM_RUNNING) return;
     vertex_wg_body<N, T, BOX>(a, sp, cb->rho, cb->mu_scale, (int)blockIdx.x, smem);
+    typedef const __attribute__((address_space(4))) char *KernargPtr;
+    KernargPtr kp = (KernargPtr)__builtin_amdgcn_kernarg_segment_ptr();
+    asm volatile("" : "+s"(kp));
+    typedef const __attribute__((address_space(4))) WgTail<T> *TailPtr;
+    TailPtr tp = (TailPtr)(kp + wg_tail_kernarg_offset<T>());
+    if (!tp->enabled) return;
+    const WgTail<T> tail = *(const WgTail<T> *)tp;
+    const double mu_scale = __hip_atomic_load(&tail.cb->mu_scale, __ATOMIC_RELAXED, __HIP_MEMORY_SCOPE_WORKGROUP);
+    wg_fused_tail<T, 2 * N + 1>(tail, mu_scale, (int)blockIdx.x >= a.n_vtx, smem);
 }
 
 #if GCS_WG_THREADS == 256
@@ -103,13 +152,13 @@
 template <int N> constexpr bool WG_HAS_BOX = N == 3 || N == 6;
 template <class F> auto with_state(int dtype, F &&f) { return with_state_type(dtype == GCSADMM_F64, f); }
 
-template <class K, int N, class T, class X>
-void launch_kernels(const WgLaunchDesc &d, const gcs_wg::WgArgs<T> &a, unsigned grid, int lds, const X &extra, hipStream_t s)
+template <class K, int N, class T, class X, class... More>
+void launch_kernels(const WgLaunchDesc &d, const gcs_wg::WgArgs<T> &a, unsigned grid, int lds, const X &extra, hipStream_t s, const More &...more)
 {
     if constexpr (WG_HAS_BOX<N>) {
-        if (d.box) { hipLaunchKernelGGL((K::template kernel<N, T, true>()), dim3(grid), dim3(WG_THREADS), lds, s, a, extra, d.step.cb); return; }
-    }
-    hipLaunchKernelGGL((K::template kernel<N, T, false>()), dim3(grid), dim3(WG_THREADS), lds, s, a, extra, d.step.cb);
+        if (d.box) { hipLaunchKernelGGL((K::template kernel<N, T, true>()), dim3(grid), dim3(WG_THREADS), lds, s, a, extra, d.step.cb, more...); return; }
+    }
+    hipLaunchKernelGGL((K::template kernel<N, T, false>()), dim3(grid), dim3(WG_THREADS), lds, s, a, extra, d.step.cb, more...);
 }
 
 template <class K, int N> hipError_t set_lds(int dtype, int lds_bytes)
@@ -131,16 +180,24 @@
     return a;
 }
 
+template <class T> WgTail<T> in_lds_tail(const WgTailDesc &d)
+{
+    const EdgeArgs<void> &e = d.edge;
+    return WgTail<T>{d.enabled,
+                     EdgeArgs<T>{e.E, e.NI, e.c, e.edge_inc_tail, e.edge_inc_head, e.inc_counted, e.edge_counted, (const T *)e.copy, (T *)e.zedge, (T *)e.mu, e.partials},
+                     d.cb, d.sums, d.cp, d.counters, d.trace, d.ticket};
+}
+
 template <int N> void launch(const WgLaunchDesc &d, hipStream_t s)
 {
     with_state(d.dtype, [&](auto t) {
         using T = decltype(t);
-        const gcs_wg::WgArgs<T> a = in_lds_args<T>(d);
+        gcs_wg::WgArgs<T> a = in_lds_args<T>(d);
+        a.publish = d.tail.enabled;
         const SpecialArgs sp{d.n_special, d.special_vtx, d.special_kind};
         const unsigned grid = (unsigned)(d.n_vtx + (d.n_special + WG_THREADS - 1) / WG_THREADS);
         if (grid == 0) return;
-        const int lds = std::max(d.lds_bytes, (int)(4 * MAX_SPECIAL_DEG * sizeof(double)));
-        launch_kernels<InLdsKernels, N, T>(d, a, grid, lds, sp, s);
+        launch_kernels<InLdsKernels, N, T>(d, a, grid, wg_launch_lds_bytes(d.lds_bytes, d.tail.enabled != 0), sp, s, in_lds_tail<T>(d.tail));
     });
 }
 
diff --git a/gcs_admm_amd/csrc/vertex_wg_launch.h b/gcs_admm_amd/csrc/vertex_wg_launch.h
--- a/gcs_admm_amd/csrc/vertex_wg_launch.h
+++ b/gcs_admm_amd/csrc/vertex_wg_launch.h
@@ -1,10 +1,22 @@
 #pragma once
 #include <hip/hip_runtime.h>
 
+#include "edge_step.h"
 #include "gcsadmm.h"
 #include "step_args.h"
 
 namespace gcsadmm_k {
+
+struct WgTailDesc {
+    int enabled = 0;
+    EdgeArgs<void> edge{};
+    gcsadmm_control_block *cb = nullptr;
+    double *sums = nullptr;
+    ControlParams cp{};
+    int *counters = nullptr;
+    double *trace = nullptr;
+    unsigned *ticket = nullptr;
+};
 
 struct WgLaunchDesc {
     StepDesc step;
@@ -15,6 +27,7 @@
     int box;
     const int *order;
     int *unit_iters;
+    WgTailDesc tail;
 };
 
 struct WgSplitArgs {
diff --git a/gcs_admm_amd/solver.py b/gcs_admm_amd/solver.py
--- a/gcs_admm_amd/solver.py
+++ b/gcs_admm_amd/solver.py
@@ -112,6 +112,9 @@
     def enqueue(self, k: int):
         self._call("gcsadmm_run", C.byref(self.state), int(k), self.trace.data_ptr(), self._stream())
 
+    def set_fused_tail(self, mode: int = 1) -> bool:
+        return bool(self.lib.gcsadmm_set_fused_tail(self.h, int(mode)))
+
     def enqueue_timed(self, k: int):
         vm, em = C.c_float(0), C.c_float(0)
         vl, el = C.c_int32(0), C.c_int32(0)
diff --git a/include/gcsadmm.h b/include/gcsadmm.h
--- a/include/gcsadmm.h
+++ b/include/gcsadmm.h
@@ -100,6 +100,8 @@
 
 gcsadmm_status gcsadmm_run(gcsadmm_handle h, const gcsadmm_state *st, int32_t k, double *trace_dev, void *stream);
 
+int32_t gcsadmm_set_fused_tail(gcsadmm_handle h, int32_t mode);
+
 gcsadmm_status gcsadmm_read_control(gcsadmm_handle h, gcsadmm_control_block *out, void *stream);
 
 gcsadmm_status gcsadmm_cost(gcsadmm_handle h, const gcsadmm_state *st, double eps_edge, double *cost_dev, void *stream);
```

New measurement: 10140 iterations/s (median of 6 runs). +3.5%, better.
